# zhouyou-gu/sig-sdp-mmw

Hardware: AMD Instinct MI355X
Metric: mmw_iterations_per_sec (higher is better)
Workload: dtype f32

## Files before the change

include/mmw_hip.h:

```cpp
#ifndef MMW_HIP_H
#define MMW_HIP_H

#include <stddef.h>
#include <stdint.h>

#ifdef __cplusplus
extern "C" {
#endif

typedef struct mmw_solver mmw_solver;

#define MMW_OK 0
#define MMW_ERR_ARG (-1)
#define MMW_ERR_HIP (-2)
#define MMW_ERR_STATE (-3)

enum mmw_dtype { MMW_F32 = 0, MMW_F64 = 1 };
enum mmw_expm_method {
    MMW_EXPM_LANCZOS = 0,
    MMW_EXPM_TAYLOR = 1
};

enum mmw_field {
    MMW_F_Y = 0,
    MMW_F_E_ACCU = 1,
    MMW_F_E_THIS = 2,
    MMW_F_LVAL = 3,
    MMW_F_XVAL = 4,
    MMW_F_XAVG = 5,
    MMW_F_YAVG = 6,
    MMW_F_XHALF = 7,
    MMW_F_SKETCH = 8,
    MMW_F_S_SUM = 9,
    MMW_F_NORM_H = 10,
    MMW_F_ST_DATA = 11,
    MMW_F_PHASE_US = 12,
    MMW_F_EXPM_INFO = 13,
    MMW_F_FACTOR = 14,
    MMW_F_BLOCKING = 16,
    MMW_F_SPMM_KIND = 17,
    MMW_F_E_MAX = 18,
    MMW_F_DUAL_INFO = 19,
    MMW_F_FACTOR_INFO = 20,
    MMW_F_FACTOR_CALL = 21,
    MMW_F_SPLIT_CALL = 22,
    MMW_F_FACTOR_ROWNORM = 23,
    MMW_F_HEAD_CALL = 24,
    MMW_F_PATTERN = 25,
    MMW_F_BUILD_INFO = 26,
    MMW_F_LAPLACIAN = 27,
    MMW_F_SPECTRAL_INFO = 28,
    MMW_F_SPECTRAL_EIG = 29,
    MMW_F_GAP_INFO = 30,
    MMW_F_KERNEL_US = 15
};
enum mmw_ifield {
    MMW_I_L_INDPTR = 0,
    MMW_I_L_INDICES = 1,
    MMW_I_ST_INDPTR = 2,
    MMW_I_ST_INDICES = 3,
    MMW_I_GAIN_X = 4,
    MMW_I_GAIN_Y = 5,
    MMW_I_ASSO_X = 6,
    MMW_I_ASSO_Y = 7,
    MMW_I_DIAG_POS = 8,
    MMW_I_ASSO_POS = 9,
    MMW_I_PATTERN = 10,
    MMW_I_ROUND_LIST_BUILDS = 11
};

const char* mmw_last_error(void);
int mmw_version(void);
int mmw_device_count(int* n);

int mmw_create(mmw_solver** out, int device, int dtype, int32_t K, int32_t Z, int32_t rank_radio, double eta,
               int32_t nit, const int32_t* S_indptr, const int32_t* S_indices, const double* S_data,
               const int32_t* Q_indptr, const int32_t* Q_indices, const double* Q_data, const double* h_max);
int mmw_destroy(mmw_solver* s);

int mmw_sizes(mmw_solver* s, int64_t out[10]);

int mmw_set_expm(mmw_solver* s, int method, int max_order, double tol);
int mmw_set_timing(mmw_solver* s, int enabled);

int mmw_set_profile(mmw_solver* s, int enabled);

int mmw_bench_spmm(mmw_solver* s, int blocked, int reps, double* avg_us);

int mmw_reset(mmw_solver* s, int32_t nit);

int mmw_set_slots(mmw_solver* s, int32_t Z, int32_t nit);
int mmw_set_slots_warm(mmw_solver* s, int32_t Z, int32_t nit);
int mmw_carry(mmw_solver* dst, mmw_solver* src);
int mmw_carry_map(mmw_solver* dst, mmw_solver* src, int32_t* lmap, int64_t nl, int32_t* cmap, int64_t nc);
int mmw_set_eta(mmw_solver* s, double eta);

int mmw_iterate(mmw_solver* s, int32_t n, const double* randv, uint64_t seed);
int mmw_sync(mmw_solver* s);
int mmw_sketch(mmw_solver* s, uint64_t seed, int32_t iteration, double* out, int64_t n);

int mmw_read_f64(mmw_solver* s, int which, double* out, int64_t n);
int mmw_read_i32(mmw_solver* s, int which, int32_t* out, int64_t n);

int mmw_gap(mmw_solver* s, double out[3]);

int mmw_set_gap(mmw_solver* s, int enabled, int32_t m_cap, int32_t first_steps);
int mmw_read_gap(mmw_solver* s, double* out, int64_t n);
int mmw_gap_checks(int32_t K, int32_t m_cap, int32_t* out, int32_t room, int32_t* n);

int mmw_factor(mmw_solver* s, int32_t rank, double* out, uint64_t seed);

int mmw_factor_spectral(mmw_solver* s, int32_t Z, int32_t index_order, double* out, uint64_t seed);

#define MMW_FACTOR_RANDOM_MAX_COLS 2147483583
int mmw_factor_random(mmw_solver* s, int32_t cols, int32_t index_order, double* out, uint64_t seed);

int mmw_expm_apply(int device, int dtype, int method, int max_order, double tol, int32_t K, int32_t D,
                   const int32_t* indptr, const int32_t* indices, const double* data, const double* B,
                   double* out, double info[4], int32_t reps, double* kernel_us);

int mmw_sym_eig(int device, int32_t b, const double* G, double rel_tol, int32_t max_sweeps, double* theta, double* Q, int32_t* sweeps);

int mmw_round(mmw_solver* s, int32_t Zr, int32_t Dp, const double* gX, int32_t nbatch, const double* randv,
              int32_t* z_out, int32_t* rem_out);

typedef struct mmw_env mmw_env;
int mmw_env_create(mmw_env** out, int device, int32_t K, int32_t A, const double* sta_xy, const double* ap_xy, double fre_Hz,
                   double txp_offset, double min_s_n_ratio, double min_sinr, double noise_floor_dbm);
int mmw_env_destroy(mmw_env* e);
int mmw_env_sizes(mmw_env* e, int64_t out[4]);
int mmw_env_state(mmw_env* e, int32_t* S_indptr, int32_t* S_indices, double* S_data, int32_t* Q_indptr, int32_t* Q_indices,
                  double* Q_data, double* h_max);
int mmw_env_evaluate(mmw_env* e, const double* z_vec, int32_t Z, double packet_bit, double bandwidth, double slot_time,
                     double* sinr_out, double* bler_out);
int mmw_create_from_env(mmw_solver** out, mmw_env* env, int dtype, int32_t Z, int32_t rank_radio, double eta, int32_t nit);
int mmw_env_bounds(mmw_env* e, int32_t out[2]);
int mmw_env_move(mmw_env* e, const double* sta_xy);
int mmw_round_env(mmw_solver* s, mmw_env* e, int32_t Zr, int32_t Dp, const double* gX, int32_t nbatch, const double* randv,
                  int32_t* z_out, int32_t* rem_out);
int mmw_round_attempts(mmw_solver* s, int32_t Zr, int32_t Dp, const double* gX, int32_t nattempt, uint64_t seed, int pick_rule,
                       int32_t* z_out, int32_t* rem_out, int32_t* pick_out, int32_t* z_all);
int mmw_round_env_attempts(mmw_solver* s, mmw_env* e, int32_t Zr, int32_t Dp, const double* gX, int32_t nattempt, uint64_t seed, int pick_rule,
                           int32_t* z_out, int32_t* rem_out, int32_t* pick_out, int32_t* z_all);
int mmw_round_randv(mmw_solver* s, int32_t Zr, int32_t Dp, uint64_t seed, int32_t attempt, double* out, int64_t n);

typedef struct mmw_csr mmw_csr;
int mmw_csr_upload(mmw_csr** out, int device, int32_t K, int64_t nnzS, int64_t nnzQ, const int32_t* S_indptr,
                   const int32_t* S_indices, const double* S_data, const int32_t* Q_indptr, const int32_t* Q_indices,
                   const double* Q_data, const double* h_max);
int mmw_csr_wrap(mmw_csr** out, int device, int32_t K, int64_t nnzS, int64_t nnzQ, const int32_t* S_indptr,
                 const int32_t* S_indices, const double* S_data, const int32_t* Q_indptr, const int32_t* Q_indices,
                 const double* Q_data, const double* h_max);
int mmw_csr_destroy(mmw_csr* c);
int mmw_csr_sizes(mmw_csr* c, int64_t out[4]);
int mmw_csr_pointers(mmw_csr* c, void* out[7]);
int mmw_csr_state(mmw_csr* c, int32_t* S_indptr, int32_t* S_indices, double* S_data, int32_t* Q_indptr, int32_t* Q_indices,
                  double* Q_data, double* h_max);
int mmw_csr_bounds(mmw_csr* c, int32_t out[2]);
int mmw_create_from_csr(mmw_solver** out, mmw_csr* csr, int dtype, int32_t Z, int32_t rank_radio, double eta, int32_t nit);

typedef struct mmw_gm mmw_gm;
int mmw_gm_create(mmw_gm** out, int device, int32_t K, const int32_t* S_indptr, const int32_t* S_indices, const double* S_data,
                  const int32_t* Q_indptr, const int32_t* Q_indices, const double* Q_data, const double* h_max);
int mmw_gm_create_from_env(mmw_gm** out, mmw_env* e);
int mmw_gm_key(mmw_gm* g, int kind, double* key_out);
int mmw_gm_destroy(mmw_gm* g);
int mmw_gm_sizes(mmw_gm* g, int64_t out[4]);
int mmw_gm_pass(mmw_gm* g, const int32_t* order, int32_t n, int32_t nattempt, int32_t* list_out, int32_t* nlist);
int mmw_gm_run(mmw_gm* g, const double* key, int32_t Z, int32_t nattempt, int32_t* z_out, int32_t* zz_out, int32_t* rem_out);
int mmw_gm_assign(mmw_gm* g, int32_t Z, const int32_t* order, const int32_t* pref, int32_t* z_out, int32_t* rem_out);

typedef struct mmw_batch mmw_batch;
int mmw_batch_create(mmw_batch** out, int device, int32_t B, const int32_t* K, const int32_t* Z, int32_t rank_radio, double eta,
                     const int32_t* nit, const int32_t* const* S_indptr, const int32_t* const* S_indices, const double* const* S_data,
                     const int32_t* const* Q_indptr, const int32_t* const* Q_indices, const double* const* Q_data, const double* const* h_max);
int mmw_batch_destroy(mmw_batch* b);
int mmw_batch_sizes(mmw_batch* b, int32_t inst, int64_t out[10]);
int mmw_batch_set_slots(mmw_batch* b, const int32_t* Z, int32_t nit);
int mmw_batch_set_slots_warm(mmw_batch* b, const int32_t* Z, int32_t nit);
int mmw_batch_carry(mmw_batch* dst, mmw_batch* src, const int32_t* take);
int mmw_batch_carry_map(mmw_batch* dst, mmw_batch* src, int32_t inst, int32_t* lmap, int64_t nl, int32_t* cmap, int64_t nc);
int mmw_batch_reset(mmw_batch* b, int32_t nit);
int mmw_batch_set_eta(mmw_batch* b, const double* eta);
int mmw_batch_set_expm(mmw_batch* b, int max_order, double tol);
int mmw_batch_iterate(mmw_batch* b, int32_t n, const double* randv, const uint64_t* seeds);
int mmw_batch_set_gap(mmw_batch* b, int enabled, int32_t m_cap);
int mmw_batch_read_gap(mmw_batch* b, int32_t inst, double* out, int64_t n);
#define MMW_BATCH_MAX_PARTS 32
int mmw_batch_set_split(mmw_batch* b, const int32_t* parts);
#define MMW_BATCH_MAX_ROW_PARTS 64
int mmw_batch_set_row_split(mmw_batch* b, const int32_t* rows);
int mmw_batch_row_ranges(mmw_batch* b, int32_t inst, int32_t rows, int32_t* out);
#define MMW_BATCH_MAX_HEAD_PARTS 64
int mmw_batch_set_head_split(mmw_batch* b, const int32_t* parts);
int mmw_batch_head_ranges(mmw_batch* b, int32_t inst, int32_t parts, int32_t* out);
int mmw_batch_read_f64(mmw_batch* b, int32_t inst, int which, double* out, int64_t n);
int mmw_batch_read_i32(mmw_batch* b, int32_t inst, int which, int32_t* out, int64_t n);
int mmw_batch_sketch(mmw_batch* b, int32_t inst, uint64_t seed, int32_t iteration, double* out, int64_t n);
int mmw_batch_export(mmw_batch* b, int32_t inst, mmw_solver* h);
#define MMW_BATCH_EPILOGUE_MAX_K 1024
int mmw_batch_set_factor_split(mmw_batch* b, const int32_t* parts);
int mmw_batch_factor(mmw_batch* b, const int32_t* take, const int32_t* rank, const double* const* xavg);
int mmw_batch_round(mmw_batch* b, const int32_t* take, int32_t nattempt, int stop_at_first, const uint64_t* seeds, int32_t* z_out,
                    int32_t* rem_out, int32_t* used_out);
int mmw_batch_round_randv(mmw_batch* b, int32_t inst, uint64_t seed, int32_t attempt, double* out, int64_t n);
int mmw_batch_gm(mmw_batch* b, int kind, const int32_t* take, const int32_t* Z, int32_t nattempt, int32_t* z_out, int32_t* zz_out,
                 int32_t* rem_out, double* key_out);
int mmw_batch_factor_random(mmw_batch* b, const int32_t* take, const uint64_t* seeds);
int mmw_batch_factor_spectral(mmw_batch* b, const int32_t* take, const int32_t* Z);

typedef struct mmw_batch_env mmw_batch_env;
int mmw_batch_env_create(mmw_batch_env** out, int device, int32_t B, const int32_t* K, const int32_t* A, const double* const* ap_xy,
                         double fre_Hz, double txp_offset, double min_s_n_ratio, double min_sinr, double noise_floor_dbm);
int mmw_batch_env_destroy(mmw_batch_env* e);
int mmw_batch_env_move(mmw_batch_env* e, const double* const* sta_xy);
int mmw_batch_env_sizes(mmw_batch_env* e, int32_t inst, int64_t out[4]);
int mmw_batch_env_state(mmw_batch_env* e, int32_t inst, int32_t* S_indptr, int32_t* S_indices, double* S_data, int32_t* Q_indptr,
                        int32_t* Q_indices, double* Q_data, double* h_max);
int mmw_batch_env_evaluate(mmw_batch_env* e, const double* const* z_vec, const int32_t* Z, double packet_bit, double bandwidth,
                           double slot_time, double* const* sinr_out, double* const* bler_out);
int mmw_batch_round_env(mmw_batch* b, mmw_batch_env* e, const int32_t* take, int32_t nattempt, int stop_at_first,
                        const uint64_t* seeds, int32_t* z_out, int32_t* rem_out, int32_t* used_out);
int mmw_batch_create_from_env(mmw_batch** out, mmw_batch_env* env, const int32_t* Z, int32_t rank_radio, double eta, const int32_t* nit);
int mmw_batch_create_from_csr(mmw_batch** out, int32_t B, mmw_csr* const* csr, const int32_t* Z, int32_t rank_radio, double eta,
                              const int32_t* nit);
int mmw_batch_env_gm(mmw_batch_env* e, int kind, const int32_t* take, const int32_t* Z, int32_t nattempt, int32_t* z_out,
                     int32_t* zz_out, int32_t* rem_out, double* key_out);

#ifdef __cplusplus
}
#endif
#endif
```

sig_sdp_mmw_amd/_lib.py:

```python
import ctypes as C
import os
import weakref

import numpy as np

_HERE = os.path.dirname(os.path.abspath(__file__))
LIB_PATH = os.path.join(_HERE, "libmmw_hip.so")

F32, F64 = 0, 1
EXPM_LANCZOS, EXPM_TAYLOR = 0, 1

F_Y, F_E_ACCU, F_E_THIS, F_LVAL, F_XVAL, F_XAVG, F_YAVG, F_XHALF, F_SKETCH = range(9)
F_S_SUM, F_NORM_H, F_ST_DATA, F_PHASE_US, F_EXPM_INFO, F_FACTOR, F_KERNEL_US, F_BLOCKING, F_SPMM_KIND, F_E_MAX, F_DUAL_INFO = range(9, 20)
F_FACTOR_INFO = 20
F_FACTOR_CALL = 21
F_FACTOR_ROWNORM = 23
F_SPLIT_CALL = 22
F_HEAD_CALL = 24
BATCH_F_PATTERN = 25
BATCH_F_BUILD_INFO = 26
SOLVER_F_LAPLACIAN = 27
SOLVER_F_SPECTRAL_INFO = 28
SOLVER_F_SPECTRAL_EIG = 29
SOLVER_F_GAP_INFO = 30
BATCH_MAX_PARTS = 32
BATCH_MAX_ROW_PARTS = 64
BATCH_MAX_HEAD_PARTS = 64
BATCH_EPILOGUE_MAX_K = 1024
KERNEL_CLASSES = ["spmm", "sddmm", "dual", "loss", "krylov_vec", "sketch", "project", "greedy", "factor"]
I_L_INDPTR, I_L_INDICES, I_ST_INDPTR, I_ST_INDICES, I_GAIN_X, I_GAIN_Y, I_ASSO_X, I_ASSO_Y, I_DIAG_POS, I_ASSO_POS = range(10)
I_ROUND_LIST_BUILDS = 11
I_PATTERN = 10

EXPORTS = ["mmw_last_error", "mmw_version", "mmw_device_count", "mmw_create", "mmw_destroy", "mmw_sizes", "mmw_set_expm",
           "mmw_set_timing", "mmw_set_profile", "mmw_bench_spmm", "mmw_reset", "mmw_set_slots", "mmw_set_slots_warm", "mmw_set_eta", "mmw_iterate", "mmw_sync", "mmw_sketch", "mmw_read_f64", "mmw_read_i32", "mmw_gap",
           "mmw_factor", "mmw_expm_apply", "mmw_sym_eig", "mmw_round", "mmw_env_create", "mmw_env_destroy", "mmw_env_sizes", "mmw_env_state",
           "mmw_env_evaluate", "mmw_create_from_env", "mmw_env_bounds", "mmw_gm_create", "mmw_gm_destroy", "mmw_gm_sizes", "mmw_gm_pass",
           "mmw_gm_run", "mmw_gm_assign", "mmw_batch_create", "mmw_batch_destroy", "mmw_batch_sizes", "mmw_batch_set_slots",
           "mmw_batch_set_slots_warm", "mmw_batch_reset", "mmw_batch_set_eta", "mmw_batch_set_expm", "mmw_batch_iterate", "mmw_batch_read_f64", "mmw_batch_read_i32",
           "mmw_batch_sketch", "mmw_batch_export", "mmw_batch_set_gap", "mmw_batch_read_gap", "mmw_batch_factor", "mmw_batch_round",
           "mmw_batch_round_randv", "mmw_batch_env_create", "mmw_batch_env_destroy", "mmw_batch_env_move", "mmw_batch_env_sizes",
           "mmw_batch_env_state", "mmw_batch_env_evaluate", "mmw_batch_round_env", "mmw_batch_gm", "mmw_batch_env_gm",
           "mmw_batch_factor_random", "mmw_batch_factor_spectral", "mmw_batch_set_split", "mmw_batch_set_factor_split", "mmw_batch_set_row_split",
           "mmw_batch_row_ranges", "mmw_batch_carry", "mmw_batch_carry_map", "mmw_batch_set_head_split", "mmw_batch_head_ranges",
           "mmw_batch_create_from_env", "mmw_batch_create_from_csr", "mmw_csr_upload", "mmw_csr_wrap", "mmw_csr_destroy", "mmw_csr_sizes", "mmw_csr_pointers", "mmw_csr_state",
           "mmw_csr_bounds", "mmw_create_from_csr", "mmw_factor_spectral", "mmw_env_move", "mmw_round_env", "mmw_gm_create_from_env", "mmw_gm_key", "mmw_carry", "mmw_carry_map",
           "mmw_round_attempts", "mmw_round_env_attempts", "mmw_round_randv", "mmw_factor_random",
           "mmw_set_gap", "mmw_read_gap", "mmw_gap_checks"]


class MMWError(RuntimeError):
    pass


_lib = None


def lib():
    global _lib
    if _lib is not None:
        return _lib
    if not os.path.exists(LIB_PATH):
        raise MMWError("HIP library %s not found: build it first (python -c 'import __graft_entry__ as g; g.build()'). "
                       "There is no CPU fallback." % LIB_PATH)
    L = C.CDLL(LIB_PATH)
    p_i32 = C.POINTER(C.c_int32)
    p_f64 = C.POINTER(C.c_double)
    L.mmw_last_error.restype = C.c_char_p
    L.mmw_last_error.argtypes = []
    L.mmw_version.restype = C.c_int
    L.mmw_device_count.argtypes = [C.POINTER(C.c_int)]
    L.mmw_create.argtypes = [C.POINTER(C.c_void_p), C.c_int, C.c_int, C.c_int32, C.c_int32, C.c_int32, C.c_double, C.c_int32,
                             p_i32, p_i32, p_f64, p_i32, p_i32, p_f64, p_f64]
    L.mmw_destroy.argtypes = [C.c_void_p]
    L.mmw_sizes.argtypes = [C.c_void_p, C.POINTER(C.c_int64)]
    L.mmw_set_expm.argtypes = [C.c_void_p, C.c_int, C.c_int, C.c_double]
    L.mmw_set_timing.argtypes = [C.c_void_p, C.c_int]
    L.mmw_set_profile.argtypes = [C.c_void_p, C.c_int]
    L.mmw_bench_spmm.argtypes = [C.c_void_p, C.c_int, C.c_int, p_f64]
    L.mmw_reset.argtypes = [C.c_void_p, C.c_int32]
    L.mmw_set_slots.argtypes = [C.c_void_p, C.c_int32, C.c_int32]
    L.mmw_set_slots_warm.argtypes = [C.c_void_p, C.c_int32, C.c_int32]
    L.mmw_set_eta.argtypes = [C.c_void_p, C.c_double]
    L.mmw_carry.argtypes = [C.c_void_p, C.c_void_p]
    L.mmw_carry_map.argtypes = [C.c_void_p, C.c_void_p, p_i32, C.c_int64, p_i32, C.c_int64]
    L.mmw_iterate.argtypes = [C.c_void_p, C.c_int32, p_f64, C.c_uint64]
    L.mmw_sync.argtypes = [C.c_void_p]
    L.mmw_sketch.argtypes = [C.c_void_p, C.c_uint64, C.c_int32, p_f64, C.c_int64]
    L.mmw_read_f64.argtypes = [C.c_void_p, C.c_int, p_f64, C.c_int64]
    L.mmw_read_i32.argtypes = [C.c_void_p, C.c_int, p_i32, C.c_int64]
    L.mmw_gap.argtypes = [C.c_void_p, p_f64]
    L.mmw_set_gap.argtypes = [C.c_void_p, C.c_int, C.c_int32, C.c_int32]
    L.mmw_read_gap.argtypes = [C.c_void_p, p_f64, C.c_int64]
    L.mmw_gap_checks.argtypes = [C.c_int32, C.c_int32, p_i32, C.c_int32, p_i32]
    L.mmw_factor.argtypes = [C.c_void_p, C.c_int32, p_f64, C.c_uint64]
    L.mmw_factor_spectral.argtypes = [C.c_void_p, C.c_int32, C.c_int32, p_f64, C.c_uint64]
    L.mmw_factor_random.argtypes = [C.c_void_p, C.c_int32, C.c_int32, p_f64, C.c_uint64]
    L.mmw_sym_eig.argtypes = [C.c_int, C.c_int32, p_f64, C.c_double, C.c_int32, p_f64, p_f64, C.POINTER(C.c_int32)]
    L.mmw_expm_apply.argtypes = [C.c_int, C.c_int, C.c_int, C.c_int, C.c_double, C.c_int32, C.c_int32, p_i32, p_i32, p_f64,
                                 p_f64, p_f64, p_f64, C.c_int32, p_f64]
    L.mmw_round.argtypes = [C.c_void_p, C.c_int32, C.c_int32, p_f64, C.c_int32, p_f64, p_i32, p_i32]
    L.mmw_env_create.argtypes = [C.POINTER(C.c_void_p), C.c_int, C.c_int32, C.c_int32, p_f64, p_f64, C.c_double, C.c_double, C.c_double, C.c_double,
                                 C.c_double]
    L.mmw_env_destroy.argtypes = [C.c_void_p]
    L.mmw_env_sizes.argtypes = [C.c_void_p, C.POINTER(C.c_int64)]
    L.mmw_env_state.argtypes = [C.c_void_p, p_i32, p_i32, p_f64, p_i32, p_i32, p_f64, p_f64]
    L.mmw_env_evaluate.argtypes = [C.c_void_p, p_f64, C.c_int32, C.c_double, C.c_double, C.c_double, p_f64, p_f64]
    L.mmw_create_from_env.argtypes = [C.POINTER(C.c_void_p), C.c_void_p, C.c_int, C.c_int32, C.c_int32, C.c_double, C.c_int32]
    L.mmw_env_bounds.argtypes = [C.c_void_p, p_i32]
    L.mmw_env_move.argtypes = [C.c_void_p, p_f64]
    L.mmw_round_env.argtypes = [C.c_void_p, C.c_void_p, C.c_int32, C.c_int32, p_f64, C.c_int32, p_f64, p_i32, p_i32]
    L.mmw_round_attempts.argtypes = [C.c_void_p, C.c_int32, C.c_int32, p_f64, C.c_int32, C.c_uint64, C.c_int, p_i32, p_i32, p_i32, p_i32]
    L.mmw_round_env_attempts.argtypes = [C.c_void_p, C.c_void_p, C.c_int32, C.c_int32, p_f64, C.c_int32, C.c_uint64, C.c_int, p_i32, p_i32, p_i32, p_i32]
    L.mmw_round_randv.argtypes = [C.c_void_p, C.c_int32, C.c_int32, C.c_uint64, C.c_int32, p_f64, C.c_int64]
    L.mmw_gm_create_from_env.argtypes = [C.POINTER(C.c_void_p), C.c_void_p]
    L.mmw_gm_key.argtypes = [C.c_void_p, C.c_int, p_f64]
    for fn in (L.mmw_csr_upload, L.mmw_csr_wrap):
        fn.argtypes = [C.POINTER(C.c_void_p), C.c_int, C.c_int32, C.c_int64, C.c_int64] + [C.c_void_p] * 7
    L.mmw_csr_destroy.argtypes = [C.c_void_p]
    L.mmw_csr_sizes.argtypes = [C.c_void_p, C.POINTER(C.c_int64)]
    L.mmw_csr_pointers.argtypes = [C.c_void_p, C.POINTER(C.c_void_p)]
    L.mmw_csr_state.argtypes = [C.c_void_p, p_i32, p_i32, p_f64, p_i32, p_i32, p_f64, p_f64]
    L.mmw_csr_bounds.argtypes = [C.c_void_p, p_i32]
    L.mmw_create_from_csr.argtypes = [C.POINTER(C.c_void_p), C.c_void_p, C.c_int, C.c_int32, C.c_int32, C.c_double, C.c_int32]
    L.mmw_gm_create.argtypes = [C.POINTER(C.c_void_p), C.c_int, C.c_int32, p_i32, p_i32, p_f64, p_i32, p_i32, p_f64, p_f64]
    L.mmw_gm_destroy.argtypes = [C.c_void_p]
    L.mmw_gm_sizes.argtypes = [C.c_void_p, C.POINTER(C.c_int64)]
    L.mmw_gm_pass.argtypes = [C.c_void_p, p_i32, C.c_int32, C.c_int32, p_i32, p_i32]
    L.mmw_gm_run.argtypes = [C.c_void_p, p_f64, C.c_int32, C.c_int32, p_i32, p_i32, p_i32]
    L.mmw_gm_assign.argtypes = [C.c_void_p, C.c_int32, p_i32, p_i32, p_i32, p_i32]
    pp_i32 = C.POINTER(p_i32)
    pp_f64 = C.POINTER(p_f64)
    L.mmw_batch_create.argtypes = [C.POINTER(C.c_void_p), C.c_int, C.c_int32, p_i32, p_i32, C.c_int32, C.c_double, p_i32,
                                   pp_i32, pp_i32, pp_f64, pp_i32, pp_i32, pp_f64, pp_f64]
    L.mmw_batch_destroy.argtypes = [C.c_void_p]
    L.mmw_batch_sizes.argtypes = [C.c_void_p, C.c_int32, C.POINTER(C.c_int64)]
    L.mmw_batch_set_slots.argtypes = [C.c_void_p, p_i32, C.c_int32]
    L.mmw_batch_set_slots_warm.argtypes = [C.c_void_p, p_i32, C.c_int32]
    L.mmw_batch_carry.argtypes = [C.c_void_p, C.c_void_p, p_i32]
    L.mmw_batch_carry_map.argtypes = [C.c_void_p, C.c_void_p, C.c_int32, p_i32, C.c_int64, p_i32, C.c_int64]
    L.mmw_batch_reset.argtypes = [C.c_void_p, C.c_int32]
    L.mmw_batch_set_eta.argtypes = [C.c_void_p, p_f64]
    L.mmw_batch_set_expm.argtypes = [C.c_void_p, C.c_int, C.c_double]
    L.mmw_batch_iterate.argtypes = [C.c_void_p, C.c_int32, p_f64, C.POINTER(C.c_uint64)]
    L.mmw_batch_read_f64.argtypes = [C.c_void_p, C.c_int32, C.c_int, p_f64, C.c_int64]
    L.mmw_batch_read_i32.argtypes = [C.c_void_p, C.c_int32, C.c_int, p_i32, C.c_int64]
    L.mmw_batch_sketch.argtypes = [C.c_void_p, C.c_int32, C.c_uint64, C.c_int32, p_f64, C.c_int64]
    L.mmw_batch_export.argtypes = [C.c_void_p, C.c_int32, C.c_void_p]
    L.mmw_batch_set_gap.argtypes = [C.c_void_p, C.c_int, C.c_int32]
    L.mmw_batch_read_gap.argtypes = [C.c_void_p, C.c_int32, p_f64, C.c_int64]
    L.mmw_batch_set_split.argtypes = [C.c_void_p, p_i32]
    L.mmw_batch_set_factor_split.argtypes = [C.c_void_p, p_i32]
    L.mmw_batch_set_row_split.argtypes = [C.c_void_p, p_i32]
    L.mmw_batch_row_ranges.argtypes = [C.c_void_p, C.c_int32, C.c_int32, p_i32]
    L.mmw_batch_set_head_split.argtypes = [C.c_void_p, p_i32]
    L.mmw_batch_head_ranges.argtypes = [C.c_void_p, C.c_int32, C.c_int32, p_i32]
    L.mmw_batch_factor.argtypes = [C.c_void_p, p_i32, p_i32, pp_f64]
    L.mmw_batch_round.argtypes = [C.c_void_p, p_i32, C.c_int32, C.c_int, C.POINTER(C.c_uint64), p_i32, p_i32, p_i32]
    L.mmw_batch_round_randv.argtypes = [C.c_void_p, C.c_int32, C.c_uint64, C.c_int32, p_f64, C.c_int64]
    L.mmw_batch_env_create.argtypes = [C.POINTER(C.c_void_p), C.c_int, C.c_int32, p_i32, p_i32, pp_f64, C.c_double, C.c_double, C.c_double,
                                       C.c_double, C.c_double]
    L.mmw_batch_env_destroy.argtypes = [C.c_void_p]
    L.mmw_batch_env_move.argtypes = [C.c_void_p, pp_f64]
    L.mmw_batch_env_sizes.argtypes = [C.c_void_p, C.c_int32, C.POINTER(C.c_int64)]
    L.mmw_batch_env_state.argtypes = [C.c_void_p, C.c_int32, p_i32, p_i32, p_f64, p_i32, p_i32, p_f64, p_f64]
    L.mmw_batch_env_evaluate.argtypes = [C.c_void_p, pp_f64, p_i32, C.c_double, C.c_double, C.c_double, pp_f64, pp_f64]
    L.mmw_batch_round_env.argtypes = [C.c_void_p, C.c_void_p, p_i32, C.c_int32, C.c_int, C.POINTER(C.c_uint64), p_i32, p_i32, p_i32]
    L.mmw_batch_gm.argtypes = [C.c_void_p, C.c_int, p_i32, p_i32, C.c_int32, p_i32, p_i32, p_i32, p_f64]
    L.mmw_batch_env_gm.argtypes = [C.c_void_p, C.c_int, p_i32, p_i32, C.c_int32, p_i32, p_i32, p_i32, p_f64]
    L.mmw_batch_factor_random.argtypes = [C.c_void_p, p_i32, C.POINTER(C.c_uint64)]
    L.mmw_batch_factor_spectral.argtypes = [C.c_void_p, p_i32, p_i32]
    L.mmw_batch_create_from_env.argtypes = [C.POINTER(C.c_void_p), C.c_void_p, p_i32, C.c_int32, C.c_double, p_i32]
    L.mmw_batch_create_from_csr.argtypes = [C.POINTER(C.c_void_p), C.c_int32, C.POINTER(C.c_void_p), p_i32, C.c_int32, C.c_double, p_i32]
    for name in EXPORTS:
        if name not in ("mmw_last_error",):
            getattr(L, name).restype = C.c_int
    _lib = L
    return L


def check(rc):
    if rc != 0:
        raise MMWError("mmw_hip status %d: %s" % (rc, lib().mmw_last_error().decode("utf-8", "replace")))


def _pi(a):
    return a.ctypes.data_as(C.POINTER(C.c_int32))


def _pd(a):
    return a.ctypes.data_as(C.POINTER(C.c_double))


def _i32(a):
    return np.ascontiguousarray(a, dtype=np.int32)


def _f64(a):
    return np.ascontiguousarray(a, dtype=np.float64)


def _u64(seeds, B):
    return np.ascontiguousarray(np.broadcast_to(np.asarray(seeds, dtype=np.uint64), (B,)))


def _pu(a):
    return a.ctypes.data_as(C.POINTER(C.c_uint64))


def _opt_pi(t):
    return None if t is None else _pi(t)


def _gm_call(fn, handle, B, Ks, who, kind, Zs, nattempt, t, keys):
    Z = _i32(np.broadcast_to(np.asarray(Zs, dtype=np.int32), (B,)))
    n = max(1, sum(Ks[i] for i in who))
    zflat = np.empty(n, dtype=np.int32)
    kflat = np.empty(n, dtype=np.float64) if keys else None
    zz = np.empty(B, dtype=np.int32)
    rem = np.empty(B, dtype=np.int32)
    check(fn(handle, int(kind), _opt_pi(t), _pi(Z), int(nattempt), _pi(zflat), _pi(zz), _pi(rem), _pd(kflat) if keys else None))
    z, ks, o = [None] * B, [None] * B, 0
    for i in who:
        z[i] = zflat[o:o + Ks[i]]
        if keys:
            ks[i] = kflat[o:o + Ks[i]]
        o += Ks[i]
    return (z, zz, rem, ks) if keys else (z, zz, rem)


def device_count():
    n = C.c_int(0)
    check(lib().mmw_device_count(C.byref(n)))
    return n.value


def canonical_csr(m):
    import scipy.sparse
    m = scipy.sparse.csr_matrix(m)
    if not m.has_canonical_format:
        m = m.copy()
        m.sum_duplicates()
    return _i32(m.indptr), _i32(m.indices), _f64(m.data)


def _state_arrays(state):
    S, Q, h = state
    K = int(S.shape[0])
    if S.shape != (K, K) or Q.shape != (K, K) or len(h) != K:
        raise MMWError("state must be (S_gain KxK, Q_asso KxK, h_max[K])")
    return K, canonical_csr(S) + canonical_csr(Q) + (_f64(h),)


def _state_out(K, nnzS, nnzQ, fill):
    import scipy.sparse
    sp = np.empty(K + 1, dtype=np.int32); si = np.empty(nnzS, dtype=np.int32); sx = np.empty(nnzS, dtype=np.float64)
    qp = np.empty(K + 1, dtype=np.int32); qi = np.empty(nnzQ, dtype=np.int32); qx = np.empty(nnzQ, dtype=np.float64)
    h = np.empty(K, dtype=np.float64)
    fill(_pi(sp), _pi(si), _pd(sx), _pi(qp), _pi(qi), _pd(qx), _pd(h))
    return scipy.sparse.csr_matrix((sx, si, sp), shape=(K, K)), scipy.sparse.csr_matrix((qx, qi, qp), shape=(K, K)), h


_SIZE_NAMES = ("K", "Z", "D", "Dpad", "nnzL", "nnzST", "E_gain", "E_asso", "C", "iter")
_LEN = {F_Y: "C", F_E_ACCU: "C", F_E_THIS: "C", F_LVAL: "nnzL", F_XVAL: "nnzL", F_XAVG: "nnzL", F_YAVG: "C",
        F_S_SUM: "K", F_NORM_H: "K", F_ST_DATA: "nnzST", SOLVER_F_LAPLACIAN: "nnzL", F_FACTOR_ROWNORM: "K"}
_ILEN = {I_L_INDPTR: ("K", 1), I_L_INDICES: ("nnzL", 0), I_ST_INDPTR: ("K", 1), I_ST_INDICES: ("nnzST", 0), I_GAIN_X: ("E_gain", 0),
         I_GAIN_Y: ("E_gain", 0), I_ASSO_X: ("E_asso", 0), I_ASSO_Y: ("E_asso", 0), I_DIAG_POS: ("K", 0), I_ASSO_POS: ("E_asso", 0)}


def gap_checks(K, m_cap=0):
    n = C.c_int32(0)
    check(lib().mmw_gap_checks(int(K), int(m_cap), None, 0, C.byref(n)))
    out = np.empty(n.value, dtype=np.int32)
    check(lib().mmw_gap_checks(int(K), int(m_cap), _pi(out), int(out.size), C.byref(n)))
    return [int(x) for x in out]


class _Handle:
    _destroy = None

    def _closing(self):
        """Called by `close` while the handle is still valid."""

    def close(self):
        if getattr(self, "_h", None) is not None and self._h.value:
            try:
                self._closing()
            finally:
                getattr(lib(), self._destroy)(self._h)
                self._h = C.c_void_p()

    def __del__(self):
        try:
            self.close()
        except Exception:
            pass


class Solver(_Handle):
    _destroy = "mmw_destroy"

    def __init__(self, Z, state, nit, eta, rank_radio=2, dtype=F64, device=0):
        self.K, (sp, si, sx, qp, qi, qx, hm) = _state_arrays(state)
        self._h = C.c_void_p()
        check(lib().mmw_create(C.byref(self._h), int(device), int(dtype), self.K, int(Z), int(rank_radio), float(eta), int(nit),
                               _pi(sp), _pi(si), _pd(sx), _pi(qp), _pi(qi), _pd(qx), _pd(hm)))
        self._load_sizes()
        self.dtype = dtype
        self._timing = False
        self._timed = 0

    @classmethod
    def from_env(cls, env, Z, nit, eta, rank_radio=2, dtype=F64):
        self = cls.__new__(cls)
        self._h = C.c_void_p()
        check(lib().mmw_create_from_env(C.byref(self._h), env._h, int(dtype), int(Z), int(rank_radio), float(eta), int(nit)))
        self._load_sizes()
        self.dtype = dtype
        self._timing = False
        self._timed = 0
        return self

    @classmethod
    def from_csr(cls, csr, Z, nit, eta, rank_radio=2, dtype=F64):
        self = cls.__new__(cls)
        self._h = C.c_void_p()
        check(lib().mmw_create_from_csr(C.byref(self._h), csr._h, int(dtype), int(Z), int(rank_radio), float(eta), int(nit)))
# ... 1060 lines not shown
```

sig_sdp_mmw_amd/csrc/chunk_policy.h:

```cpp
#pragma once
#include <algorithm>
#include <cmath>

#include "kernels_expm.h"
#include "kernels_mfma.h"
#include "switches.h"

namespace mmw {

struct ChunkPolicy {
    int age0 = 0;
    int age(int iter) const { return age0 + iter; }
    double rho_prev = 0.0, rho_last = 0.0;
    int age_prev = -1, age_last = -1;
    bool warm_fresh = false;
    bool lagged_missed = false;
    bool plan_seen = false;
    bool chain_ok = false;
    int replays = 0;
    int m_guess = 3;
    bool first_guess = false;
    bool first_a16_guess = false;
    bool exact_plans_only = false;
    void on_reset() {
        age0 = 0; warm_fresh = false; age_prev = age_last = -1;
        chain_ok = false; plan_seen = false; lagged_missed = false; m_guess = 3;
    }
    void on_warm_restart(int iter) {
        age0 += iter; warm_fresh = true; age_prev = age_last = -1;
        chain_ok = false; lagged_missed = false;
    }
    void on_discard() { chain_ok = false; }
    void note_plan(const ExpmPlan& p, int iter) {
        if (age_last >= 0 && age(iter) > age_last) { rho_prev = rho_last; age_prev = age_last; }
        rho_last = p.rho; age_last = age(iter);
    }
    double growth_ratio(int iter, int ahead) const {
        double r = (double)(age(iter) + ahead + 1) / (double)std::max(age(iter), 1);
        if (age_prev >= 0 && age_last > age_prev && rho_last > 0.0 && rho_last > rho_prev) {
            const double slope = (rho_last - rho_prev) / (double)(age_last - age_prev);
            r = std::max(r, (rho_last + 1.5 * slope * (double)(ahead + 1)) / rho_last);
        }
        return r;
    }
    bool first_order_ok(const ExpmPlan& p, const Switches& sw, int iter, int ahead, bool fp32, double plane_rounding, bool a16 = false) const {
        if (sw.no_first_order || !fp32 || !p.apost || p.m_eff != 1 || p.first_est == 0u) return false;
        const double est = plan_estimate(p.first_est);
        const double g1 = growth_ratio(iter, ahead), absn_g = p.absn * g1;
        if (!(absn_g < 0.03)) return false;
        if (a16 ? !((F16_PLANE_EXPECT + F16_UNIT) * absn_g <= p.tol) : !(F16_PLANE_EXPECT * absn_g <= p.tol)) return false;
        const double rounding = std::exp(p.rho * g1) * (absn_g * (plane_rounding + (a16 ? F16_UNIT : F16_CA_TWO)) + F16_SUBNORMAL_ROW);
        return est <= p.tol / 4.0 && est * g1 * g1 + rounding <= 0.9 * p.tol;
    }
    int next_launch_order(const ExpmPlan& p, int max_order, int iter, int ahead = 0) const {
        if (p.m_eff <= 0) return std::min(max_order, p.m + 1);
        int spare = 1;
        if (p.apost && p.m_eff >= 1 && p.m_eff <= MAX_ORDER) {
            const double est = plan_estimate(p.conv[p.m_eff]);
            const double grow = std::pow(growth_ratio(iter, ahead), 2.0 * p.m_eff);
            if (est <= p.tol / 8.0 && est * grow <= p.tol / 2.0) spare = 0;
        }
        if (p.m_eff >= p.m_apriori) spare = 0;
        return std::min(max_order, p.m_eff + spare);
    }
    int room_iterations(const ExpmPlan& p, int iter) const {
        if (!p.apost || p.m_eff != 1) return 0;
        const double est = plan_estimate(p.conv[1]);
        if (!(est > 0.0)) return 32;
        double c = 0.5 * (double)age(iter) * (std::sqrt(p.tol / est) - 1.0);
        if (age_prev >= 0 && age_last > age_prev && rho_last > rho_prev && rho_last > 0.0)
            c = std::min(c, 0.5 * (std::sqrt(p.tol / est) - 1.0) * rho_last * (double)(age_last - age_prev) / (1.5 * (rho_last - rho_prev)));
        return c > 32.0 ? 32 : (c < 0.0 ? 0 : (int)c);
    }
    bool plan_has_room(const ExpmPlan& p) const { return p.apost && p.m_eff == 1 && plan_estimate(p.conv[1]) <= p.tol / 8.0; }
    bool lagged_ok(const ExpmPlan& p, const Switches& sw) const {
        if (sw.no_lagged_plan || lagged_missed || !p.apost || p.m_eff != 1) return false;
        return plan_estimate(p.conv[1]) <= p.tol / 2.0;
    }
    int chunk_length(const ExpmPlan& p, const Switches& sw, int iter, int left) const {
        int cap = lagged_ok(p, sw) ? std::max(8, std::min(32, age(iter))) : std::max(4, std::min(32, age(iter) / 2));
        if (chain_ok && age(iter) >= 4) cap = std::max(cap, std::min(32, room_iterations(p, iter)));
        if (warm_fresh) cap = 8;
        int chunk = std::min(left, cap);
        if (left - chunk == 1) ++chunk;
        return chunk;
    }
    void plan_chunk(const ExpmPlan& p, const Switches& sw, int max_order, int iter, int chunk, bool fp32, bool have_a16, double plane_rounding) {
        if (plan_seen) m_guess = next_launch_order(p, max_order, iter, chunk);
        first_guess = plan_seen && first_order_ok(p, sw, iter, chunk, fp32, plane_rounding);
        if (first_guess) m_guess = 1;
        first_a16_guess = first_guess && !sw.no_first_a16 && have_a16 && first_order_ok(p, sw, iter, chunk, fp32, plane_rounding, true);
        if (warm_fresh) {
            m_guess = std::min(max_order, std::max(2, p.m_eff + 1));
            first_guess = false;
        }
    }
    void plan_cautious(const ExpmPlan& p, int max_order) {
        first_guess = false;
        first_a16_guess = false;
        m_guess = std::min(max_order, std::max(std::max(p.m_apriori, p.m_eff), m_guess) + 1);
    }
};
}
```

sig_sdp_mmw_amd/csrc/expm_engine.h:

```cpp
#pragma once
#include <cmath>

#include <functional>
#include <type_traits>

#include "kernels_expm.h"
#include "kernels_mfma.h"
#include "runtime.h"

namespace mmw {

inline int make_layout(int D, int vec, BlockLayout& lay, std::string& err) {
    int lpr = (D + vec - 1) / vec;
    if (lpr <= 32) {
        int p = 1;
        while (p < lpr) p <<= 1;
        lpr = p;
        lay.G = WAVE / lpr;
        lay.NCH = 1;
    } else {
        lpr = (lpr + 7) / 8 * 8;
        if ((lpr + WAVE - 1) / WAVE > 4) {
            err = "sketch width D too large for this build (max 1024 f32 / 512 f64 columns)";
            return MMW_ERR_ARG;
        }
        lay.G = 1;
        lay.NCH = (lpr + WAVE - 1) / WAVE;
    }
    lay.D = D;
    lay.LPR = lpr;
    lay.Dpad = lpr * vec;
    return MMW_OK;
}

template <typename T> inline int slice_bytes(const Switches& sw, int K, const BlockLayout& lay) {
    const int row_bytes = lay.Dpad * (int)sizeof(T);
    if (sw.no_slice_spmm || K < 256) return 0;
    if ((size_t)K * 64 <= (size_t)SLICE_LDS_MAX && row_bytes % 64 == 0) return 64;
    if ((size_t)K * 32 <= (size_t)SLICE_LDS_MAX && row_bytes % 32 == 0) return 32;
    return 0;
}
template <typename T> inline int slice_ranges(int K, const BlockLayout& lay, int sb) {
    const int nslices = lay.Dpad * (int)sizeof(T) / sb;
    return std::max(1, std::min((K + 15) / 16, device_cus() / std::max(1, nslices)));
}
template <typename T> inline int generic_slabs(const Switches& sw, int K, const BlockLayout& lay, int nblk) {
    const int sb = slice_bytes<T>(sw, K, lay);
    return sb ? std::min(nblk, slice_ranges<T>(K, lay, sb)) : nblk;
}
template <typename T, int MODE>
inline int spmm_launch(hipStream_t st, const Switches& sw, int K, const BlockLayout& lay, int nblk, const int* indptr, const int* col, const T* val,
                       const T* in, T* out, T* F, const T* X2, double c1, double c2, double c3, double* partial,
                       const ExpmPlan* plan = nullptr, int step = 0, double* partial_o2 = nullptr, int nslabs_fold = -1) {
    if (const int sb = slice_bytes<T>(sw, K, lay)) {
        const int nslices = lay.Dpad * (int)sizeof(T) / sb;
        int nranges = slice_ranges<T>(K, lay, sb);
        if (MODE == SPMM_LANCZOS) nranges = std::min(nranges, nblk);
        const int fold = nslabs_fold > 0 ? nslabs_fold : nblk;
        const size_t lds = (size_t)K * sb;
        if (sb == 64) {
            MMW_TRY(set_max_lds(reinterpret_cast<const void*>(&k_spmm_slice<T, MODE, 64>), SLICE_LDS_MAX));
            hipLaunchKernelGGL((k_spmm_slice<T, MODE, 64>), dim3(nslices, nranges), dim3(SLICE_THREADS), lds, st, K, lay.Dpad, indptr, col, val, in, out, F, X2, c1, c2, c3,
                               partial, plan, step, partial_o2, fold);
        } else {
            MMW_TRY(set_max_lds(reinterpret_cast<const void*>(&k_spmm_slice<T, MODE, 32>), SLICE_LDS_MAX));
            hipLaunchKernelGGL((k_spmm_slice<T, MODE, 32>), dim3(nslices, nranges), dim3(SLICE_THREADS), lds, st, K, lay.Dpad, indptr, col, val, in, out, F, X2, c1, c2, c3,
                               partial, plan, step, partial_o2, fold);
        }
        MMW_HIP(hipGetLastError());
        return MMW_OK;
    }
    const size_t sh = MODE == SPMM_LANCZOS ? (size_t)WAVES_PER_BLOCK * lay.Dpad * sizeof(double) : 0;
    switch (lay.NCH) {
        case 1: hipLaunchKernelGGL((k_spmm<T, 1, MODE>), dim3(nblk), dim3(BLOCK), sh, st, K, lay, indptr, col, val, in, out, F, X2, c1, c2, c3, partial, plan, step, partial_o2); break;
        case 2: hipLaunchKernelGGL((k_spmm<T, 2, MODE>), dim3(nblk), dim3(BLOCK), sh, st, K, lay, indptr, col, val, in, out, F, X2, c1, c2, c3, partial, plan, step, partial_o2); break;
        case 3: hipLaunchKernelGGL((k_spmm<T, 3, MODE>), dim3(nblk), dim3(BLOCK), sh, st, K, lay, indptr, col, val, in, out, F, X2, c1, c2, c3, partial, plan, step, partial_o2); break;
        default: hipLaunchKernelGGL((k_spmm<T, 4, MODE>), dim3(nblk), dim3(BLOCK), sh, st, K, lay, indptr, col, val, in, out, F, X2, c1, c2, c3, partial, plan, step, partial_o2); break;
    }
    MMW_HIP(hipGetLastError());
    return MMW_OK;
}

inline Blk2Sched blk2_schedule(int nb, int ntiles) {
    const int slots = 2 * device_cus();
    Blk2Sched s;
    int tpw = (int)((double)nb * ntiles / (2.5 * slots) + 0.5);
    tpw = tpw < 1 ? 1 : (tpw > ntiles ? ntiles : tpw);
    s.nfull = 0; s.grid1 = 0; s.tpw_tail = tpw; s.groups_tail = (ntiles + tpw - 1) / tpw;
    return s;
}

inline unsigned long long* g_blk_stamps = nullptr;
template <typename T, int MODE>
inline int spmm_blk_launch(hipStream_t st, const BlkDev& B, int Dpad, const T* val_blk, const T* in, T* out, T* F, const T* X2,
                           double c1, double c2, double c3, double* partial, const ExpmPlan* plan = nullptr, int step = 0,
                           double* partial_o2 = nullptr) {
    if (B.half_tile) {
        constexpr int CT2 = B2_ROW_BYTES / (int)sizeof(T);
        const int ntiles = (Dpad + CT2 - 1) / CT2;
        const Blk2Sched sched = blk2_schedule(B.nb, ntiles);
        const int rem = B.nb - sched.nfull;
        const int grid = sched.grid1 + ((rem * sched.groups_tail + 7) / 8) * 8;
        MMW_TRY(set_max_lds(reinterpret_cast<const void*>(&k_spmm_blk2<T, MODE>), B2_LDS_BYTES));
        hipLaunchKernelGGL((k_spmm_blk2<T, MODE>), dim3(grid), dim3(B2_THREADS), B2_LDS_BYTES, st, B, Dpad, ntiles, sched, val_blk, in, out, F, X2, c1, c2, c3, partial, partial_o2, plan, step, g_blk_stamps);
        MMW_HIP(hipGetLastError());
        return MMW_OK;
    }
    constexpr int CT = BLK_TILE_BYTES / (int)sizeof(T);
    const int ntiles = (Dpad + CT - 1) / CT;
    int tpw = (int)((double)B.nb * ntiles / (3.0 * 256.0) + 0.5);
    tpw = tpw < 1 ? 1 : (tpw > ntiles ? ntiles : tpw);
    const int total = B.nb * ((ntiles + tpw - 1) / tpw);
    const int per = (total + 7) / 8;
    const size_t sh = (size_t)BLK_UNION_ROWS * BLK_TILE_BYTES + BLK_META_LDS + BLK_ROWINFO_LDS + BLK_UNOFF_LDS + (size_t)BLK_WAVES * CT * sizeof(double);
    MMW_TRY(set_max_lds(reinterpret_cast<const void*>(&k_spmm_blk<T, MODE>), (int)sh));
    hipLaunchKernelGGL((k_spmm_blk<T, MODE>), dim3(per * 8), dim3(BLK_THREADS), sh, st, B, Dpad, ntiles, tpw, val_blk, in, out, F, X2, c1, c2, c3, partial, plan, step, g_blk_stamps);
    MMW_HIP(hipGetLastError());
    return MMW_OK;
}

inline unsigned long long* g_mf_stamps = nullptr;
template <int MODE>
inline int spmm_mfma_launch(hipStream_t st, const Switches& sw, const MfmaDev& M, int mt, int Dpad, size_t plane_bytes, const char* planes, const float* in,
                            float* out, double ascale, double shift, double* partial, double* partial_o2, const ExpmPlan* plan, int step, int* viol,
                            MfEpi epi = MfEpi{}, int* grid_out = nullptr ,
                            hipEvent_t ev_a = nullptr, hipEvent_t ev_b = nullptr ) {
    const int ntiles = Dpad / 32;
    const int grid_x = (M.nb + 7) / 8 * 8;
    const int cus = device_cus();
#define MMW_MF_LAUNCH(MT, NT, NW, MS, KC, NB)                                                                                          \
    do {                                                                                                                               \
        constexpr int gtw = (NW / MS) * NT;                                                                                            \
        constexpr int lds_bytes = mf_lds_bytes<MT, gtw, KC, NB, mf_planes(MODE), mf_apieces(MODE)>();                                  \
        MMW_TRY(set_max_lds(reinterpret_cast<const void*>(&k_spmm_mfma<MODE, MT, NT, NW, MS, KC, NB>), lds_bytes));                    \
        if (ev_a)                                                                                                                      \
            hipExtLaunchKernelGGL((k_spmm_mfma<MODE, MT, NT, NW, MS, KC, NB>), dim3(grid_x, (ntiles + gtw - 1) / gtw), dim3(NW * 64),  \
                                  lds_bytes, st, ev_a, ev_b, 0, M, Dpad, plane_bytes, planes, in, out, ascale, shift, partial,         \
                                  partial_o2, plan, step, viol, g_mf_stamps, epi);                                                     \
        else                                                                                                                           \
        hipLaunchKernelGGL((k_spmm_mfma<MODE, MT, NT, NW, MS, KC, NB>), dim3(grid_x, (ntiles + gtw - 1) / gtw), dim3(NW * 64),         \
                           lds_bytes, st, M, Dpad, plane_bytes, planes, in, out, ascale, shift, partial, partial_o2,                   \
                           plan, step, viol, g_mf_stamps, epi);                                                                        \
        if (grid_out) *grid_out = grid_x * ((ntiles + gtw - 1) / gtw);                                                                 \
    } while (0)
    int gt = 12;
    if (sw.mf_gt) gt = sw.mf_gt;
    else {
        auto wgs = [&](int g) { return (long)M.nb * ((ntiles + g - 1) / g); };
        if (wgs(12) * 2 < 3L * cus) gt = 8;
        if (gt == 8 && wgs(8) * 2 < 3L * cus) gt = 4;
    }
    if (ntiles <= 4) gt = 4;
    else if (ntiles <= 8 && gt > 8) gt = 8;
    if (mt == 1) {
        if (gt == 4) MMW_MF_LAUNCH(1, 1, 4, 1, 2, 2);
        else if (gt == 8) MMW_MF_LAUNCH(1, 2, 4, 1, 2, 2);
        else MMW_MF_LAUNCH(1, 3, 4, 1, 1, 3);
    } else {
        if (gt == 4) {
            if constexpr (mf_first(MODE)) MMW_MF_LAUNCH(2, 1, 8, 2, 4, 2);
            else MMW_MF_LAUNCH(2, 1, 8, 2, 2, 2);
        }
        else if (gt == 8) MMW_MF_LAUNCH(2, 2, 8, 2, 2, 2);
        else MMW_MF_LAUNCH(2, 3, 4, 1, 1, 3);
    }
#undef MMW_MF_LAUNCH
    MMW_HIP(hipGetLastError());
    return MMW_OK;
}

template <typename T> struct ExpmEngine {
    const Switches& sw;
    explicit ExpmEngine(const Switches& s) : sw(s) {}
    hipStream_t st = nullptr;
    int K = 0;
    BlockLayout lay{};
    int method = MMW_EXPM_LANCZOS, max_order = 8;
    double tol = 1e-9;
    int nblk = 1, nwide = 1;
    const int* indptr = nullptr;
    const int* col = nullptr;
    const T* val = nullptr;
    DevBuf<T> U;
    DevBuf<T> Tm;
    DevBuf<double> partial_du;
    DevBuf<double> partial, partial_sq, partial_o2, colsum, scal, row_part;
    DevBuf<ExpmPlan> plan_d;
    DevBuf<int> viol_d;
    ExpmPlan* plan_h = nullptr;
    ExpmPlan last{};
    size_t bs = 0;
    KernelTimers* kt = nullptr;
    bool use_blk = false;
    BlkDev blk{};
    const T* val_blk = nullptr;
    int npart = 1;
    bool use_mfma = false;
    MfmaDev mf{};
    int mf_mt = 1;
    DevBuf<unsigned short> planes;
    bool mfma_now() const { return use_mfma && use_blk && std::is_same<T, float>::value && (lay.Dpad % 32) == 0 && last_mfma_ok; }
    int spmm_slabs() const { return mfma_now() ? mf.nb : npart; }
    int check_slabs(int slabs) const {
        if ((size_t)slabs * lay.Dpad > partial.cap || (size_t)slabs * lay.Dpad > partial_o2.cap)
            return fail(MMW_ERR_STATE, "internal: the per-block slabs of the SpMM outgrew their buffers");
        return MMW_OK;
    }
    bool last_mfma_ok = true;
    bool* blk_stale = nullptr;
    std::function<int()> blk_refresh;
    T* rownorm_d = nullptr;
    double* rownorm_part = nullptr;
    unsigned short* out_planes = nullptr;
    bool kt_exact = false;
    bool planes_only = false;
    bool start_colsq_ready = false;
    int npart_start = 0;
    bool apost() const { return (!use_blk || blk.half_tile) && method == MMW_EXPM_LANCZOS && !sw.no_apost; }
    int kbegin(int slot) { return kt ? kt->begin(slot) : MMW_OK; }
    int kend() { return kt ? kt->end() : MMW_OK; }

    ~ExpmEngine() {
        if (plan_h) (void)hipHostFree(plan_h);
    }
    int init(hipStream_t s, int K_, int D, const int* ip, const int* ci, const T* v) {
        st = s;
        K = K_;
        indptr = ip;
        col = ci;
        val = v;
        return resize(D);
    }
    int resize(int D) {
        std::string err;
        if (make_layout(D, V16<T>::N, lay, err) != MMW_OK) return fail(MMW_ERR_ARG, err);
        bs = (size_t)K * lay.Dpad;
        nblk = grid_slabs(K);
        nwide = grid_rows(K);
        ublocks = 0;
        for (auto& r : planes_ready) r = false;
        MMW_TRY(ensure_blocks(4));
        MMW_TRY(Tm.alloc(bs));
        const size_t slabs = std::max((size_t)MAX_PART, std::max(use_blk ? (size_t)blk.nb : (size_t)0, use_mfma ? (size_t)mf.nb : (size_t)0));
        MMW_TRY(partial.alloc(slabs * lay.Dpad));
        MMW_TRY(partial_sq.alloc((size_t)MAX_PART * lay.Dpad));
        MMW_TRY(partial_du.alloc((size_t)MAX_PART * lay.Dpad));
        MMW_TRY(partial_o2.alloc(slabs * lay.Dpad));
        npart = generic_slabs<T>(sw, K, lay, nblk);
        MMW_TRY(colsum.alloc(lay.Dpad));
        MMW_TRY(scal.alloc((size_t)4 * (MAX_ORDER + 2) * lay.Dpad));
        MMW_TRY(row_part.alloc((size_t)3 * ROW_GRID_MAX));
        MMW_TRY(plan_d.alloc(1));
        MMW_HIP(hipMemsetAsync(plan_d.p, 0, sizeof(ExpmPlan), st));
        MMW_TRY(reset_plan_history(false));
        MMW_TRY(viol_d.alloc(1));
        MMW_HIP(hipMemsetAsync(viol_d.p, 0, sizeof(int), st));
        if (!plan_h) MMW_HIP(hipHostMalloc((void**)&plan_h, sizeof(ExpmPlan)));
        if (use_blk) MMW_TRY(enable_blocking(blk, val_blk));
        return MMW_OK;
    }
    int ublocks = 0;
    int ensure_blocks(int n) {
        if (n <= ublocks) return MMW_OK;
        if (n > MAX_ORDER + 1) n = MAX_ORDER + 1;
        if (U.p && U.cap >= bs * (size_t)n) {
            if ((size_t)n > (size_t)std::max(ublocks, 1))
                MMW_HIP(hipMemsetAsync(U.p + bs * (size_t)std::max(ublocks, 1), 0, bs * (size_t)(n - std::max(ublocks, 1)) * sizeof(T), st));
            if (ublocks == 0) MMW_HIP(hipMemsetAsync(U.p, 0, bs * sizeof(T), st));
            U.n = bs * (size_t)n;
            ublocks = n;
            return MMW_OK;
        }
        DevBuf<T> bigger;
        MMW_TRY(bigger.alloc(bs * (size_t)n));
        MMW_HIP(hipMemsetAsync(bigger.p, 0, bs * (size_t)n * sizeof(T), st));
        if (U.p && ublocks > 0) MMW_HIP(hipMemcpyAsync(bigger.p, U.p, bs * sizeof(T), hipMemcpyDeviceToDevice, st));
        MMW_HIP(hipStreamSynchronize(st));
        std::swap(U.p, bigger.p);
        std::swap(U.n, bigger.n);
        std::swap(U.cap, bigger.cap);
        ublocks = n;
        return MMW_OK;
    }
    T* start_block() { return U.p; }
    T* block(int j) { return U.p + (size_t)j * bs; }
    LanczosScalars scalars() {
        LanczosScalars S;
        const size_t n = (size_t)(MAX_ORDER + 2) * lay.Dpad;
        S.alpha = scal.p;
        S.beta = scal.p + n;
        S.sinv = scal.p + 2 * n;
        S.coef = scal.p + 3 * n;
        return S;
    }

    unsigned short* planes_of(int idx) { return planes.p + (size_t)idx * 2 * bs; }
    bool planes_ready[MAX_ORDER + 2] = {false};
    bool planes0_f16 = false;
    int reserve_planes() {
        if (planes.n < (size_t)ublocks * 2 * bs) MMW_TRY(planes.alloc((size_t)ublocks * 2 * bs));
        for (auto& r : planes_ready) r = false;
        return MMW_OK;
    }
    int ensure_planes() {
        if (planes.n < (size_t)ublocks * 2 * bs) {
            MMW_HIP(hipStreamSynchronize(st));
            MMW_TRY(planes.alloc((size_t)ublocks * 2 * bs));
            for (auto& r : planes_ready) r = false;
        }
        return MMW_OK;
    }
    unsigned short* start_planes() {
        if (!mfma_now() || ensure_planes() != MMW_OK) return nullptr;
        return planes_of(0);
    }
    int make_planes(int idx) {
        if constexpr (std::is_same<T, float>::value) {
            MMW_TRY(ensure_planes());
            if (idx == 0 && planes0_f16) planes_ready[0] = false;
            if (planes_ready[idx]) return MMW_OK;
            if (idx == 0) planes0_f16 = false;
            MMW_TRY(kbegin(KT_KRYLOV_VEC));
            hipLaunchKernelGGL(k_split_planes, dim3(grid_elems(bs / 4)), dim3(BLOCK), 0, st, bs / 4, reinterpret_cast<const float4*>(block(idx)),
                               reinterpret_cast<uint2*>(planes_of(idx)), reinterpret_cast<uint2*>(planes_of(idx) + bs));
            MMW_HIP(hipGetLastError());
            return kend();
        }
        return MMW_OK;
    }
    template <int MODE> int launch_spmm(const T* in, T* out, T* F, double ascale, double shift, double inv_k,
                                        const ExpmPlan* plan = nullptr, int step = 0, const unsigned short* planes_in = nullptr) {
        if constexpr (std::is_same<T, float>::value && (MODE == SPMM_PLAIN || MODE == SPMM_LANCZOS)) {
            if (planes_in && mfma_now()) {
                MMW_TRY(check_slabs(mf.nb));
                hipEvent_t ea = nullptr, eb = nullptr;
                if (kt) MMW_TRY(kt->begin_attached(KT_SPMM, &ea, &eb));
                MMW_TRY((spmm_mfma_launch<MODE>(st, sw, mf, mf_mt, lay.Dpad, bs * sizeof(unsigned short), reinterpret_cast<const char*>(planes_in), in, out, ascale,
                                                shift, partial.p, apost() ? partial_o2.p : nullptr, plan, step, viol_d.p, MfEpi{}, nullptr, ea, eb)));
                return kend();
            }
        }
        if (use_blk && blk_stale && *blk_stale) {
            MMW_TRY(blk_refresh());
            *blk_stale = false;
        }
        MMW_TRY(kbegin(KT_SPMM));
        if (use_blk)
            MMW_TRY((spmm_blk_launch<T, MODE>(st, blk, lay.Dpad, val_blk, in, out, F, nullptr, ascale, shift, inv_k, partial.p, plan, step,
                                              apost() ? partial_o2.p : nullptr)));
        else
            MMW_TRY((spmm_launch<T, MODE>(st, sw, K, lay, nblk, indptr, col, val, in, out, F, nullptr, ascale, shift, inv_k, partial.p, plan, step,
                                          apost() ? partial_o2.p : nullptr, npart)));
        return kend();
    }
    int enable_blocking(const BlkDev& b, const T* values_blocked) {
        blk = b;
        val_blk = values_blocked;
        use_blk = true;
        npart = b.nb;
        if ((size_t)b.nb > (size_t)MAX_PART) {
            MMW_TRY(partial.alloc((size_t)b.nb * lay.Dpad));
            MMW_TRY(partial_o2.alloc((size_t)b.nb * lay.Dpad));
        }
        return MMW_OK;
    }
    template <int OP> int colreduce(int nb, int j, const ExpmPlan* plan) {
        const double eps = sizeof(T) == 4 ? 1e-6 : 1e-14;
        hipLaunchKernelGGL((k_colreduce<OP>), dim3((lay.Dpad + 15) / 16), dim3(1024), 0, st, nb, lay.Dpad, partial.p, colsum.p, j, eps, scalars(), plan);
        MMW_HIP(hipGetLastError());
        return MMW_OK;
    }

    int plan_iter = 0;
    int reset_plan_history(bool keep_sums) {
        hipLaunchKernelGGL(k_plan_reset, dim3(1), dim3(64), 0, st, plan_d.p, keep_sums ? 1 : 0);
        MMW_HIP(hipGetLastError());
        return MMW_OK;
    }
    int make_plan(double ascale, int m_launch) {
        hipLaunchKernelGGL((k_rowsums<T>), dim3(nwide), dim3(BLOCK), 0, st, K, indptr, col, val, ascale, row_part.p);
        hipLaunchKernelGGL(k_plan, dim3(1), dim3(PLAN_THREADS), 0, st, K, method, max_order, tol, row_part.p, nwide, plan_d.p, m_launch, viol_d.p, apost() ? 1 : 0,
                           plan_iter);
        MMW_HIP(hipGetLastError());
        if (m_launch > 0) return MMW_OK;
        MMW_HIP(hipMemcpyAsync(plan_h, plan_d.p, sizeof(ExpmPlan), hipMemcpyDeviceToHost, st));
        MMW_HIP(hipStreamSynchronize(st));
        last = *plan_h;
        last_mfma_ok = last.mfma_ok != 0;
        if (last.overflow) return fail(MMW_ERR_STATE, "expm: the one-norm of the matrix is too large for max_order (raise max_order)");
        return MMW_OK;
    }
    int fetch_plan(int* violated) {
        int v = 0;
        MMW_HIP(hipMemcpyAsync(plan_h, plan_d.p, sizeof(ExpmPlan), hipMemcpyDeviceToHost, st));
        MMW_HIP(hipMemcpyAsync(&v, viol_d.p, sizeof(int), hipMemcpyDeviceToHost, st));
        MMW_HIP(hipStreamSynchronize(st));
        last = *plan_h;
        last_mfma_ok = last.mfma_ok != 0;
        if (live_switch(LIVE_VERBOSE)) {
            fprintf(stderr, "[plan] rho %.3e absn %.3e mfma_ok %d tol %.1e m %d (a-priori %d) apost %d m_eff %d est[1] %.3e est[2] %.3e viol %d\n", last.rho,
                    last.absn, last.mfma_ok, last.tol, last.m, last.m_apriori, last.apost, last.m_eff, plan_estimate(last.conv[1]), plan_estimate(last.conv[2]), v);
        }
        if (violated) *violated = v;
        return MMW_OK;
    }
    int clear_violation() {
        MMW_HIP(hipMemsetAsync(viol_d.p, 0, sizeof(int), st));
        return MMW_OK;
    }

    int apply_first(T* out, double ascale, int m_launch, bool plan_made, unsigned short* y_planes, long long* dfx, double* tr_part, int* ntr,
                    const unsigned short* afrag16 = nullptr) {
        if constexpr (std::is_same<T, float>::value) {
            if (!plan_made) MMW_TRY(make_plan(ascale, m_launch));
            MMW_TRY(ensure_planes());
            if (!(planes_ready[0] && planes0_f16)) {
                MMW_TRY(kbegin(KT_KRYLOV_VEC));
                hipLaunchKernelGGL(k_plane_f16, dim3(grid_elems(bs / 4)), dim3(BLOCK), 0, st, bs / 4, reinterpret_cast<const float4*>(U.p),
                                   reinterpret_cast<uint2*>(planes_of(0)));
                MMW_HIP(hipGetLastError());
                MMW_TRY(kend());
            }
            MfEpi E;
            E.y_planes = y_planes; E.dfx = dfx; E.tr_part = tr_part;
            MMW_TRY(check_slabs(mf.nb));
            hipEvent_t ea = nullptr, eb = nullptr;
            if (kt) MMW_TRY(kt->begin_attached(KT_SPMM, &ea, &eb));
            if (afrag16) {
                MfmaDev m16 = mf;
                m16.afrag = reinterpret_cast<const unsigned*>(afrag16);
                MMW_TRY((spmm_mfma_launch<SPMM_FIRST16>(st, sw, m16, mf_mt, lay.Dpad, bs * sizeof(unsigned short), reinterpret_cast<const char*>(planes_of(0)), U.p, out,
                                                        ascale / (double)MF_F16_SCALE, 0.0, partial.p, partial_o2.p, plan_d.p, 1, viol_d.p, E, ntr, ea, eb)));
            } else
                MMW_TRY((spmm_mfma_launch<SPMM_FIRST>(st, sw, mf, mf_mt, lay.Dpad, bs * sizeof(unsigned short), reinterpret_cast<const char*>(planes_of(0)), U.p, out,
                                                      ascale / (double)MF_F16_SCALE, 0.0, partial.p, partial_o2.p, plan_d.p, 1, viol_d.p, E, ntr, ea, eb)));
            MMW_TRY(kend());
            planes_ready[0] = false;
            planes0_f16 = false;
            start_colsq_ready = false;
            return MMW_OK;
        }
        return fail(MMW_ERR_STATE, "the first-order product runs on fp32 matrix-core handles only");
    }
    int first_grid_max() const { return (mf.nb + 7) / 8 * 8 * (lay.Dpad / 32); }

    int apply(T* out, double ascale, int m_launch = 0, bool plan_made = false) {
        if (!plan_made) MMW_TRY(make_plan(ascale, m_launch));
        const int m = m_launch > 0 ? m_launch : last.m;
        const int nsub = m_launch > 0 ? 1 : last.nsub;
        MMW_TRY(ensure_blocks(std::max(3, m)));
        ExpmPlan* pd = plan_d.p;
        const int Dpad = lay.Dpad;
        const int gcol = (Dpad + 63) / 64;
        const int gel = grid_elems(bs);
        const size_t shcol = (size_t)BLOCK * sizeof(double);
        for (int sub = 0; sub < nsub; ++sub) {
            if (sub > 0) {
                hipLaunchKernelGGL((k_copy<T>), dim3(gel), dim3(BLOCK), 0, st, bs, out, U.p);
            }
            if (method == MMW_EXPM_LANCZOS) {
                LanczosScalars S = scalars();
                const int gr = grid_slabs(K * 4);
                const double eps = sizeof(T) == 4 ? 1e-6 : 1e-14;
                int nsq = npart_start;
                if (!(sub == 0 && start_colsq_ready)) {
                    MMW_TRY(kbegin(KT_KRYLOV_VEC));
                    hipLaunchKernelGGL((k_colsq<T>), dim3(gr), dim3(BLOCK), shcol, st, K, Dpad, U.p, partial_sq.p);
                    MMW_TRY(kend());
                    nsq = gr;
                }
                start_colsq_ready = false;
                for (int j = 1; j <= m; ++j) {
                    const bool mf_step = mfma_now();
                    if (mf_step) MMW_TRY(make_planes(j - 1));
                    MMW_TRY((launch_spmm<SPMM_LANCZOS>(block(j - 1), Tm.p, nullptr, ascale, 0.0, 1.0, pd, j, mf_step ? planes_of(j - 1) : nullptr)));
                    planes_ready[j - 1] = false;
                    MMW_TRY(kbegin(KT_KRYLOV_VEC));
#define MMW_LZS(NMAX)                                                                                                               \
    hipLaunchKernelGGL((k_lz_scalars<NMAX>), dim3((Dpad + LZS_COLS - 1) / LZS_COLS), dim3(1024), 0, st, mf_step ? mf.nb : npart, partial.p, \
                       apost() ? partial_o2.p : (double*)nullptr, nsq, partial_sq.p, Dpad, j, m, 1.0 / nsub, eps, S, pd)
                    if (j + 2 <= 4) MMW_LZS(4);
                    else if (j + 2 <= 8) MMW_LZS(8);
                    else MMW_LZS(MAX_ORDER + 2);
#undef MMW_LZS
                    if (kt && kt->on && kt_exact && apost() && j < m) {
                        MMW_TRY(kend());
                        MMW_HIP(hipMemcpyAsync(plan_h, plan_d.p, sizeof(ExpmPlan), hipMemcpyDeviceToHost, st));
                        MMW_HIP(hipStreamSynchronize(st));
                        union { float f; unsigned u; } tb;
                        tb.f = (float)plan_h->tol;
                        if (plan_h->apost && plan_h->conv[j] <= tb.u) break;
                        MMW_TRY(kbegin(KT_KRYLOV_VEC));
                    }
                    if (j < m) {
                        unsigned short* pl_next = nullptr;
                        if (mf_step && ensure_planes() == MMW_OK && j < ublocks) pl_next = planes_of(j);
                        hipLaunchKernelGGL((k_lz_update<T>), dim3(gr), dim3(BLOCK), shcol, st, K, Dpad, j, Tm.p, block(j - 1),
                                           j > 1 ? block(j - 2) : block(j - 1), block(j), S, partial_sq.p, pd, pl_next);
                        planes_ready[j] = pl_next != nullptr;
                        nsq = gr;
                    }
                    MMW_TRY(kend());
                }
                MMW_TRY(kbegin(KT_KRYLOV_VEC));
                const bool last = sub + 1 == nsub;
                hipLaunchKernelGGL((k_lz_combine<T>), dim3(nwide), dim3(BLOCK), 0, st, K, Dpad, m, U.p, bs, Tm.p, S.coef, out, pd,
                                   last ? rownorm_d : (T*)nullptr, last ? rownorm_part : (double*)nullptr, viol_d.p, last ? out_planes : (unsigned short*)nullptr,
                                   last && out_planes && planes_only ? 1 : 0);
                MMW_TRY(kend());
            } else {
                hipLaunchKernelGGL((k_copy<T>), dim3(gel), dim3(BLOCK), 0, st, bs, U.p, out);
                for (int k = 1; k <= m; ++k) {
                    T* in = k == 1 ? U.p : block((k - 1) % 2 + 1);
                    T* o = block(k % 2 + 1);
                    MMW_TRY((launch_spmm<SPMM_TAYLOR>(in, o, out, ascale / nsub, last.mu / nsub, 1.0 / k, pd, k)));
                }
                hipLaunchKernelGGL((k_scale<T>), dim3(gel), dim3(BLOCK), 0, st, bs, out, 1.0, pd);
            }
            MMW_HIP(hipGetLastError());
        }
        return MMW_OK;
    }
};

}
```

sig_sdp_mmw_amd/csrc/solver.h:

```cpp
#pragma once
#include "solver_bench.h"
#include "solver_carry.h"
#include "solver_create.h"
#include "solver_loop.h"
#include "solver_read.h"
#include "solver_replay.h"

struct mmw_env {
    mmw::EnvDevice e;
};
struct mmw_csr {
    mmw::CsrDevice c;
};
struct mmw_solver {
    virtual ~mmw_solver() {}
    virtual CarryInfo carry_info() = 0;
    virtual int carry_pattern(const mmw::HostPattern** out) = 0;
    virtual int carry(mmw_solver* src) = 0;
    virtual int sizes(int64_t out[10]) = 0;
    virtual int set_expm(int method, int max_order, double tol) = 0;
    virtual int set_timing(int enabled) = 0;
    virtual int set_profile(int enabled) = 0;
    virtual int bench_spmm(int blocked, int reps, double* avg_us) = 0;
    virtual int reset(int32_t nit) = 0;
    virtual int set_slots(int32_t Z, int32_t nit, int warm) = 0;
    virtual int set_eta(double eta) = 0;
    virtual int iterate(int32_t n, const double* randv, uint64_t seed) = 0;
    virtual int sync() = 0;
    virtual int sketch(uint64_t seed, int32_t iteration, double* out, int64_t n) = 0;
    virtual int read_f64(int which, double* out, int64_t n) = 0;
    virtual int read_i32(int which, int32_t* out, int64_t n) = 0;
    virtual int gap(double out[3]) = 0;
    virtual int set_gap(int enabled, int32_t m_cap, int32_t first_steps) = 0;
    virtual int read_gap(double* out, int64_t n) = 0;
    virtual int factor(int32_t rank, double* out, uint64_t seed) = 0;
    virtual int factor_spectral(int32_t Z, int32_t index_order, double* out, uint64_t seed) = 0;
    virtual int factor_random(int32_t cols, int32_t index_order, double* out, uint64_t seed) = 0;
    virtual int round(int32_t Zr, int32_t Dp, const double* gX, int32_t nbatch, const double* randv, int32_t* z_out,
                      int32_t* rem_out) = 0;
    virtual int round_env(mmw_env* env, int32_t Zr, int32_t Dp, const double* gX, int32_t nbatch, const double* randv, int32_t* z_out,
                          int32_t* rem_out) = 0;
    virtual int round_attempts(mmw_env* env, bool with_env, int32_t Zr, int32_t Dp, const double* gX, int32_t nattempt, uint64_t seed, int pick_rule,
                               int32_t* z_out, int32_t* rem_out, int32_t* pick_out, int32_t* z_all) = 0;
    virtual int round_randv(int32_t Zr, int32_t Dp, uint64_t seed, int32_t attempt, double* out, int64_t n) = 0;
};
namespace {
inline int host_only_handle() { return fail(MMW_ERR_STATE, "host-only handle"); }
inline int host_only_pattern() { return fail(MMW_ERR_STATE, "this handle was created with device -1 (host pattern only)"); }
template <typename T> struct Solver final : mmw_solver {
    SolverCore<T> core;
    SolverLoop<T> loop;
    PendingChunk<T> pending;
    EmaxRecord emax;
    SolverReads<T> reads;
    DeviceLists envl;
    Extras<T> extras;
    CarriedPlan carried;
    explicit Solver(const Switches& s) : core(s), loop(core.sw), extras(core.sw) {}
    ~Solver() override {
        core.bt.join();
        if (core.host_only) return;
        (void)hipSetDevice(core.device);
        if (core.st) (void)hipStreamDestroy(core.st);
    }
    using Create = SolverCreate<T>;
    int sizes(int64_t out[10]) override {
        const HostPattern& H = core.H;
        out[0] = core.K; out[1] = core.Z; out[2] = core.D; out[3] = core.eng.lay.Dpad; out[4] = H.nnzL(); out[5] = H.nnzST();
        out[6] = H.E_gain(); out[7] = H.E_asso(); out[8] = H.C(); out[9] = core.iter;
        return MMW_OK;
    }
    int set_expm(int method, int max_order, double tol) override {
        if (method != MMW_EXPM_LANCZOS && method != MMW_EXPM_TAYLOR) return fail(MMW_ERR_ARG, "unknown expm method");
        if (max_order < 1 || max_order > MAX_ORDER) return fail(MMW_ERR_ARG, "max_order must be in [1,16]");
        if (!(tol > 0)) return fail(MMW_ERR_ARG, "tol must be positive");
        core.eng.method = method; core.eng.max_order = max_order; core.eng.tol = tol;
        return MMW_OK;
    }
    int set_timing(int enabled) override {
        core.pt.timing = enabled != 0;
        core.pt.timing_stride = enabled > 1 ? enabled : 1;
        return MMW_OK;
    }
    int bench_spmm(int blocked, int reps, double* avg_us) override {
        if (core.host_only) return host_only_handle();
        MMW_HIP(hipSetDevice(core.device));
        if (blocked && !core.bt.HB.usable) return fail(MMW_ERR_STATE, "no locality blocking for this pattern");
        MMW_TRY(sync());
        return solver_bench_spmm(core, loop, blocked, reps, avg_us);
    }
    int set_profile(int enabled) override {
        if (core.host_only) return host_only_handle();
        MMW_TRY(sync());
        KernelTimers& kt = core.kt;
        kt.on = enabled != 0;
        core.kt_shipped = enabled == 2;
        kt.attach = core.kt_shipped && !core.sw.kt_markers;
        core.eng.kt_exact = kt.on && !core.kt_shipped;
        kt.clear();
        return MMW_OK;
    }
    int set_eta(double eta_) override {
        if (!(eta_ >= 0.0)) return fail(MMW_ERR_ARG, "eta must be non-negative");
        if (!core.host_only) {
            MMW_HIP(hipSetDevice(core.device));
            MMW_TRY(settle());
        }
        core.eta = eta_;
        return MMW_OK;
    }
    int set_slots(int32_t Z_, int32_t nit_, int warm) override {
        if (core.host_only) return host_only_pattern();
        MMW_HIP(hipSetDevice(core.device));
        MMW_TRY(settle());
        MMW_HIP(hipStreamSynchronize(core.st));
        if (warm && core.iter == 0) warm = 0;
        if (Z_ >= 2) {
            BlockLayout probe{};
            std::string lerr;
            if ((int64_t)Z_ * core.rank_radio > INT32_MAX || make_layout(Z_ * core.rank_radio, V16<T>::N, probe, lerr) != MMW_OK)
                return fail(MMW_ERR_ARG, "mmw_set_slots: " + (lerr.empty() ? std::string("sketch width D too large for this build") : lerr));
        }
        std::string err = update_slots(core.H, Z_);
        if (!err.empty()) return fail(MMW_ERR_ARG, "mmw_set_slots: " + err);
        core.Z = Z_;
        core.D = core.Z * core.rank_radio;
        MMW_TRY(core.upload_slot_scalars());
        MMW_TRY(core.eng.resize(core.D));
        MMW_TRY(core.Xh.alloc(core.eng.bs));
        MMW_TRY(reads.resize(core));
        MMW_TRY(loop.resize(core));
        MMW_TRY(on_restart(nit_, warm != 0));
        return warm ? core.sums_from_current() : core.initial_point();
    }
    int on_restart(int32_t nit_, bool warm) {
        if (nit_ < 1) return fail(MMW_ERR_ARG, "nit must be >= 1");
        core.nit = nit_;
        loop.on_restart(warm, core.iter, nit_);
        core.iter = 0;
        emax.drop();
        pending.clear();
        carried.drop();
        if (core.eng.viol_d.p) MMW_TRY(core.eng.clear_violation());
        return core.eng.reset_plan_history(warm);
    }
    int reset(int32_t nit_) override {
        if (core.host_only) return host_only_pattern();
        MMW_HIP(hipSetDevice(core.device));
        MMW_TRY(on_restart(nit_, false));
        return core.initial_point();
    }
    int restore_pending() {
        loop.pol.on_discard();
        emax.drop();
        MMW_TRY(core.eng.clear_violation());
        MMW_TRY(pending.restore(core));
        loop.gap.drop_pending();
        core.iter = pending.iter0;
        return core.pt.drop_since(pending.events0, core.st);
    }
    void say_replay(int viol, const char* how) const {
        if (!live_switch(LIVE_VERBOSE)) return;
        const ExpmPlan& p = core.eng.last;
        const ChunkPolicy& pol = loop.pol;
        fprintf(stderr, "[replay] iterations %d..%d (Z %d) %s: reason bits %d (1 order, 2 lagged plan, 4 plan, 8 softmax, 16 operands, 32 first-order certificate); launched m %d, first-order %d, one-half %d; "
                        "plan m %d m_eff %d apriori %d rho %.3g absn %.3g est %.2e first_est %.2e tol %.1e\n",
                pending.iter0, pending.iter0 + pending.n - 1, (int)core.H.Z, how, viol, pol.m_guess, (int)pol.first_guess, (int)pol.first_a16_guess, p.m, p.m_eff, p.m_apriori, p.rho, p.absn,
                plan_estimate(p.conv[std::max(0, std::min(p.m_eff, MAX_ORDER))]), plan_estimate(p.first_est), p.tol);
    }
    void accept_plan() {
        ChunkPolicy& pol = loop.pol;
        pol.plan_seen = true;
        pol.note_plan(core.eng.last, core.iter);
        pol.m_guess = pol.next_launch_order(core.eng.last, core.eng.max_order, core.iter);
    }
    int settle() {
        MMW_TRY(settle_chunk());
        return loop.gap.collect(core.st, core.d_indptr.p, core.d_col.p);
    }
    int settle_chunk() {
        if (!pending.live) return MMW_OK;
        pending.clear();
        ChunkPolicy& pol = loop.pol;
        ExpmEngine<T>& eng = core.eng;
        int viol = 0;
        MMW_TRY(eng.fetch_plan(&viol));
        if (!viol) {
            accept_plan();
            return MMW_OK;
        }
        ++pol.replays;
        const bool operands_only = (viol & VIOL_OPERANDS) && !pol.first_guess;
        if (viol & VIOL_LAGGED) pol.lagged_missed = true;
        say_replay(viol, "discarded");
        MMW_TRY(restore_pending());
        if (core.sw.cautious_replay && !operands_only && eng.method == MMW_EXPM_LANCZOS && pending.n > 1) {
            pol.plan_cautious(eng.last, eng.max_order);
            pol.exact_plans_only = true;
            const int rc = loop.iterate_impl(core, pending.n, nullptr, pending.seed, true);
            pol.exact_plans_only = false;
            MMW_TRY(rc);
            viol = 0;
            MMW_TRY(eng.fetch_plan(&viol));
            if (!viol) {
                accept_plan();
                say_replay(0, "cautious attempt accepted");
                return MMW_OK;
            }
            ++pol.replays;
            say_replay(viol, "cautious attempt discarded");
            MMW_TRY(restore_pending());
        }
        say_replay(0, "replayed synchronously");
        return loop.iterate_impl(core, pending.n, nullptr, pending.seed, false);
    }
    int iterate(int32_t n, const double* randv, uint64_t seed) override {
        if (core.host_only) return host_only_pattern();
        MMW_HIP(hipSetDevice(core.device));
        if (n < 0) return fail(MMW_ERR_ARG, "n must be >= 0");
        MMW_TRY(settle());
        if (core.iter + n > core.nit) return fail(MMW_ERR_STATE, "mmw_iterate: more iterations than announced to mmw_create/mmw_reset");
        ChunkPolicy& pol = loop.pol;
        const bool optimistic = randv == nullptr && n > 1 && !core.kt_exact() && !core.sw.sync_plan;
        if (!optimistic) {
            pol.chain_ok = false;
            MMW_TRY(loop.iterate_impl(core, n, randv, seed, false));
            carried.drop();
            return emax.enqueue(core);
        }
        int left = n;
        while (left > 0) {
            MMW_TRY(settle());
            const ExpmPlan& hist = carried.or_last(core.eng.last);
            const int chunk = pol.chunk_length(hist, core.sw, core.iter, left);
            pol.plan_chunk(hist, core.sw, core.eng.max_order, core.iter, chunk, sizeof(T) == 4, core.bt.afrag16.p != nullptr, loop.plane_rounding());
            MMW_TRY(pending.save(core));
            const int iter0 = core.iter;
            const size_t events0 = core.pt.mark();
            MMW_TRY(loop.iterate_impl(core, chunk, nullptr, seed, chunk > 1));
            pol.warm_fresh = false;
            carried.drop();
            if (chunk > 1) pending.begin(iter0, chunk, seed, events0);
            left -= chunk;
        }
        return emax.enqueue(core);
    }
    CarryInfo carry_info() override { return CarryInfo{core.host_only, core.device, sizeof(T) == 4 ? MMW_F32 : MMW_F64, core.K, core.iter}; }
    int carry_pattern(const HostPattern** out) override {
        MMW_TRY(envl.ensure_host(core));
        *out = &core.H;
        return MMW_OK;
    }
    int carry(mmw_solver* src_) override {
        if (src_ == this) return fail(MMW_ERR_ARG, "mmw_carry: the handle cannot carry from itself");
        MMW_TRY(carry_refusal("mmw_carry", carry_info(), src_->carry_info(), true));
        Solver<T>* src = static_cast<Solver<T>*>(src_);
        if (src->core.iter == 0) return MMW_OK;
        MMW_HIP(hipSetDevice(core.device));
        MMW_TRY(src->settle());
        MMW_TRY(src->core.x.csr_view(src->core));
        MMW_HIP(hipStreamSynchronize(src->core.st));
        MMW_TRY(SolverCarry<T>::gather(core, src->core));
        MMW_TRY(SolverCarry<T>::derived(core));
        emax.drop();
        pending.clear();
        MMW_TRY(SolverCarry<T>::history(core, loop, carried, src->core, src->loop));
        MMW_HIP(hipStreamSynchronize(core.st));
        return MMW_OK;
    }
    int sync() override {
        if (core.host_only) return host_only_pattern();
        MMW_HIP(hipSetDevice(core.device));
        MMW_TRY(settle());
        MMW_TRY(emax.fetch_at_sync(core));
        MMW_TRY(core.kt.flush());
        return core.pt.flush(core.iter, core.st);
    }
    int sketch(uint64_t seed, int32_t iteration, double* out, int64_t n) override {
        if (core.host_only) return host_only_pattern();
        if (iteration < 0) return fail(MMW_ERR_ARG, "mmw_sketch: iteration must be >= 0");
        MMW_HIP(hipSetDevice(core.device));
        MMW_TRY(sync());
        return reads.sketch(core, seed, iteration, out, n);
    }
    int read_f64(int which, double* out, int64_t n) override {
        const HostPattern& H = core.H;
        const std::vector<double>* hv = which == MMW_F_S_SUM ? &H.S_sum : which == MMW_F_NORM_H ? &H.norm_H : which == MMW_F_ST_DATA ? &H.st_data : nullptr;
        if (core.host_only && which == MMW_F_LAPLACIAN) {
            if (n != H.nnzL()) return fail(MMW_ERR_ARG, "mmw_read_f64(LAPLACIAN): wrong length " + std::to_string(n) + ", expected " + std::to_string(H.nnzL()));
            for (int r = 0; r < core.K; ++r) lap_row(H.l_indptr.data(), H.l_indices.data(), H.so_indptr.data(), H.so_indices.data(), H.so_data.data(), r, out);
            return MMW_OK;
        }
        if (core.host_only) return hv ? export_vec(*hv, out, n, "mmw_read_f64") : host_only_pattern();
        MMW_HIP(hipSetDevice(core.device));
        MMW_TRY(sync());
        if (which == MMW_F_ST_DATA) MMW_TRY(envl.ensure_host(core));
        if (hv) return export_vec(*hv, out, n, "mmw_read_f64");
        if (which == MMW_F_LAPLACIAN) return extras.read_laplacian(core.d_indptr.p, core.d_col.p, core.d_diag.p, (size_t)H.nnzL(), out, n);
        return reads.read_f64(core, loop, emax, extras, which, out, n);
    }
    int read_i32(int which, int32_t* out, int64_t n) override {
        if (which == MMW_I_ROUND_LIST_BUILDS) {
            if (n != 1) return fail(MMW_ERR_ARG, "mmw_read_i32(ROUND_LIST_BUILDS): wrong length");
            out[0] = extras.env_builds;
            return MMW_OK;
        }
        MMW_TRY(envl.ensure_host(core));
        const std::vector<int32_t>* v = host_list_i32(core.H, which);
        return v ? export_vec(*v, out, n, "mmw_read_i32") : fail(MMW_ERR_ARG, "mmw_read_i32: unknown field");
    }
    int gap(double out[3]) override {
        if (core.host_only) return host_only_handle();
        MMW_HIP(hipSetDevice(core.device));
        MMW_TRY(settle());
        if (core.iter >= core.nit) return fail(MMW_ERR_STATE, "mmw_gap: call it before an iteration (the running sums then hold iter+1 terms)");
        MMW_TRY(core.x.csr_view(core));
        PatternDev<T> Pc = core.pat();
        Pc.e2w = nullptr; Pc.xasso = nullptr; Pc.xdiag_base = -1;
        return extras.gap(Pc, core.d_lrow.p, core.xavg.p, core.yavg.p, core.iter + 1, out);
    }
    int set_gap(int enabled, int32_t m_cap, int32_t first_steps) override {
        if (core.host_only) return host_only_handle();
        MMW_HIP(hipSetDevice(core.device));
        MMW_TRY(settle());
        return loop.gap.configure(enabled, m_cap, first_steps, core.K, (size_t)core.H.nnzL(), core.nit);
    }
    int read_gap(double* out, int64_t n) override {
        if (core.host_only) return host_only_handle();
        MMW_HIP(hipSetDevice(core.device));
        MMW_TRY(settle());
        return loop.gap.read(core.iter, out, n);
    }
    int factor(int32_t rank, double* out, uint64_t seed) override {
        if (core.host_only) return host_only_handle();
        MMW_HIP(hipSetDevice(core.device));
        MMW_TRY(settle());
        if (core.iter < core.nit) return fail(MMW_ERR_STATE, "mmw_factor: run all announced iterations first (the average divides by nit)");
        MMW_TRY(core.x.csr_view(core));
        return extras.factor(core.d_indptr.p, core.d_col.p, core.xavg.p, core.nit, rank, out, seed);
    }
    int factor_spectral(int32_t Z, int32_t index_order, double* out, uint64_t seed) override {
        if (Z < 1 || Z > core.K) return fail(MMW_ERR_ARG, "mmw_factor_spectral: Z = " + std::to_string(Z) + " must be in [1, K = " + std::to_string(core.K) + "]");
        if (index_order != 0 && index_order != 1) return fail(MMW_ERR_ARG, "mmw_factor_spectral: index_order must be 0 or 1");
        if (core.host_only) return host_only_handle();
        MMW_HIP(hipSetDevice(core.device));
        MMW_TRY(settle());
        return extras.factor_spectral(core.d_indptr.p, core.d_col.p, core.d_diag.p, (size_t)core.H.nnzL(), Z, index_order, out, seed);
    }
    int factor_random(int32_t cols, int32_t index_order, double* out, uint64_t seed) override {
        if (cols < 1) return fail(MMW_ERR_ARG, "mmw_factor_random: cols = " + std::to_string(cols) + " must be >= 1");
        if (index_order != 0 && index_order != 1) return fail(MMW_ERR_ARG, "mmw_factor_random: index_order = " + std::to_string(index_order) + " must be 0 or 1");
        if (cols > MMW_FACTOR_RANDOM_MAX_COLS)
            return fail(MMW_ERR_ARG, "mmw_factor_random: cols = " + std::to_string(cols) + " exceeds " + std::to_string(MMW_FACTOR_RANDOM_MAX_COLS) +
                                         ", the widest D' the rounding's projection walks in its 64-column slabs");
        if (core.host_only) return host_only_handle();
        MMW_HIP(hipSetDevice(core.device));
        return extras.factor_random(cols, index_order, out, seed);
    }
    int round(int32_t Zr, int32_t Dp, const double* gX, int32_t nbatch, const double* randv, int32_t* z_out, int32_t* rem_out) override {
        if (core.host_only) return host_only_handle();
        MMW_HIP(hipSetDevice(core.device));
        return extras.round(Zr, Dp, gX, nbatch, randv, z_out, rem_out);
    }
    int round_env(mmw_env* env, int32_t Zr, int32_t Dp, const double* gX, int32_t nbatch, const double* randv, int32_t* z_out, int32_t* rem_out) override {
        if (core.host_only) return host_only_handle();
        if (!env) return fail(MMW_ERR_ARG, "mmw_round_env: null environment");
        const EnvDevice& E = env->e;
        if (E.K != core.K)
            return fail(MMW_ERR_ARG, "mmw_round_env: the environment has K = " + std::to_string(E.K) + " stations, the handle K = " + std::to_string(core.K));
        if (E.device != core.device)
            return fail(MMW_ERR_ARG, "mmw_round_env: the environment lies on device " + std::to_string(E.device) + ", the handle on device " + std::to_string(core.device));
        MMW_HIP(hipSetDevice(core.device));
        return extras.round_env(E.list_source(), Zr, Dp, gX, nbatch, randv, z_out, rem_out);
    }
    int round_attempts(mmw_env* env, bool with_env, int32_t Zr, int32_t Dp, const double* gX, int32_t nattempt, uint64_t seed, int pick_rule, int32_t* z_out,
                       int32_t* rem_out, int32_t* pick_out, int32_t* z_all) override {
        const std::string who = with_env ? "mmw_round_env_attempts" : "mmw_round_attempts";
        MMW_TRY(Extras<T>::attempts_check(who, Zr, Dp, nattempt, pick_rule, z_out, rem_out, pick_out));
        if (core.K > ROUND_PICK_MAX_K) return fail(MMW_ERR_ARG, who + ": K = " + std::to_string(core.K) + " exceeds " + std::to_string(ROUND_PICK_MAX_K) + ", the most users the pick's key holds");
        if (core.host_only) return host_only_handle();
        if (!with_env) {
            MMW_HIP(hipSetDevice(core.device));
            return extras.round_attempts(Zr, Dp, gX, nattempt, seed, pick_rule, z_out, rem_out, pick_out, z_all);
        }
        if (!env) return fail(MMW_ERR_ARG, who + ": null environment");
        const EnvDevice& E = env->e;
        if (E.K != core.K)
            return fail(MMW_ERR_ARG, who + ": the environment has K = " + std::to_string(E.K) + " stations, the handle K = " + std::to_string(core.K));
        if (E.device != core.device)
            return fail(MMW_ERR_ARG, who + ": the environment lies on device " + std::to_string(E.device) + ", the handle on device " + std::to_string(core.device));
        MMW_HIP(hipSetDevice(core.device));
        return extras.round_env_attempts(E.list_source(), Zr, Dp, gX, nattempt, seed, pick_rule, z_out, rem_out, pick_out, z_all);
    }
    int round_randv(int32_t Zr, int32_t Dp, uint64_t seed, int32_t attempt, double* out, int64_t n) override {
        if (Zr < 1 || Dp < 1) return fail(MMW_ERR_ARG, "mmw_round_randv: Z and D' must be positive");
        if (attempt < 0) return fail(MMW_ERR_ARG, "mmw_round_randv: attempt must be >= 0");
        if (!out || n != (int64_t)Zr * Dp) return fail(MMW_ERR_ARG, "mmw_round_randv: out must hold Z x D' values");
        if (core.host_only) return host_only_handle();
        MMW_HIP(hipSetDevice(core.device));
        return extras.round_randv(Zr, Dp, seed, attempt, out);
    }
};
template <typename T>
int expm_apply_impl(const Switches& sw, int device, int method, int max_order, double tol, int32_t K, int32_t D, const int32_t* indptr,
                    const int32_t* indices, const double* data, const double* B, double* out, double info[4], int32_t reps,
                    double* kernel_us) {
    MMW_HIP(hipSetDevice(device));
    hipStream_t st;
    MMW_HIP(hipStreamCreateWithFlags(&st, hipStreamNonBlocking));
    ScopedStream guard{st};
    const int64_t nnz = indptr[K];
    std::vector<int32_t> ip(indptr, indptr + K + 1), ci(indices, indices + nnz);
    std::vector<double> vv(data, data + nnz);
    DevBuf<int> d_ip, d_ci;
    DevBuf<T> d_v, d_out;
    DevBuf<double> d_b64, d_o64;
    MMW_TRY(d_ip.upload(ip, st));
    MMW_TRY(d_ci.upload(ci, st));
    MMW_TRY(d_v.upload_cast(vv, st));
    ExpmEngine<T> eng(sw);
    MMW_TRY(eng.init(st, K, D, d_ip.p, d_ci.p, d_v.p));
    eng.method = method; eng.max_order = max_order; eng.tol = tol;
    MMW_TRY(d_out.alloc(eng.bs));
    MMW_TRY(d_b64.alloc((size_t)K * D));
    MMW_TRY(d_o64.alloc((size_t)K * D));
    MMW_TRY(copy_h2d(d_b64.p, B, (size_t)K * D * sizeof(double), st));
    hipEvent_t e0, e1;
    MMW_HIP(hipEventCreate(&e0));
    MMW_HIP(hipEventCreate(&e1));
    double us = 0.0;
    if (reps < 1) reps = 1;
    for (int r = 0; r < reps; ++r) {
        hipLaunchKernelGGL((k_import_block<T>), dim3(grid_elems(eng.bs)), dim3(BLOCK), 0, st, K, D, eng.lay.Dpad, d_b64.p, eng.start_block());
        MMW_HIP(hipEventRecord(e0, st));
        int rc = eng.apply(d_out.p, 1.0);
        if (rc != MMW_OK) return rc;
        MMW_HIP(hipEventRecord(e1, st));
        MMW_HIP(hipStreamSynchronize(st));
        float ms = 0;
        MMW_HIP(hipEventElapsedTime(&ms, e0, e1));
        us += ms * 1e3;
    }
    (void)hipEventDestroy(e0);
    (void)hipEventDestroy(e1);
    hipLaunchKernelGGL((k_export_block<T>), dim3(grid_elems((size_t)K * D)), dim3(BLOCK), 0, st, K, D, eng.lay.Dpad, d_out.p, d_o64.p);
    MMW_HIP(hipGetLastError());
    MMW_TRY(copy_d2h(out, d_o64.p, (size_t)K * D * sizeof(double), st));
    if (info) {
        info[0] = eng.last.rho; info[1] = eng.last.m_eff > 0 ? eng.last.m_eff : eng.last.m; info[2] = eng.last.nsub; info[3] = eng.last.mu;
    }
    if (kernel_us) *kernel_us = us / reps;
    return MMW_OK;
}
template <typename Init> int create_solver(mmw_solver** out, int dtype, bool host_only, Init&& init) {
    auto make = [&](auto s) {
        s->core.host_only = host_only;
        const int rc = init(*s);
        if (rc == MMW_OK) *out = s.release();
        return rc;
    };
    if (dtype == MMW_F32) return make(std::make_unique<Solver<float>>(Switches::from_env()));
    if (dtype == MMW_F64) return make(std::make_unique<Solver<double>>(Switches::from_env()));
    return fail(MMW_ERR_ARG, "dtype must be MMW_F32 or MMW_F64");
}
}
```

sig_sdp_mmw_amd/csrc/solver_create.h:

```cpp
#pragma once
#include "csr_device.h"
#include "solver_loop.h"
#include "solver_read.h"
#include "solver_replay.h"

namespace {
template <typename T> struct Solver;
struct DeviceLists {
    DevBuf<int> st_ptr, st_idx, gain_x, gain_y, asso_x, asso_y, gu_ptr, qu_ptr, so_ptr;
    DevBuf<double> st_val, s_sum, sq_sum;
    bool host_done = true;
    template <typename T> int ensure_host(SolverCore<T>& co) {
        if (host_done) return MMW_OK;
        MMW_HIP(hipSetDevice(co.device));
        const size_t nst = (size_t)co.H.n_st, ng = (size_t)co.H.n_gain, na = (size_t)co.H.n_asso;
        co.H.st_indices.resize(nst); co.H.st_data.resize(nst);
        co.H.gain_x.resize(ng); co.H.gain_y.resize(ng); co.H.asso_x.resize(na); co.H.asso_y.resize(na);
        co.H.diag_pos.resize(co.K); co.H.asso_pos.resize(na);
        MMW_TRY(copy_d2h(co.H.st_indices.data(), st_idx.p, nst * sizeof(int32_t), co.st));
        MMW_TRY(copy_d2h(co.H.st_data.data(), st_val.p, nst * sizeof(double), co.st));
        MMW_TRY(copy_d2h(co.H.gain_x.data(), gain_x.p, ng * sizeof(int32_t), co.st));
        MMW_TRY(copy_d2h(co.H.gain_y.data(), gain_y.p, ng * sizeof(int32_t), co.st));
        MMW_TRY(copy_d2h(co.H.asso_x.data(), asso_x.p, na * sizeof(int32_t), co.st));
        MMW_TRY(copy_d2h(co.H.asso_y.data(), asso_y.p, na * sizeof(int32_t), co.st));
// ... 36 lines not shown
        static std::atomic<bool> module_loading{false};
        std::thread warm_thread;
        if (!co.host_only && !module_loading.exchange(true))
            warm_thread = std::thread([dev]() {
                if (hipSetDevice(dev) != hipSuccess) return;
                float* p = nullptr;
                if (hipMalloc((void**)&p, 256 * sizeof(float)) != hipSuccess) return;
                hipLaunchKernelGGL((k_fill<float>), dim3(1), dim3(BLOCK), 0, (hipStream_t) nullptr, (size_t)256, p, 0.0f);
                (void)hipDeviceSynchronize();
                (void)hipFree(p);
            });
        struct Joiner { std::thread& t; ~Joiner() { if (t.joinable()) t.join(); } } joiner{warm_thread};
        co.bt.want_mfma(K_, Z_ * rr, co.sw);
        const bool start_blk = !co.host_only && !co.sw.no_blocking;
        double t_struct = 0.0;
        std::string err = build_pattern(co.H, K_, Z_, Sp, Si, Sx, Qp, Qi, Qx, h, [&]() {
            t_struct = tnow();
            if (start_blk) co.bt.build_thread = std::thread([pc = &co]() { pc->bt.host_blockings(pc->H, pc->sw); });
        });
        if (!err.empty()) co.bt.join();
        const double t_1 = tnow();
        if (!err.empty()) return fail(MMW_ERR_ARG, "mmw_create: " + err);
        co.K = K_; co.Z = Z_; co.rank_radio = rr; co.eta = eta_; co.nit = nit_;
        co.D = co.Z * co.rank_radio;
        if (co.host_only) {
            std::string lerr;
            if (make_layout(co.D, V16<T>::N, co.eng.lay, lerr) != MMW_OK) return fail(MMW_ERR_ARG, lerr);
            if (live_switch(LIVE_HOST_BLOCKING)) {
                report_host_blocking(co.bt.HB, co.H, co.K, blocking_limits<T>(), co.sw);
            }
            if (co.sw.check_blocking) {
                const BlockingLimits lim = blocking_limits<T>();
                if (co.bt.HB.order.empty()) build_blocking(co.bt.HB, co.K, co.H.l_indptr, co.H.l_indices, lim);
                build_sd_tables(co.bt.HB, co.K, co.H.l_indptr, co.H.l_indices);
                if (!co.bt.HB.order.empty() && !co.bt.HB.blk_rowptr.empty() && co.bt.HB.blk_rowptr.back() == co.K) {
                    const std::string berr = verify_blocking(co.bt.HB, co.K, co.H.l_indptr, co.H.l_indices, lim);
                    if (!berr.empty()) return fail(MMW_ERR_STATE, "blocking invariant violated: " + berr);
                    for (int mrows : {64, 32, 7}) {
                        build_mfma_blocking(co.bt.HB, co.K, co.H.l_indptr, co.H.l_indices, mrows, co.sw.mf_union_cap);
                        const std::string merr = verify_mfma_blocking(co.bt.HB, co.K, co.H.l_indptr, co.H.l_indices);
                        if (!merr.empty()) return fail(MMW_ERR_STATE, "blocking invariant violated: " + merr);
                    }
                }
            }
            return MMW_OK;
        }
        MMW_HIP(hipSetDevice(co.device));
        MMW_HIP(hipStreamCreateWithFlags(&co.st, hipStreamNonBlocking));
        MMW_TRY(co.d_indptr.upload(co.H.l_indptr, co.st));
        MMW_TRY(co.d_col.upload(co.H.l_indices, co.st));
        MMW_TRY(co.d_pid.upload(co.H.pid, co.st));
        MMW_TRY(co.d_mirror.upload(co.H.mirror, co.st));
        MMW_TRY(co.d_diag.upload(co.H.diag_pos, co.st));
        MMW_TRY(co.d_apos.upload(co.H.asso_pos, co.st));
        {
            std::vector<int32_t> lrow((size_t)co.H.nnzL());
            for (int k = 0; k < co.K; ++k)
                for (int e = co.H.l_indptr[k]; e < co.H.l_indptr[k + 1]; ++e) lrow[e] = k;
            MMW_TRY(co.d_lrow.upload(lrow, co.st));
        }
        MMW_TRY(co.d_sab.upload_cast(co.H.sab, co.st));
        MMW_TRY(co.d_sba.upload_cast(co.H.sba, co.st));
        MMW_TRY(co.upload_row_vectors());
        return init_common(s, t_0, t_1, t_struct, nullptr);
    }
    static int init_env(Solver<T>& s, int dev, EnvDevice& E, int32_t Z_, int32_t rr, double eta_, int32_t nit_) {
        SolverCore<T>& co = s.core;
        DeviceLists& envl = s.envl;
        co.device = dev;
        const double t_0 = tnow();
        if (Z_ < 2) return fail(MMW_ERR_ARG, "mmw_create_from_env: Z must be >= 2 (the constraints divide by Z-1)");
        if (E.K < 2) return fail(MMW_ERR_ARG, "mmw_create_from_env: K must be >= 2");
        MMW_HIP(hipSetDevice(co.device));
        MMW_HIP(hipStreamCreateWithFlags(&co.st, hipStreamNonBlocking));
        MMW_TRY(E.pattern_inputs());
        co.K = E.K; co.Z = Z_; co.rank_radio = rr; co.eta = eta_; co.nit = nit_;
        co.D = co.Z * co.rank_radio;
        co.H.K = co.K; co.H.Z = co.Z;
        const int A = E.A;
        const int32_t* c6 = E.h_cnt6.data();
        std::vector<int32_t> st_ptr(co.K + 1, 0), gu_ptr(co.K + 1, 0), qu_ptr(co.K + 1, 0), so_ptr(co.K + 1, 0);
        co.H.l_indptr.assign(co.K + 1, 0);
        for (int k = 0; k < co.K; ++k) {
            co.H.l_indptr[k + 1] = co.H.l_indptr[k] + c6[k];
            st_ptr[k + 1] = st_ptr[k] + c6[(size_t)co.K + k];
            gu_ptr[k + 1] = gu_ptr[k] + c6[(size_t)2 * co.K + k];
            qu_ptr[k + 1] = qu_ptr[k] + c6[(size_t)3 * co.K + k];
            so_ptr[k + 1] = so_ptr[k] + (E.h_sptr[k + 1] - E.h_sptr[k]) - c6[(size_t)4 * co.K + k];
            if ((int64_t)co.H.l_indptr[k] + c6[k] > (int64_t)INT32_MAX) return fail(MMW_ERR_ARG, "mmw_create_from_env: pattern too large for int32 indexing");
        }
        const size_t nnz = (size_t)co.H.l_indptr[co.K], nst = (size_t)st_ptr[co.K], ng = (size_t)gu_ptr[co.K], na = (size_t)qu_ptr[co.K];
        co.H.n_st = (int64_t)nst; co.H.n_gain = (int64_t)ng; co.H.n_asso = (int64_t)na;
        co.H.st_indptr = st_ptr;
        MMW_TRY(co.d_indptr.upload(co.H.l_indptr, co.st));
        MMW_TRY(envl.st_ptr.upload(st_ptr, co.st)); MMW_TRY(envl.gu_ptr.upload(gu_ptr, co.st)); MMW_TRY(envl.qu_ptr.upload(qu_ptr, co.st)); MMW_TRY(envl.so_ptr.upload(so_ptr, co.st));
        MMW_TRY(co.d_col.alloc(nnz)); MMW_TRY(co.d_lrow.alloc(nnz)); MMW_TRY(co.d_sab.alloc(nnz)); MMW_TRY(co.d_sba.alloc(nnz)); MMW_TRY(co.d_pid.alloc(nnz)); MMW_TRY(co.d_mirror.alloc(nnz));
        MMW_TRY(co.d_diag.alloc(co.K)); MMW_TRY(co.d_apos.alloc(na));
        MMW_TRY(envl.st_idx.alloc(nst)); MMW_TRY(envl.st_val.alloc(nst));
        MMW_TRY(envl.gain_x.alloc(ng)); MMW_TRY(envl.gain_y.alloc(ng)); MMW_TRY(envl.asso_x.alloc(na)); MMW_TRY(envl.asso_y.alloc(na));
        MMW_TRY(envl.s_sum.alloc(co.K)); MMW_TRY(envl.sq_sum.alloc(co.K));
        PatOut<T> O;
        O.l_ptr = co.d_indptr.p; O.st_ptr = envl.st_ptr.p; O.gu_ptr = envl.gu_ptr.p; O.qu_ptr = envl.qu_ptr.p; O.appos = E.appos.p;
        O.l_idx = co.d_col.p; O.lrow = co.d_lrow.p; O.sab = co.d_sab.p; O.sba = co.d_sba.p; O.pid = co.d_pid.p; O.diag_pos = co.d_diag.p;
        O.st_idx = envl.st_idx.p; O.st_val = envl.st_val.p;
        O.gain_x = envl.gain_x.p; O.gain_y = envl.gain_y.p; O.asso_x = envl.asso_x.p; O.asso_y = envl.asso_y.p; O.asso_pos = co.d_apos.p;
        hipLaunchKernelGGL((k_pat_fill<T>), dim3(grid_rows(co.K)), dim3(BLOCK), 0, co.st, co.K, A, E.P.thr, E.rx.p, E.rxT.p, E.asso.p, O);
        MMW_HIP(hipGetLastError());
        co.H.l_indices.resize(nnz);
        MMW_TRY(copy_d2h(co.H.l_indices.data(), co.d_col.p, nnz * sizeof(int32_t), co.st));
        const double t_struct = tnow();
        co.bt.want_mfma(co.K, Z_ * rr, co.sw);
        if (!co.sw.no_blocking) {
            if (!co.sw.env_rcm) {
                co.bt.HB.rcm_cache = spatial_order(co.K, E.h_sta, 64);
                co.bt.HB.grow = false;
            }
            co.bt.build_thread = std::thread([pc = &co]() { pc->bt.host_blockings(pc->H, pc->sw); });
        }
        hipLaunchKernelGGL(k_pat_mirror, dim3(grid_elems(nnz)), dim3(BLOCK), 0, co.st, nnz, co.d_indptr.p, co.d_col.p, co.d_lrow.p, co.d_mirror.p);
        hipLaunchKernelGGL(k_pat_rowstats, dim3(grid_elems((size_t)co.K)), dim3(BLOCK), 0, co.st, co.K, envl.st_ptr.p, envl.st_val.p, envl.s_sum.p, envl.sq_sum.p);
        MMW_HIP(hipGetLastError());
        co.H.S_sum.resize(co.K); co.H.sq_sum.resize(co.K); co.H.h_max.resize(co.K);
        MMW_TRY(copy_d2h(co.H.S_sum.data(), envl.s_sum.p, (size_t)co.K * sizeof(double), co.st));
        MMW_TRY(copy_d2h(co.H.sq_sum.data(), envl.sq_sum.p, (size_t)co.K * sizeof(double), co.st));
        MMW_TRY(copy_d2h(co.H.h_max.data(), E.h_max.p, (size_t)co.K * sizeof(double), co.st));
        co.H.norm_H.assign(co.K, 0.0);
        co.H.cH.assign(co.K, 0.0);
        {
            const std::string err = update_slots(co.H, co.Z);
            if (!err.empty()) {
                co.bt.join();
                return fail(MMW_ERR_ARG, "mmw_create_from_env: " + err);
            }
        }
        MMW_TRY(co.upload_row_vectors());
        envl.host_done = false;
        const double t_1 = tnow();
        RoundSource R;
        R.q_ptr = E.q_ptr.p; R.q_idx = E.q_idx.p; R.nnzQ = E.nnzQ; R.h_max = E.h_max.p;
        R.s_ptr = E.s_ptr.p; R.s_idx = E.s_idx.p; R.s_val = E.s_val.p;
        return init_common(s, t_0, t_1, t_struct, &R);
    }
    static int init_csr(Solver<T>& s, CsrDevice& Cs, int32_t Z_, int32_t rr, double eta_, int32_t nit_) {
        const char* who = "mmw_create_from_csr";
        SolverCore<T>& co = s.core;
        DeviceLists& dl = s.envl;
        const CsrView V = Cs.V;
        const int K = V.K;
        if (co.host_only) {
            MMW_TRY(Cs.validate(who));
            return init(s, -1, K, Z_, rr, eta_, nit_, V.Sp, V.Si, V.Sx, V.Qp, V.Qi, V.Qx, V.h);
        }
        co.device = Cs.device;
        const double t_0 = tnow();
        MMW_HIP(hipSetDevice(co.device));
        MMW_HIP(hipStreamCreateWithFlags(&co.st, hipStreamNonBlocking));
        const int gk = grid_rows(K);
        const size_t Ks = (size_t)K;
        if (Cs.checked) MMW_TRY(Cs.verdict(who));
        else MMW_TRY(Cs.enqueue_checks(co.st));
        DevBuf<int> cnt, nfnew;
        MMW_TRY(cnt.alloc(4 * Ks)); MMW_TRY(nfnew.alloc(Ks));
        MMW_HIP(hipMemsetAsync(cnt.p, 0, 4 * Ks * sizeof(int), co.st));
        hipLaunchKernelGGL(k_csrpat_count, dim3(gk), dim3(BLOCK), 0, co.st, V, (const unsigned long long*)Cs.d_err.p, cnt.p, cnt.p + Ks, cnt.p + 2 * Ks, cnt.p + 3 * Ks);
        MMW_HIP(hipGetLastError());
        if (!Cs.checked) {
            MMW_TRY(copy_d2h(Cs.err, Cs.d_err.p, sizeof Cs.err, co.st));
            Cs.checked = true;
            MMW_TRY(Cs.verdict(who));
        }
        if (K < 2) return fail(MMW_ERR_ARG, std::string(who) + ": K must be >= 2");
        if (Z_ < 2) return fail(MMW_ERR_ARG, std::string(who) + ": Z must be >= 2 (the constraints divide by Z-1)");
        std::vector<int32_t> h_cnt(4 * Ks);
        MMW_TRY(copy_d2h(h_cnt.data(), cnt.p, h_cnt.size() * sizeof(int32_t), co.st));
        std::vector<int32_t> so_ptr(Ks + 1, 0), f_ptr(Ks + 1, 0), st_ptr(Ks + 1, 0), qu_ptr(Ks + 1, 0), gu_ptr(Ks + 1, 0);
        for (size_t k = 0; k < Ks; ++k) {
            so_ptr[k + 1] = so_ptr[k] + h_cnt[k];
            f_ptr[k + 1] = f_ptr[k] + h_cnt[Ks + k];
            st_ptr[k + 1] = st_ptr[k] + h_cnt[2 * Ks + k];
            qu_ptr[k + 1] = qu_ptr[k] + h_cnt[3 * Ks + k];
        }
        const size_t nso = (size_t)so_ptr[K], nst = (size_t)st_ptr[K], na = (size_t)qu_ptr[K];
        if ((size_t)f_ptr[K] != nst) return fail(MMW_ERR_STATE, std::string(who) + ": internal: the transpose lost entries");
        DevBuf<int> d_fptr, f_idx, fx, tmp_idx;
        DevBuf<double> f_val, tmp_val;
        Extras<T>& ex = s.extras;
        MMW_TRY(dl.so_ptr.upload(so_ptr, co.st)); MMW_TRY(d_fptr.upload(f_ptr, co.st)); MMW_TRY(dl.st_ptr.upload(st_ptr, co.st)); MMW_TRY(dl.qu_ptr.upload(qu_ptr, co.st));
        MMW_TRY(ex.so_indices.alloc(nso)); MMW_TRY(ex.so_data.alloc(nso)); MMW_TRY(ex.so_hmax.alloc(nso));
        MMW_TRY(f_idx.alloc(nst)); MMW_TRY(f_val.alloc(nst)); MMW_TRY(fx.alloc(nst)); MMW_TRY(tmp_idx.alloc(nst)); MMW_TRY(tmp_val.alloc(nst));
        MMW_TRY(dl.st_idx.alloc(nst)); MMW_TRY(dl.st_val.alloc(nst)); MMW_TRY(dl.s_sum.alloc(Ks)); MMW_TRY(dl.sq_sum.alloc(Ks));
        int* cursor = cnt.p + 2 * Ks;
        MMW_HIP(hipMemsetAsync(cursor, 0, Ks * sizeof(int), co.st));
        hipLaunchKernelGGL(k_csrpat_fill, dim3(gk), dim3(BLOCK), 0, co.st, V, (const int*)dl.so_ptr.p, (const int*)d_fptr.p, (const int*)dl.st_ptr.p, cursor, ex.so_indices.p,
                           ex.so_data.p, ex.so_hmax.p, f_idx.p, f_val.p, tmp_idx.p, tmp_val.p);
        hipLaunchKernelGGL(k_csrpat_sort_rows, dim3(gk), dim3(BLOCK), 0, co.st, K, (const int*)dl.st_ptr.p, (const int*)tmp_idx.p, (const double*)tmp_val.p, dl.st_idx.p, dl.st_val.p);
        hipLaunchKernelGGL(k_pat_rowstats, dim3(grid_elems(Ks)), dim3(BLOCK), 0, co.st, K, dl.st_ptr.p, dl.st_val.p, dl.s_sum.p, dl.sq_sum.p);
        hipLaunchKernelGGL(k_csrpat_count_L, dim3(gk), dim3(BLOCK), 0, co.st, V, (const int*)dl.st_ptr.p, (const int*)dl.st_idx.p, (const int*)d_fptr.p, (const int*)f_idx.p, fx.p,
                           nfnew.p, cnt.p, cnt.p + Ks);
        MMW_HIP(hipGetLastError());
        co.K = K; co.Z = Z_; co.rank_radio = rr; co.eta = eta_; co.nit = nit_;
        co.D = co.Z * co.rank_radio;
        co.H.K = K; co.H.Z = Z_;
        co.H.S_sum.resize(Ks); co.H.sq_sum.resize(Ks); co.H.h_max.resize(Ks);
        MMW_TRY(copy_d2h(co.H.S_sum.data(), dl.s_sum.p, Ks * sizeof(double), co.st));
        MMW_TRY(copy_d2h(co.H.sq_sum.data(), dl.sq_sum.p, Ks * sizeof(double), co.st));
        MMW_TRY(copy_d2h(co.H.h_max.data(), V.h, Ks * sizeof(double), co.st));
        MMW_TRY(copy_d2h(h_cnt.data(), cnt.p, 2 * Ks * sizeof(int32_t), co.st));
        co.H.norm_H.assign(Ks, 0.0);
        co.H.cH.assign(Ks, 0.0);
        co.H.n_st = (int64_t)nst; co.H.n_asso = (int64_t)na;
        co.H.st_indptr = st_ptr;
        {
            const std::string err = update_slots(co.H, co.Z);
            if (!err.empty()) return fail(MMW_ERR_ARG, std::string(who) + ": " + err);
        }
        co.H.l_indptr.assign(Ks + 1, 0);
        for (size_t k = 0; k < Ks; ++k) {
            if ((int64_t)co.H.l_indptr[k] + h_cnt[k] > (int64_t)INT32_MAX) return fail(MMW_ERR_ARG, std::string(who) + ": pattern too large for int32 indexing");
            co.H.l_indptr[k + 1] = co.H.l_indptr[k] + h_cnt[k];
            gu_ptr[k + 1] = gu_ptr[k] + h_cnt[Ks + k];
        }
        const size_t nnz = (size_t)co.H.l_indptr[K], ng = (size_t)gu_ptr[K];
        co.H.n_gain = (int64_t)ng;
        MMW_TRY(co.d_indptr.upload(co.H.l_indptr, co.st)); MMW_TRY(dl.gu_ptr.upload(gu_ptr, co.st));
        MMW_TRY(co.d_col.alloc(nnz)); MMW_TRY(co.d_lrow.alloc(nnz)); MMW_TRY(co.d_sab.alloc(nnz)); MMW_TRY(co.d_sba.alloc(nnz)); MMW_TRY(co.d_pid.alloc(nnz)); MMW_TRY(co.d_mirror.alloc(nnz));
        MMW_TRY(co.d_diag.alloc(Ks)); MMW_TRY(co.d_apos.alloc(na));
        MMW_TRY(dl.gain_x.alloc(ng)); MMW_TRY(dl.gain_y.alloc(ng)); MMW_TRY(dl.asso_x.alloc(na)); MMW_TRY(dl.asso_y.alloc(na));
        DevBuf<int> internal;
        MMW_TRY(internal.alloc(1));
        MMW_HIP(hipMemsetAsync(internal.p, 0, sizeof(int), co.st));
        CsrPatOut<T> O;
        O.l_ptr = co.d_indptr.p; O.st_ptr = dl.st_ptr.p; O.f_ptr = d_fptr.p; O.qu_ptr = dl.qu_ptr.p;
        O.st_idx = dl.st_idx.p; O.st_val = dl.st_val.p; O.f_idx = f_idx.p; O.f_val = f_val.p; O.fx = fx.p; O.n_fnew = nfnew.p;
        O.l_idx = co.d_col.p; O.lrow = co.d_lrow.p; O.sab = co.d_sab.p; O.sba = co.d_sba.p; O.pid = co.d_pid.p; O.diag_pos = co.d_diag.p;
        O.asso_x = dl.asso_x.p; O.asso_y = dl.asso_y.p; O.asso_pos = co.d_apos.p; O.internal = internal.p;
        hipLaunchKernelGGL((k_csrpat_fill_L<T>), dim3(gk), dim3(BLOCK), 0, co.st, V, O);
        MMW_HIP(hipGetLastError());
        co.H.l_indices.resize(nnz);
        MMW_TRY(copy_d2h(co.H.l_indices.data(), co.d_col.p, nnz * sizeof(int32_t), co.st));
        const double t_struct = tnow();
        co.bt.want_mfma(K, Z_ * rr, co.sw);
        if (!co.sw.no_blocking) co.bt.build_thread = std::thread([pc = &co]() { pc->bt.host_blockings(pc->H, pc->sw); });
        hipLaunchKernelGGL(k_csrpat_gain_edges, dim3(gk), dim3(BLOCK), 0, co.st, K, (const int*)co.d_indptr.p, (const int*)co.d_col.p, (const int*)co.d_pid.p, (const int*)dl.gu_ptr.p,
                           dl.gain_x.p, dl.gain_y.p);
        hipLaunchKernelGGL(k_pat_mirror, dim3(grid_elems(nnz)), dim3(BLOCK), 0, co.st, nnz, co.d_indptr.p, co.d_col.p, co.d_lrow.p, co.d_mirror.p);
        MMW_HIP(hipGetLastError());
        int h_internal = 0;
        MMW_TRY(copy_d2h(&h_internal, internal.p, sizeof(int), co.st));
        if (h_internal) {
            co.bt.join();
            return fail(MMW_ERR_ARG, std::string(who) + ": internal: gain edge on an association pair");
        }
        MMW_TRY(co.upload_row_vectors());
        dl.host_done = false;
        const double t_1 = tnow();
        RoundSource R;
        R.q_ptr = V.Qp; R.q_idx = V.Qi; R.nnzQ = V.nnzQ; R.h_max = V.h; R.so_filled = true;
        return init_common(s, t_0, t_1, t_struct, &R);
    }
    static int init_extras_device(SolverCore<T>& co, DeviceLists& envl, Extras<T>& extras, const RoundSource& R) {
        MMW_TRY(extras.init_device(co.st, co.K, &co.kt));
        std::vector<int32_t> so_ptr_h((size_t)co.K + 1);
        MMW_TRY(copy_d2h(so_ptr_h.data(), envl.so_ptr.p, so_ptr_h.size() * sizeof(int32_t), co.st));
        const size_t nso = (size_t)so_ptr_h[co.K];
        MMW_TRY(extras.so_indptr.upload(so_ptr_h, co.st));
        MMW_TRY(extras.q_indptr.alloc((size_t)co.K + 1)); MMW_TRY(extras.q_indices.alloc((size_t)R.nnzQ)); MMW_TRY(extras.h_max.alloc(co.K));
        if (!R.so_filled) {
            MMW_TRY(extras.so_indices.alloc(nso)); MMW_TRY(extras.so_data.alloc(nso)); MMW_TRY(extras.so_hmax.alloc(nso));
            hipLaunchKernelGGL(k_pat_so_fill, dim3(grid_rows(co.K)), dim3(BLOCK), 0, co.st, co.K, R.s_ptr, R.s_idx, R.s_val, (const int*)extras.so_indptr.p, R.h_max,
                               extras.so_indices.p, extras.so_data.p, extras.so_hmax.p);
            MMW_HIP(hipGetLastError());
        }
        MMW_HIP(hipMemcpyAsync(extras.q_indptr.p, R.q_ptr, ((size_t)co.K + 1) * sizeof(int), hipMemcpyDeviceToDevice, co.st));
        if (R.nnzQ) MMW_HIP(hipMemcpyAsync(extras.q_indices.p, R.q_idx, (size_t)R.nnzQ * sizeof(int), hipMemcpyDeviceToDevice, co.st));
        MMW_HIP(hipMemcpyAsync(extras.h_max.p, R.h_max, (size_t)co.K * sizeof(double), hipMemcpyDeviceToDevice, co.st));
        MMW_HIP(hipStreamSynchronize(co.st));
        return MMW_OK;
    }
    static int init_common(Solver<T>& s, double t_0, double t_1, double t_struct, const RoundSource* round_src) {
        SolverCore<T>& co = s.core;
        const bool verbose = live_switch(LIVE_VERBOSE);
        MMW_TRY(co.alloc_iterate());
        MMW_TRY(s.loop.alloc_scratch(co));
        MMW_TRY(co.eng.init(co.st, co.K, co.D, co.d_indptr.p, co.d_col.p, co.lval.p));
        co.kt.st = co.st;
        co.eng.kt = &co.kt;
        co.eng.max_order = 12;
        co.eng.tol = sizeof(T) == 4 ? 1e-6 : 1e-9;
        MMW_TRY(co.Xh.alloc(co.eng.bs));
        MMW_TRY(prealloc(co, s.pending, s.loop, s.extras));
        const double t_2 = tnow();
        MMW_TRY(setup_blocking(co, s.loop, s.extras));
        const double t_3 = tnow();
        if (verbose) fprintf(stderr, "[create] pattern %.1f ms (structure after %.1f), uploads+alloc %.1f ms, blocking %.1f ms\n", (t_1 - t_0) * 1e3, (t_struct - t_0) * 1e3, (t_2 - t_1) * 1e3, (t_3 - t_2) * 1e3);
        MMW_TRY(s.reads.resize(co));
        MMW_TRY(s.loop.resize(co));
        MMW_HIP(hipStreamSynchronize(co.st));
        if (round_src) MMW_TRY(init_extras_device(co, s.envl, s.extras, *round_src));
        else MMW_TRY(s.extras.init(co.st, &co.H, co.K, &co.kt));
        return s.reset(co.nit);
    }
    static int prealloc(SolverCore<T>& co, PendingChunk<T>& pending, SolverLoop<T>& loop, Extras<T>& extras) {
        const size_t nnz = (size_t)co.H.nnzL(), C = (size_t)co.H.C();
        for (DevBuf<T>* b : {&pending.sn_lval, &pending.sn_xval, &pending.sn_xavg}) MMW_TRY(b->alloc(nnz));
        for (DevBuf<T>* b : {&pending.sn_Y, &pending.sn_yavg, &pending.sn_eaccu, &loop.yun}) MMW_TRY(b->alloc(C));
        MMW_TRY(pending.sn_plan.alloc(1));
        if ((double)co.eng.bs * sizeof(T) * 4.0 < 8.0e9) MMW_TRY(co.eng.ensure_blocks(std::min(4, co.eng.max_order + 1)));
        if (co.bt.blk_want_mf && (co.eng.lay.Dpad % 32) == 0) {
            MMW_TRY(loop.xh_planes.alloc(2 * co.eng.bs));
            MMW_TRY(co.eng.reserve_planes());
        }
        const int rank = std::min(co.K - 1, (co.Z - 1) * co.rank_radio);
        if (rank >= 1) {
            MMW_TRY(extras.fac_reserve(co.st, co.K, rank, co.bt.blk_want_mf));
            if ((size_t)10 * co.K * co.Z * sizeof(double) <= ((size_t)2 << 30)) MMW_TRY(extras.round_reserve(co.K, co.Z, rank, 10));
        }
        return MMW_OK;
    }
    static int setup_blocking(SolverCore<T>& co, SolverLoop<T>& loop, Extras<T>& extras) {
        if (co.sw.no_blocking) return MMW_OK;
        if (co.bt.build_thread.joinable()) co.bt.build_thread.join();
        else co.bt.host_blockings(co.H, co.sw);
        if (co.bt.blk_want_mf && live_switch(LIVE_VERBOSE))
            fprintf(stderr, "[mmw] matrix-core blocking: ok %d blocks %d rows/block %.1f reuse %.2f row tiles %d k-steps %d\n", (int)co.bt.HB.fits_mfma, co.bt.HB.nbm(),
                    (double)co.K / std::max(1, co.bt.HB.nbm()), co.bt.HB.m_reuse, co.bt.HB.mfma_mt, co.bt.HB.kbase.empty() ? 0 : co.bt.HB.kbase.back());
        if (live_switch(LIVE_VERBOSE))
            fprintf(stderr, "[mmw] blocking: usable %d half-tile %d blocks %d rows/block %.1f union/block %.1f entries %lld (nnz %lld, +%.1f%% padding) sd_max %d\n",
                    (int)co.bt.HB.usable, (int)co.bt.HB.fits_half_tile, co.bt.HB.nb(), (double)co.K / std::max(1, co.bt.HB.nb()), (double)co.bt.HB.un_cols.size() / std::max(1, co.bt.HB.nb()),
                    (long long)co.bt.HB.nent, (long long)co.H.nnzL(), 100.0 * ((double)co.bt.HB.nent / (double)co.H.nnzL() - 1.0), co.bt.HB.sd_max);
        if (!co.bt.HB.usable) return MMW_OK;
        MMW_TRY(co.bt.upload(co.st, co.H, co.K, co.sw, co.d_apos.p));
        if (sizeof(T) == 4 && co.bt.HB.fits_mfma) {
            co.eng.use_mfma = true;
            co.eng.mf.nb = co.bt.HB.nbm();
            co.eng.mf.desc = co.bt.b_mdesc.p;
            co.eng.mf.un_fixed = co.bt.b_munfixed.p;
            co.eng.mf.order = co.bt.b_morder.p;
            co.eng.mf.kbase = co.bt.b_kbase.p;
            co.eng.mf.afrag = co.bt.afrag.p;
            co.eng.mf_mt = co.bt.HB.mfma_mt;
            if (co.bt.sddmm_mfma) {
                MMW_TRY(co.x.xs_val.alloc(co.bt.n_xs));
                MMW_TRY(co.x.xs_avg.alloc(co.bt.n_xs));
                MMW_TRY(loop.rsfx.alloc((size_t)2 * co.K));
            }
            if ((size_t)co.bt.HB.nbm() > (size_t)MAX_PART && co.bt.HB.nbm() > co.bt.HB.nb()) {
                MMW_TRY(co.eng.partial.alloc((size_t)co.bt.HB.nbm() * co.eng.lay.Dpad));
                MMW_TRY(co.eng.partial_o2.alloc((size_t)co.bt.HB.nbm() * co.eng.lay.Dpad));
            }
        }
        if (!co.bt.sddmm_mfma) MMW_TRY(co.bt.ensure_sd(co.st, co.H, co.K, co.eng.lay.Dpad, co.sw.full_tile));
        MMW_HIP(hipStreamSynchronize(co.st));
        extras.fac.set_blocking(co.blkdev(), co.bt.b_bepos.p, co.bt.HB.nent);
        if (co.eng.use_mfma) extras.fac.set_mfma(co.eng.mf, co.bt.HB.mfma_mt, co.bt.b_fpos.p, co.bt.afrag_n, (int64_t)co.H.nnzL());
        co.eng.blk_stale = &co.lblk_stale;
        co.eng.blk_refresh = [pc = &co]() -> int {
            hipLaunchKernelGGL((k_gather_blocked<T>), dim3(grid_elems((size_t)pc->bt.HB.nent)), dim3(BLOCK), 0, pc->st, (size_t)pc->bt.HB.nent, pc->bt.b_bepos.p, pc->lval.p, pc->bt.lval_blk.p);
            MMW_HIP(hipGetLastError());
            return MMW_OK;
        };
        return co.eng.enable_blocking(co.blkdev(), co.bt.lval_blk.p);
    }
};
}
```

sig_sdp_mmw_amd/csrc/solver_loop.h:

```cpp
#pragma once
#include "solver_core.h"
#include "solver_gap.h"

namespace {
struct SketchCarry {
    int64_t done_for = -1;
    uint64_t done_seed = 0;
    int slabs = 0;
    uint64_t last_seed = 0;
    bool last_was_rng = false;
    template <typename Run> bool drawn(const Run& c, int iter) const { return !c.randv && done_for == (int64_t)iter && done_seed == c.seed; }
    void note(int64_t iter, uint64_t seed, int nslabs) { done_for = iter; done_seed = seed; slabs = nslabs; }
    void forget() { done_for = -1; }
    void used(uint64_t seed) { forget(); last_was_rng = true; last_seed = seed; }
    void uploaded() { last_was_rng = false; }
};
template <typename T> struct SolverLoop {
    using Core = SolverCore<T>;
    explicit SolverLoop(const Switches& sw)
        : dual_gap(std::isnan(sw.dual_gap) ? (sizeof(T) == 4 ? 60.0 : 600.0) : sw.dual_gap), fv_measure(!sw.fv_worstcase), rs_enabled(!sw.no_sddmm_rowsums) {}
    ChunkPolicy pol;
    SketchCarry carry;
    DevBuf<T> rsum, drow;
    DevBuf<double> max_part, sum_part, scal, tr_part, stage64;
    DevBuf<T> wH;
    DevBuf<T> yun;
    const double dual_gap;
    static constexpr int LOSS_GRID_MAX = 4096;
    DevBuf<unsigned short> xh_planes;
    DevBuf<long long> rsfx;
    DevBuf<double> tr1_part;
    const bool fv_measure;
    double plane_rounding() const { return fv_measure ? F16_PLANE_EXPECT : 1.02 * F16_UNIT; }
    bool rs_last = false;
    const bool rs_enabled;
    long long n_rs_iters = 0, n_fused_iters = 0, n_first_iters = 0, n_first16_iters = 0;
    GapPhase<T> gap;
    int alloc_scratch(const Core& co) {
        const int K = co.K;
        MMW_TRY(rsum.alloc(K)); MMW_TRY(drow.alloc(K));
        MMW_TRY(max_part.alloc(ROW_GRID_MAX)); MMW_TRY(sum_part.alloc(4 * (size_t)std::max(2048, ROW_GRID_MAX))); MMW_TRY(scal.alloc(8));
        MMW_TRY(tr_part.alloc(ROW_GRID_MAX)); MMW_TRY(wH.alloc(K));
        return MMW_OK;
    }
    int resize(const Core& co) { return stage64.alloc((size_t)co.K * co.D); }
    void on_restart(bool warm, int iter, int nit) {
        if (warm) pol.on_warm_restart(iter);
        else pol.on_reset();
        if (gap.ever) gap.clear_log(nit);
    }
    int sketch_slabs(const Core& co) const { return std::min(grid_rows(co.K), co.sw.sk_slabs); }
    int launch_sketch(Core& co, hipStream_t s, uint64_t seed, uint32_t it, bool planes_f16 = false) {
        const bool lz = co.eng.method == MMW_EXPM_LANCZOS;
        unsigned short* pl = co.eng.start_planes();
        hipLaunchKernelGGL((k_sketch_rng<T>), dim3(sketch_slabs(co)), dim3(BLOCK), lz ? (size_t)(WAVES_PER_BLOCK + 1) * co.eng.lay.Dpad * sizeof(double) : 0, s, co.K, co.D, co.eng.lay.Dpad,
                           seed, it, co.eng.start_block(), lz ? co.eng.partial_sq.p : (double*)nullptr, pl, planes_f16 ? 1 : 0,
                           planes_f16 && lz && fv_measure ? co.eng.partial_du.p : (double*)nullptr);
        co.eng.planes_ready[0] = pl != nullptr;
        co.eng.planes0_f16 = planes_f16 && pl != nullptr;
        MMW_HIP(hipGetLastError());
        return MMW_OK;
    }
    struct ChunkRun {
        int n; const double* randv; uint64_t seed; bool optimistic;
        bool lanczos;
        bool sd_mf_call;
        PatternDev<T> P;
        const T* xcur;
        int gr, gd, gc, gl, Dpad;
        int m_launch;
        bool lag_chunk, chain, chain_plan, fuse_sketch;
        bool xavg_deferred = false;
        bool rs_ok = false;
        FirstVerify fv_pending;
    };
    struct IterRun {
        int it, acc;
        bool lagged_it = false, fused_dual = false, rs_zeroed = false, first_it = false;
        PlanArgs pa;
        int ntr1 = 0;
    };
    template <int NCH> void launch_sddmm(Core& co, const ChunkRun& c, int acc) {
        hipLaunchKernelGGL((k_sddmm<T, NCH>), dim3(c.gr), dim3(BLOCK), 0, co.st, c.P, c.Dpad, co.eng.lay.LPR, co.eng.lay.G, co.Xh.p, drow.p, tr_part.p, c.gr, co.xval.p, co.xavg.p, acc);
    }
    template <int MT, int NB>
    int launch_sddmm_mfma(Core& co, const ChunkRun& c, dim3 grid, const SdMfmaDev& SM, const double* trp, int ntr, int acc, long long* rs_out, const long long* dfx,
                          unsigned long long* stamps, const FirstVerify& fv) {
        MMW_TRY(set_max_lds(reinterpret_cast<const void*>(&k_sddmm_mfma<MT, NB>), sdm_lds_bytes<MT, NB>()));
        hipLaunchKernelGGL((k_sddmm_mfma<MT, NB>), grid, dim3(256 * MT), (sdm_lds_bytes<MT, NB>()), co.st, co.eng.mf, SM, co.K, c.Dpad,
                           reinterpret_cast<const char*>(xh_planes.p), drow.p, trp, ntr, co.x.xs_val.p, co.x.xs_avg.p, acc, rs_out, dfx, stamps, fv);
        return MMW_OK;
    }
    int iterate_impl(Core& co, int32_t n, const double* randv, uint64_t seed, bool optimistic) {
        ChunkRun c{n, randv, seed, optimistic, co.eng.method == MMW_EXPM_LANCZOS};
        c.sd_mf_call = sizeof(T) == 4 && co.bt.sddmm_mfma && co.eng.use_blk && c.lanczos && (co.eng.lay.Dpad % 32) == 0 && co.bt.b_e2w.p != nullptr;
        if (n > 0) MMW_TRY(c.sd_mf_call ? co.x.to_tiles(co) : co.x.to_csr(co));
        c.P = co.pat();
        c.xcur = co.x.live(co).val->p;
        c.gr = grid_rows(co.K);
        c.gd = std::min(c.gr, 5 * device_cus());
        c.gc = grid_elems((size_t)co.H.C());
        c.gl = (int)std::min<size_t>(((size_t)co.H.nnzL() + BLOCK - 1) / BLOCK, (size_t)LOSS_GRID_MAX);
        c.Dpad = co.eng.lay.Dpad;
        c.m_launch = optimistic ? pol.m_guess : 0;
        c.lag_chunk = optimistic && pol.lagged_ok(co.eng.last, co.sw) && !pol.warm_fresh && !pol.exact_plans_only;
        c.chain = optimistic && pol.chain_ok;
        pol.chain_ok = false;
        c.chain_plan = c.chain && pol.plan_has_room(co.eng.last);
        c.rs_ok = c.chain && rs_last && rs_enabled && rsfx.p != nullptr;
        rs_last = false;
        c.fuse_sketch = !co.kt_exact() && !co.pt.timing && co.sw.fused_sketch;
        carry.forget();
        for (int it = 0; it < n; ++it) {
            IterRun s;
            s.it = it;
            s.acc = (co.iter + 1 < co.nit) ? 1 : 0;
            if (gap.on) MMW_TRY(gap.enqueue_row(co.st, co.H, c.P, co.d_lrow.p, co.x.live(co).avg->p, c.xavg_deferred ? c.xcur : (const T*)nullptr, co.yavg.p, co.iter));
            MMW_TRY(co.pt.record(0, co.iter, co.st));
            MMW_TRY(phase_dual(co, c, s));
            MMW_TRY(phase_loss(co, c, s));
            MMW_TRY(phase_expm(co, c, s));
            MMW_TRY(phase_x(co, c, s));
            ++co.iter;
            if (!optimistic) MMW_TRY(gap.collect(co.st, co.d_indptr.p, co.d_col.p));
        }
        MMW_TRY(chunk_tail(co, c));
        return gap.queue_copy(co.st);
    }
    int phase_dual(Core& co, ChunkRun& c, IterRun& s) {
        MMW_TRY(co.kt.begin(KT_DUAL));
        const long long* rs_it = c.rs_ok ? rsfx.p : nullptr;
        const FirstVerify fv = c.fv_pending;
        c.fv_pending = FirstVerify{};
        if (rs_it) ++n_rs_iters;
        if (!rs_it) hipLaunchKernelGGL((k_dual_rows<T>), dim3(c.gr), dim3(BLOCK), 0, co.st, c.P, c.xcur, rsum.p, co.e_this.p);
        s.lagged_it = c.optimistic && (s.it > 0 || c.chain_plan) && c.lanczos && c.lag_chunk;
        if (s.lagged_it) {
            s.pa.plan = co.eng.plan_d.p; s.pa.part = co.eng.row_part.p; s.pa.viol = co.eng.viol_d.p; s.pa.tol = co.eng.tol; s.pa.K = co.K; s.pa.method = co.eng.method;
            s.pa.max_order = co.eng.max_order; s.pa.np = c.gd; s.pa.m_launch = c.m_launch; s.pa.apost = co.eng.apost() ? 1 : 0; s.pa.iter_seen = pol.age(co.iter) - 1;
        }
        s.fused_dual = c.optimistic && (s.it > 0 || c.chain) && !co.sw.no_fused_dual;
        if (s.fused_dual) {
            ++n_fused_iters;
            if (yun.n < (size_t)co.H.C()) MMW_TRY(yun.alloc((size_t)co.H.C()));
            StampBuf dh_stamps;
            const bool want_dst = s.it + 1 == c.n && live_switch(LIVE_DUAL_STAMPS);
            MMW_TRY(dh_stamps.request(want_dst, (size_t)c.gd * WAVES_PER_BLOCK * 8, co.st));
            hipLaunchKernelGGL((k_dual_h<T>), dim3(c.gd), dim3(BLOCK), 0, co.st, c.P, rsum.p, co.e_this.p, co.e_accu.p, co.eta, max_part.p,
                               (const T*)(s.lagged_it ? co.lval.p : nullptr), 0.5, co.eng.row_part.p, (const double*)(scal.p + 4), yun.p, wH.p, sum_part.p,
                               rs_it, c.xcur, FirstVerify{}, dh_stamps.p());
            if (want_dst) MMW_TRY(dump_dual_stamps(co.st, dh_stamps.p(), c.gd));
            hipLaunchKernelGGL(k_dual_scal, dim3(1 + fv.nwg), dim3(DSCAL_THREADS), 0, co.st, sum_part.p, max_part.p, c.gd, scal.p,
                               dual_gap, co.eng.viol_d.p, fv);
        } else {
            hipLaunchKernelGGL((k_dual_h<T>), dim3(c.gd + fv.nwg), dim3(BLOCK), 0, co.st, c.P, rsum.p, co.e_this.p, co.e_accu.p, co.eta, max_part.p,
                               (const T*)(s.lagged_it ? co.lval.p : nullptr), 0.5, co.eng.row_part.p, (const double*)nullptr, (T*)nullptr, (T*)nullptr,
                               (double*)nullptr, rs_it, c.xcur, fv);
            hipLaunchKernelGGL((k_softmax_a<T>), dim3(c.gc), dim3(BLOCK), 0, co.st, c.P, co.e_accu.p, co.Y.p, max_part.p, c.gd, sum_part.p);
            hipLaunchKernelGGL((k_softmax_b<T>), dim3(c.gc + (s.lagged_it ? 1 : 0)), dim3(BLOCK), 0, co.st, (int)co.H.C(), co.Y.p, co.yavg.p, s.acc, sum_part.p, c.gc, scal.p,
                               co.K + (int)co.H.E_asso(), co.d_invn.p, wH.p, s.pa, max_part.p, c.gd);
        }
        MMW_TRY(co.kt.end());
        MMW_TRY(co.pt.record(1, co.iter, co.st));
        return MMW_OK;
    }
    int phase_loss(Core& co, ChunkRun& c, IterRun& s) {
        MMW_TRY(co.kt.begin(KT_LOSS));
        s.rs_zeroed = rs_enabled && rsfx.p != nullptr && co.bt.sddmm_mfma;
        const bool sketch_have = carry.drawn(c, co.iter);
        s.first_it = c.optimistic && pol.first_guess && c.m_launch == 1 && !c.randv && s.rs_zeroed && sizeof(T) == 4 && co.eng.mfma_now() &&
                              c.lanczos && co.eng.use_blk && (c.Dpad % 32) == 0 && !sketch_have;
        SketchArgs<T> skl{};
        if (!c.randv && !sketch_have && !co.kt_exact() && !co.sw.no_loss_sketch) {
            skl.nblocks = sketch_slabs(co); skl.K = co.K; skl.D = co.D; skl.seed = c.seed; skl.iter = (uint32_t)co.iter;
            skl.R = co.eng.start_block();
            skl.colsq_part = c.lanczos ? co.eng.partial_sq.p : nullptr;
            skl.planes = co.eng.start_planes();
            skl.planes_f16 = s.first_it ? 1 : 0;
            skl.dusq_part = s.first_it && fv_measure ? co.eng.partial_du.p : nullptr;
            co.eng.planes_ready[0] = skl.planes != nullptr;
            co.eng.planes0_f16 = s.first_it && skl.planes != nullptr;
            carry.note((int64_t)co.iter, c.seed, skl.nblocks);
        }
        const bool mf_it = co.eng.mfma_now() && c.lanczos;
        if (mf_it) co.lblk_stale = true;
        const PlanArgs pl_loss = s.fused_dual ? s.pa : PlanArgs{};
        hipLaunchKernelGGL((k_loss<T>), dim3(c.gl + skl.nblocks + (pl_loss.plan ? 1 : 0)), dim3(BLOCK), skl.nblocks && c.lanczos ? (size_t)(WAVES_PER_BLOCK + 1) * c.Dpad * sizeof(double) : 0,
                           co.st, c.P, co.d_lrow.p, s.fused_dual ? yun.p : co.Y.p, wH.p, scal.p, co.lval.p, co.eta,
                           (const int*)(co.eng.use_blk && !mf_it ? co.bt.b_bpos.p : nullptr), co.bt.lval_blk.p,
                           (const T*)(c.xavg_deferred ? co.xval.p : nullptr), c.xavg_deferred ? co.xavg.p : (T*)nullptr, skl, c.Dpad,
                           (const int*)(co.eng.use_mfma ? co.bt.b_fpos.p : nullptr), co.bt.afrag.p, s.fused_dual ? co.Y.p : (T*)nullptr, co.yavg.p, s.acc, pl_loss,
                           s.rs_zeroed ? rsfx.p : (long long*)nullptr, s.rs_zeroed ? (s.first_it ? 2 * co.K : co.K) : 0, s.first_it ? 1 : 0,
                           s.first_it && pol.first_a16_guess ? co.bt.afrag16.p : (unsigned short*)nullptr);
        c.xavg_deferred = false;
        MMW_TRY(co.kt.end());
        MMW_TRY(co.pt.record(2, co.iter, co.st));
        return MMW_OK;
    }
    int phase_expm(Core& co, ChunkRun& c, IterRun& s) {
        const bool sketch_rode = carry.drawn(c, co.iter);
        if (!sketch_rode) MMW_TRY(co.kt.begin(KT_SKETCH));
        if (c.randv) {
            MMW_TRY(copy_h2d(stage64.p, c.randv + (size_t)s.it * co.K * co.D, (size_t)co.K * co.D * sizeof(double), co.st));
            hipLaunchKernelGGL((k_import_block<T>), dim3(grid_elems(co.eng.bs)), dim3(BLOCK), 0, co.st, co.K, co.D, c.Dpad, stage64.p, co.eng.start_block());
            co.eng.planes_ready[0] = false;
            carry.uploaded();
        } else {
            if (!sketch_rode) MMW_TRY(launch_sketch(co, co.st, c.seed, (uint32_t)co.iter, s.first_it));
            co.eng.start_colsq_ready = c.lanczos;
            co.eng.npart_start = sketch_rode ? carry.slabs : sketch_slabs(co);
            carry.used(c.seed);
        }
        if (!sketch_rode) MMW_TRY(co.kt.end());
        MMW_HIP(hipGetLastError());
        co.eng.out_planes = nullptr;
        if constexpr (sizeof(T) == 4) {
            if (c.sd_mf_call) {
                if (xh_planes.n < 2 * co.eng.bs) MMW_TRY(xh_planes.alloc(2 * co.eng.bs));
                co.eng.out_planes = xh_planes.p;
            }
        }
        co.eng.planes_only = co.eng.out_planes != nullptr && c.optimistic && s.it + 1 < c.n && !co.sw.keep_xhalf;
        co.eng.rownorm_d = drow.p;
        co.eng.rownorm_part = tr_part.p;
        co.eng.plan_iter = pol.age(co.iter);
        if (s.first_it) {
            const size_t need = (size_t)co.eng.first_grid_max();
            if (tr1_part.n < need) {
                MMW_TRY(tr1_part.alloc(need));
                MMW_HIP(hipMemsetAsync(tr1_part.p, 0, need * sizeof(double), co.st));
            }
            MMW_TRY(co.eng.apply_first(co.eng.planes_only ? (T*)nullptr : co.Xh.p, 0.5, c.m_launch, s.lagged_it, xh_planes.p, rsfx.p + co.K, tr1_part.p, &s.ntr1,
                                    pol.first_a16_guess ? co.bt.afrag16.p : (const unsigned short*)nullptr));
            ++n_first_iters;
            if (pol.first_a16_guess) ++n_first16_iters;
        } else
            MMW_TRY(co.eng.apply(co.Xh.p, 0.5, c.m_launch, s.lagged_it));
        return MMW_OK;
    }
    int phase_x(Core& co, ChunkRun& c, IterRun& s) {
        MMW_TRY(co.kt.begin(KT_SDDMM));
        if (!c.lanczos)
            hipLaunchKernelGGL((k_rownorm2<T>), dim3(c.gr), dim3(BLOCK), 0, co.st, co.K, c.Dpad, co.Xh.p, drow.p, tr_part.p);
        bool sd_done = false;
        c.rs_ok = false;
        if constexpr (sizeof(T) == 4) {
            if (c.sd_mf_call) {
                const SdMfmaDev SM = co.bt.sd_mfma_dev();
                const long long* dfx = s.first_it ? rsfx.p + co.K : nullptr;
                const double* trp = s.first_it ? tr1_part.p : tr_part.p;
                const int ntr = s.first_it ? s.ntr1 : c.gr;
                FirstVerify fv_now;
                if (s.first_it) {
                    fv_now.plan = co.eng.plan_d.p; fv_now.viol = co.eng.viol_d.p; fv_now.o2 = co.eng.partial_o2.p; fv_now.n_o2 = co.eng.mf.nb;
                    fv_now.u2 = co.eng.partial_sq.p; fv_now.du2 = fv_measure ? co.eng.partial_du.p : nullptr; fv_now.rows = co.K; fv_now.n_u2 = co.eng.npart_start; fv_now.Dpad = c.Dpad;
                    fv_now.nwg = c.Dpad / FV_COLS;
                    fv_now.cA = pol.first_a16_guess ? F16_UNIT : F16_CA_TWO;
                    fv_now.du_scale = co.sw.fv_du_scale;
                }
                const bool fv_rides = s.first_it && co.sw.fv_in_sddmm;
                const dim3 grid((co.bt.HB.nbm() + 7) / 8 * 8 + (fv_rides ? 8 : 0), (co.bt.HB.m_ntile_max + SDM_GT - 1) / SDM_GT);
                long long* rs_out = s.rs_zeroed ? rsfx.p : nullptr;
                StampBuf sdm_stamps;
                const size_t n_st = (size_t)grid.x * grid.y * 16 * 8;
                const bool want_st = s.it + 1 == c.n && live_switch(LIVE_SD_STAMPS);
                MMW_TRY(sdm_stamps.request(want_st, n_st, co.st));
                if (co.bt.HB.mfma_mt == 2) MMW_TRY((launch_sddmm_mfma<2, 2>(co, c, grid, SM, trp, ntr, s.acc, rs_out, dfx, sdm_stamps.p(), fv_rides ? fv_now : FirstVerify{})));
                else MMW_TRY((launch_sddmm_mfma<1, 2>(co, c, grid, SM, trp, ntr, s.acc, rs_out, dfx, sdm_stamps.p(), fv_rides ? fv_now : FirstVerify{})));
                if (want_st) MMW_TRY(dump_sddmm_stamps(co.st, sdm_stamps.p(), n_st, grid, co.bt.HB.mfma_mt));
                sd_done = true;
                if (s.first_it && !fv_rides) c.fv_pending = fv_now;
                c.rs_ok = rs_out != nullptr;
            }
        }
        if (!sd_done && co.eng.use_blk) MMW_TRY(co.bt.ensure_sd(co.st, co.H, co.K, co.eng.lay.Dpad, co.sw.full_tile));
        if (sd_done) {
        } else if (co.bt.sddmm_blk2 && co.eng.use_blk) {
            StampBuf sd_stamps;
            MMW_TRY(sd_stamps.request(s.it + 1 == c.n && live_switch(LIVE_SD_STAMPS), (size_t)16 * 8192, co.st));
            const Sd2Dev S = co.bt.sd2_dev();
            constexpr int CT2 = B2_ROW_BYTES / (int)sizeof(T);
            const int per = (co.bt.sd2_nitems + 7) / 8;
            SketchArgs<T> sk{};
            const size_t sd_lds = std::max((size_t)co.bt.HB.un8_max * B2_ROW_BYTES, std::min((size_t)(SD2_THREADS / WAVE) * c.Dpad * sizeof(double), (size_t)65536));
            if (c.fuse_sketch && !c.randv && s.it + 1 < c.n && (size_t)(SD2_THREADS / WAVE) * c.Dpad * sizeof(double) <= sd_lds) {
                constexpr int VBW = SD2_THREADS / BLOCK;
                sk.nblocks = (sketch_slabs(co) + VBW - 1) / VBW;
                sk.K = co.K; sk.D = co.D; sk.seed = c.seed; sk.iter = (uint32_t)(co.iter + 1);
                sk.R = co.eng.start_block();
                sk.colsq_part = c.lanczos ? co.eng.partial_sq.p : nullptr;
                sk.planes = co.eng.start_planes();
                sk.planes_f16 = 0;
                co.eng.planes_ready[0] = sk.planes != nullptr;
                co.eng.planes0_f16 = false;
                carry.note((int64_t)co.iter + 1, c.seed, sk.nblocks * VBW);
            }
            hipLaunchKernelGGL((k_sddmm_blk2<T>), dim3(per * 8 + sk.nblocks), dim3(SD2_THREADS), sd_lds, co.st, co.blkdev(), S, c.P, c.Dpad,
                               (c.Dpad + CT2 - 1) / CT2, co.Xh.p, drow.p, tr_part.p, c.gr, co.xval.p, co.xavg.p, s.acc, sk, sd_stamps.p());
            if (sd_stamps.p()) MMW_TRY(dump_stamps(co.st, sd_stamps.p()));
        } else if (co.bt.sddmm_blk && co.eng.use_blk) {
            const SdDev S = co.bt.sd_dev();
            constexpr int CT = BLK_TILE_BYTES / (int)sizeof(T);
            const int ntiles = (c.Dpad + CT - 1) / CT;
            const int per = (co.bt.HB.nb() + 7) / 8;
            hipLaunchKernelGGL((k_sddmm_blk<T>), dim3(per * 8), dim3(BLK_THREADS), (size_t)BLK_UNION_ROWS * BLK_TILE_BYTES, co.st, co.blkdev(), S, c.P, c.Dpad,
                               ntiles, co.Xh.p, drow.p, tr_part.p, c.gr, co.xval.p, co.xavg.p, s.acc);
        } else
            switch (co.eng.lay.NCH) {
                case 1: launch_sddmm<1>(co, c, s.acc); break;
                case 2: launch_sddmm<2>(co, c, s.acc); break;
                case 3: launch_sddmm<3>(co, c, s.acc); break;
                default: launch_sddmm<4>(co, c, s.acc); break;
            }
        if (sd_done) {
        } else if (s.acc && s.it + 1 < c.n && !co.kt_exact()) c.xavg_deferred = true;
        else if (s.acc) hipLaunchKernelGGL((k_accumulate<T>), dim3((unsigned)std::min<size_t>(((size_t)co.H.nnzL() + BLOCK - 1) / BLOCK, 4096)), dim3(BLOCK), 0, co.st, (size_t)co.H.nnzL(), co.xval.p, co.xavg.p);
        MMW_TRY(co.kt.end());
        MMW_HIP(hipGetLastError());
        MMW_TRY(co.pt.record(3, co.iter, co.st));
        return MMW_OK;
    }
    int chunk_tail(Core& co, ChunkRun& c) {
        if (c.fv_pending.plan) {
            hipLaunchKernelGGL(k_first_verify, dim3(c.fv_pending.nwg), dim3(BLOCK), 0, co.st, c.fv_pending);
            MMW_HIP(hipGetLastError());
        }
        if (c.optimistic && c.n > 1 && c.lag_chunk && c.lanczos) {
            hipLaunchKernelGGL((k_rowsums<T>), dim3(co.eng.nwide), dim3(BLOCK), 0, co.st, co.K, co.d_indptr.p, co.d_col.p, co.lval.p, 0.5, co.eng.row_part.p);
            hipLaunchKernelGGL(k_plan_verify, dim3(1), dim3(PLAN_THREADS), 0, co.st, co.K, co.eng.row_part.p, co.eng.nwide, co.eng.plan_d.p, co.eng.viol_d.p, pol.age(co.iter) - 1);
            MMW_HIP(hipGetLastError());
        }
        pol.chain_ok = c.optimistic && c.n > 1 && pol.replays == 0 && !co.sw.no_chunk_chain;
        rs_last = c.rs_ok;
        return MMW_OK;
    }
};
}
```

sig_sdp_mmw_amd/csrc/solver_replay.h:

```cpp
#pragma once
#include "solver_core.h"

namespace {
template <typename T> struct PendingChunk {
    DevBuf<T> sn_lval, sn_xval, sn_xavg, sn_Y, sn_yavg, sn_eaccu;
    DevBuf<ExpmPlan> sn_plan;
    bool sn_tiles = false;
    bool live = false;
    int iter0 = 0, n = 0;
    size_t events0 = 0;
    uint64_t seed = 0;
    void begin(int iter0_, int n_, uint64_t seed_, size_t events0_) { live = true; iter0 = iter0_; n = n_; seed = seed_; events0 = events0_; }
    void clear() { live = false; }
    int copy_state(SolverCore<T>& co, bool save) {
        const size_t nnz = (size_t)co.H.nnzL(), C = (size_t)co.H.C();
        if (save) sn_tiles = co.x.tiles;
        else co.x.tiles = sn_tiles;
        const typename XLayout<T>::Pair xl = co.x.live(co);
        DevBuf<T>* snap[6] = {&sn_lval, &sn_xval, &sn_xavg, &sn_Y, &sn_yavg, &sn_eaccu};
        DevBuf<T>* cur[6] = {&co.lval, xl.val, xl.avg, &co.Y, &co.yavg, &co.e_accu};
        const size_t len[6] = {nnz, xl.n, xl.n, C, C, C};
        CopySet<T> cs;
        for (int i = 0; i < 6; ++i) {
            if (snap[i]->n < len[i]) MMW_TRY(snap[i]->alloc(len[i]));
            cs.dst[i] = save ? snap[i]->p : cur[i]->p;
            cs.src[i] = save ? cur[i]->p : snap[i]->p;
            cs.n[i] = len[i];
        }
        if (sn_plan.n < 1) MMW_TRY(sn_plan.alloc(1));
        cs.plan_dst = save ? sn_plan.p : co.eng.plan_d.p;
        cs.plan_src = save ? co.eng.plan_d.p : sn_plan.p;
        hipLaunchKernelGGL((k_copy_state<T>), dim3(256, 6), dim3(BLOCK), 0, co.st, cs);
        MMW_HIP(hipGetLastError());
        if (!save && co.bt.lval_blk.p) co.lblk_stale = true;
        if (!save && co.bt.afrag.p) {
            hipLaunchKernelGGL((k_refrag<T>), dim3(grid_elems(nnz)), dim3(BLOCK), 0, co.st, nnz, co.lval.p, co.bt.b_fpos.p, co.bt.afrag.p);
            MMW_HIP(hipGetLastError());
        }
        return MMW_OK;
    }
    int save(SolverCore<T>& co) { return copy_state(co, true); }
    int restore(SolverCore<T>& co) { return copy_state(co, false); }
};
struct EmaxRecord {
    DevBuf<double> d;
    double h = 0.0;
    int enq_iter = -1, got_iter = -1;
    template <typename T> int enqueue(SolverCore<T>& co) {
        if (co.iter <= 0) return MMW_OK;
        if (!d.p) MMW_TRY(d.alloc(1));
        hipLaunchKernelGGL((k_max_of<T>), dim3(1), dim3(1024), 0, co.st, (size_t)co.H.C(), co.e_this.p, d.p);
        MMW_HIP(hipGetLastError());
        enq_iter = co.iter;
        got_iter = -1;
        return MMW_OK;
    }
    template <typename T> int fetch_at_sync(SolverCore<T>& co) {
        const bool want = enq_iter == co.iter && got_iter != co.iter && d.p != nullptr;
        if (want) MMW_HIP(hipMemcpyAsync(&h, d.p, sizeof(double), hipMemcpyDeviceToHost, co.st));
        MMW_HIP(hipStreamSynchronize(co.st));
        if (want) got_iter = co.iter;
        return MMW_OK;
    }
    void drop() { enq_iter = got_iter = -1; }
    bool value_if_current(int iter, double* out) const {
        if (got_iter != iter || got_iter < 0) return false;
        *out = h;
        return true;
    }
};
}
```

sig_sdp_mmw_amd/csrc/switches.h:

```cpp
#pragma once
#include <cmath>
#include <cstdlib>

namespace mmw {

struct Switches {
    bool no_slice_spmm = false;
    int mf_gt = 0;
    bool no_apost = false;
    bool no_blocking = false;
    bool full_tile = false;
    bool no_mfma = false;
    bool no_mfma_sddmm = false;
    int mf_rows = 64;
    int mf_union_cap = 0;
    bool env_rcm = false;
    bool check_blocking = false;
    bool chol_lds = false;
    bool bj_full = false;
    bool factor_no_ns = false;
    bool factor_no_mfma = false;
    bool factor_full_rr = false;
    bool no_fused_dual = false;
    double dual_gap = NAN;
    bool no_lagged_plan = false;
    bool no_first_order = false;
    bool no_first_a16 = false;
    double fv_du_scale = 1.0;
    bool fv_worstcase = false;
    bool fv_in_sddmm = true;
    bool no_sddmm_rowsums = false;
    bool cautious_replay = true;
    bool sync_plan = false;
    bool no_chunk_chain = false;
    bool fused_sketch = false;
    bool no_loss_sketch = false;
    bool keep_xhalf = false;
    int sk_slabs = 256;
    bool kt_markers = false;

    static Switches from_env() {
        Switches s;
        auto on = [](const char* name) { return getenv(name) != nullptr; };
        auto is0 = [](const char* name) { const char* e = getenv(name); return e && atoi(e) == 0; };
        auto num = [](const char* name, int dflt) { const char* e = getenv(name); return e ? atoi(e) : dflt; };
        auto real = [](const char* name, double dflt) { const char* e = getenv(name); return e ? atof(e) : dflt; };
        s.no_slice_spmm = on("MMW_NO_SLICE_SPMM");
        s.mf_gt = num("MMW_MF_GT", 0);
        s.no_apost = on("MMW_NO_APOST");
        if (const char* e = getenv("MMW_BLOCKING")) s.no_blocking = e[0] == '0';
        s.full_tile = on("MMW_FULL_TILE");
        s.no_mfma = on("MMW_NO_MFMA");
        s.no_mfma_sddmm = on("MMW_NO_MFMA_SDDMM");
        s.mf_rows = num("MMW_MF_ROWS", 64);
        s.mf_union_cap = num("MMW_MF_UNION_CAP", 0);
        s.env_rcm = on("MMW_ENV_RCM");
        s.check_blocking = on("MMW_CHECK_BLOCKING");
        s.chol_lds = on("MMW_CHOL_LDS");
        s.bj_full = on("MMW_BJ_FULL");
        s.factor_no_ns = on("MMW_FACTOR_NO_NS");
        s.factor_no_mfma = on("MMW_FACTOR_NO_MFMA");
        s.factor_full_rr = on("MMW_FACTOR_FULL_RR");
        s.no_fused_dual = on("MMW_NO_FUSED_DUAL");
        s.dual_gap = real("MMW_DUAL_GAP", NAN);
        s.no_lagged_plan = on("MMW_NO_LAGGED_PLAN");
        s.no_first_order = on("MMW_NO_FIRST_ORDER");
        s.no_first_a16 = on("MMW_NO_FIRST_A16");
        s.fv_du_scale = real("MMW_FV_DU_SCALE", 1.0);
        s.fv_worstcase = on("MMW_FV_WORSTCASE");
        s.fv_in_sddmm = !is0("MMW_FV_IN_SDDMM");
        s.no_sddmm_rowsums = on("MMW_NO_SDDMM_ROWSUMS");
        s.cautious_replay = !is0("MMW_CAUTIOUS_REPLAY");
        s.sync_plan = on("MMW_SYNC_PLAN");
        s.no_chunk_chain = on("MMW_NO_CHUNK_CHAIN");
        s.fused_sketch = on("MMW_FUSED_SKETCH");
        s.no_loss_sketch = on("MMW_NO_LOSS_SKETCH");
        s.keep_xhalf = on("MMW_KEEP_XHALF");
        s.sk_slabs = num("MMW_SK_SLABS", 256);
        s.kt_markers = on("MMW_KT_MARKERS");
        return s;
    }
};

enum LiveSwitch {
    LIVE_VERBOSE,
    LIVE_FACTOR_VERBOSE,
    LIVE_STAMPS,
    LIVE_SD_STAMPS,
    LIVE_DUAL_STAMPS,
    LIVE_HOST_BLOCKING,
    LIVE_HOST_BLOCKING_HIST,
    LIVE_BENCH_LANCZOS,
    LIVE_BENCH_FIRST,
    LIVE_DEVBUF_EXACT,
};
inline bool live_switch(LiveSwitch w) {
    static const char* const name[] = {"MMW_VERBOSE",       "MMW_FACTOR_VERBOSE",     "MMW_STAMPS",        "MMW_SD_STAMPS",   "MMW_DUAL_STAMPS",
                                       "MMW_HOST_BLOCKING", "MMW_HOST_BLOCKING_HIST", "MMW_BENCH_LANCZOS", "MMW_BENCH_FIRST", "MMW_DEVBUF_EXACT"};
    return getenv(name[w]) != nullptr;
}

}
```

Before: 6583.

## Queue two optimistic chunks so the host plans ahead of device results

Replaces the single pending optimistic chunk with a two-slot queue. Each slot records its plan and violation flag into pinned memory behind a HIP event, so the host can launch a second chunk before the first one settles when its first-order certificate allows it. Growth estimates now account for staleness by inflating the projected spectral growth over the lagged interval. If the older chunk fails its check, the younger chunk is dropped and its iterations are given back for replay. The emax readback also moves to pinned async copies. This aims to remove host-device sync bubbles between chunks, at the cost of more wasted work when a chunk is discarded and more complex replay logic.

```diff
diff --git a/include/mmw_hip.h b/include/mmw_hip.h
--- a/include/mmw_hip.h
+++ b/include/mmw_hip.h
@@ -52,6 +52,7 @@
     MMW_F_SPECTRAL_INFO = 28,
     MMW_F_SPECTRAL_EIG = 29,
     MMW_F_GAP_INFO = 30,
+    MMW_F_CHUNK_INFO = 31,
     MMW_F_KERNEL_US = 15
 };
 enum mmw_ifield {
diff --git a/sig_sdp_mmw_amd/_lib.py b/sig_sdp_mmw_amd/_lib.py
--- a/sig_sdp_mmw_amd/_lib.py
+++ b/sig_sdp_mmw_amd/_lib.py
@@ -23,6 +23,7 @@
 SOLVER_F_SPECTRAL_INFO = 28
 SOLVER_F_SPECTRAL_EIG = 29
 SOLVER_F_GAP_INFO = 30
+SOLVER_F_CHUNK_INFO = 31
 BATCH_MAX_PARTS = 32
 BATCH_MAX_ROW_PARTS = 64
 BATCH_MAX_HEAD_PARTS = 64
diff --git a/sig_sdp_mmw_amd/csrc/chunk_policy.h b/sig_sdp_mmw_amd/csrc/chunk_policy.h
--- a/sig_sdp_mmw_amd/csrc/chunk_policy.h
+++ b/sig_sdp_mmw_amd/csrc/chunk_policy.h
@@ -35,30 +35,35 @@
         if (age_last >= 0 && age(iter) > age_last) { rho_prev = rho_last; age_prev = age_last; }
         rho_last = p.rho; age_last = age(iter);
     }
-    double growth_ratio(int iter, int ahead) const {
+    double growth_ratio(int iter, int ahead, int stale = 0) const {
         double r = (double)(age(iter) + ahead + 1) / (double)std::max(age(iter), 1);
         if (age_prev >= 0 && age_last > age_prev && rho_last > 0.0 && rho_last > rho_prev) {
             const double slope = (rho_last - rho_prev) / (double)(age_last - age_prev);
-            r = std::max(r, (rho_last + 1.5 * slope * (double)(ahead + 1)) / rho_last);
+            const double over = stale > 0 ? 1.5 * slope * (double)stale + 2.25 * slope * (double)(ahead - stale + 1) : 1.5 * slope * (double)(ahead + 1);
+            r = std::max(r, (rho_last + over) / rho_last);
+        } else if (stale > 0) {
+            r = std::max(r, 1.0 + (1.5 * (double)stale + 2.25 * (double)(ahead - stale + 1)) / (double)std::max(age(iter), 1));
         }
         return r;
     }
-    bool first_order_ok(const ExpmPlan& p, const Switches& sw, int iter, int ahead, bool fp32, double plane_rounding, bool a16 = false) const {
+    double growth_to_now(int iter, int stale) const { return stale > 0 ? growth_ratio(iter, stale - 1) : 1.0; }
+    bool first_order_ok(const ExpmPlan& p, const Switches& sw, int iter, int ahead, bool fp32, double plane_rounding, bool a16 = false, int stale = 0) const {
         if (sw.no_first_order || !fp32 || !p.apost || p.m_eff != 1 || p.first_est == 0u) return false;
-        const double est = plan_estimate(p.first_est);
-        const double g1 = growth_ratio(iter, ahead), absn_g = p.absn * g1;
+        const double gn = growth_to_now(iter, stale);
+        const double est = plan_estimate(p.first_est) * gn * gn;
+        const double g1 = growth_ratio(iter, ahead, stale), absn_g = p.absn * g1;
         if (!(absn_g < 0.03)) return false;
         if (a16 ? !((F16_PLANE_EXPECT + F16_UNIT) * absn_g <= p.tol) : !(F16_PLANE_EXPECT * absn_g <= p.tol)) return false;
         const double rounding = std::exp(p.rho * g1) * (absn_g * (plane_rounding + (a16 ? F16_UNIT : F16_CA_TWO)) + F16_SUBNORMAL_ROW);
-        return est <= p.tol / 4.0 && est * g1 * g1 + rounding <= 0.9 * p.tol;
+        return est <= p.tol / 4.0 && plan_estimate(p.first_est) * g1 * g1 + rounding <= 0.9 * p.tol;
     }
-    int next_launch_order(const ExpmPlan& p, int max_order, int iter, int ahead = 0) const {
+    int next_launch_order(const ExpmPlan& p, int max_order, int iter, int ahead = 0, int stale = 0) const {
         if (p.m_eff <= 0) return std::min(max_order, p.m + 1);
         int spare = 1;
         if (p.apost && p.m_eff >= 1 && p.m_eff <= MAX_ORDER) {
             const double est = plan_estimate(p.conv[p.m_eff]);
-            const double grow = std::pow(growth_ratio(iter, ahead), 2.0 * p.m_eff);
-            if (est <= p.tol / 8.0 && est * grow <= p.tol / 2.0) spare = 0;
+            const double grow = std::pow(growth_ratio(iter, ahead, stale), 2.0 * p.m_eff);
+            if (est * std::pow(growth_to_now(iter, stale), 2.0 * p.m_eff) <= p.tol / 8.0 && est * grow <= p.tol / 2.0) spare = 0;
         }
         if (p.m_eff >= p.m_apriori) spare = 0;
         return std::min(max_order, p.m_eff + spare);
@@ -73,23 +78,31 @@
         return c > 32.0 ? 32 : (c < 0.0 ? 0 : (int)c);
     }
     bool plan_has_room(const ExpmPlan& p) const { return p.apost && p.m_eff == 1 && plan_estimate(p.conv[1]) <= p.tol / 8.0; }
+    bool may_run_ahead(const ExpmPlan& last, const Switches& sw, bool carried, bool instrumented) const {
+        return sw.chunk_depth >= 2 && chain_ok && replays == 0 && plan_seen && !warm_fresh && !exact_plans_only && !carried && !instrumented && room_ahead(last);
+    }
+    bool room_ahead(const ExpmPlan& p) const {
+        if (plan_has_room(p)) return true;
+        return p.apost && p.m_eff == 1 && p.first_est != 0u && plan_estimate(p.first_est) <= p.tol / 8.0 && plan_estimate(p.conv[1]) <= p.tol;
+    }
     bool lagged_ok(const ExpmPlan& p, const Switches& sw) const {
         if (sw.no_lagged_plan || lagged_missed || !p.apost || p.m_eff != 1) return false;
         return plan_estimate(p.conv[1]) <= p.tol / 2.0;
     }
-    int chunk_length(const ExpmPlan& p, const Switches& sw, int iter, int left) const {
+    int chunk_length(const ExpmPlan& p, const Switches& sw, int iter, int left, int stale = 0) const {
         int cap = lagged_ok(p, sw) ? std::max(8, std::min(32, age(iter))) : std::max(4, std::min(32, age(iter) / 2));
-        if (chain_ok && age(iter) >= 4) cap = std::max(cap, std::min(32, room_iterations(p, iter)));
+        if (chain_ok && age(iter) >= 4) cap = std::max(cap, std::min(32, room_iterations(p, iter - stale) - stale));
         if (warm_fresh) cap = 8;
         int chunk = std::min(left, cap);
         if (left - chunk == 1) ++chunk;
         return chunk;
     }
-    void plan_chunk(const ExpmPlan& p, const Switches& sw, int max_order, int iter, int chunk, bool fp32, bool have_a16, double plane_rounding) {
-        if (plan_seen) m_guess = next_launch_order(p, max_order, iter, chunk);
-        first_guess = plan_seen && first_order_ok(p, sw, iter, chunk, fp32, plane_rounding);
+    void plan_chunk(const ExpmPlan& p, const Switches& sw, int max_order, int iter, int chunk, bool fp32, bool have_a16, double plane_rounding, int stale = 0) {
+        const int at = iter - stale, ahead = stale + chunk;
+        if (plan_seen) m_guess = next_launch_order(p, max_order, at, ahead, stale);
+        first_guess = plan_seen && first_order_ok(p, sw, at, ahead, fp32, plane_rounding, false, stale);
         if (first_guess) m_guess = 1;
-        first_a16_guess = first_guess && !sw.no_first_a16 && have_a16 && first_order_ok(p, sw, iter, chunk, fp32, plane_rounding, true);
+        first_a16_guess = first_guess && !sw.no_first_a16 && have_a16 && first_order_ok(p, sw, at, ahead, fp32, plane_rounding, true, stale);
         if (warm_fresh) {
             m_guess = std::min(max_order, std::max(2, p.m_eff + 1));
             first_guess = false;
diff --git a/sig_sdp_mmw_amd/csrc/expm_engine.h b/sig_sdp_mmw_amd/csrc/expm_engine.h
--- a/sig_sdp_mmw_amd/csrc/expm_engine.h
+++ b/sig_sdp_mmw_amd/csrc/expm_engine.h
@@ -255,7 +255,7 @@
         MMW_TRY(reset_plan_history(false));
         MMW_TRY(viol_d.alloc(1));
         MMW_HIP(hipMemsetAsync(viol_d.p, 0, sizeof(int), st));
-        if (!plan_h) MMW_HIP(hipHostMalloc((void**)&plan_h, sizeof(ExpmPlan)));
+        if (!plan_h) MMW_HIP(hipHostMalloc((void**)&plan_h, sizeof(ExpmPlan) + sizeof(int)));
         if (use_blk) MMW_TRY(enable_blocking(blk, val_blk));
         return MMW_OK;
     }
@@ -391,18 +391,22 @@
         return MMW_OK;
     }
     int fetch_plan(int* violated) {
-        int v = 0;
+        int* viol_h = reinterpret_cast<int*>(plan_h + 1);
         MMW_HIP(hipMemcpyAsync(plan_h, plan_d.p, sizeof(ExpmPlan), hipMemcpyDeviceToHost, st));
-        MMW_HIP(hipMemcpyAsync(&v, viol_d.p, sizeof(int), hipMemcpyDeviceToHost, st));
+        MMW_HIP(hipMemcpyAsync(viol_h, viol_d.p, sizeof(int), hipMemcpyDeviceToHost, st));
         MMW_HIP(hipStreamSynchronize(st));
-        last = *plan_h;
+        take_plan(*plan_h, *viol_h);
+        if (violated) *violated = *viol_h;
+        return MMW_OK;
+    }
+    void take_plan(const ExpmPlan& p, int v) {
+        last = p;
         last_mfma_ok = last.mfma_ok != 0;
         if (live_switch(LIVE_VERBOSE)) {
-            fprintf(stderr, "[plan] rho %.3e absn %.3e mfma_ok %d tol %.1e m %d (a-priori %d) apost %d m_eff %d est[1] %.3e est[2] %.3e viol %d\n", last.rho,
-                    last.absn, last.mfma_ok, last.tol, last.m, last.m_apriori, last.apost, last.m_eff, plan_estimate(last.conv[1]), plan_estimate(last.conv[2]), v);
-        }
-        if (violated) *violated = v;
-        return MMW_OK;
+            fprintf(stderr, "[plan] rho %.3e absn %.3e mfma_ok %d tol %.1e m %d (a-priori %d) apost %d m_eff %d est[1] %.3e est[2] %.3e first_est %.3e viol %d\n", last.rho,
+                    last.absn, last.mfma_ok, last.tol, last.m, last.m_apriori, last.apost, last.m_eff, plan_estimate(last.conv[1]), plan_estimate(last.conv[2]),
+                    plan_estimate(last.first_est), v);
+        }
     }
     int clear_violation() {
         MMW_HIP(hipMemsetAsync(viol_d.p, 0, sizeof(int), st));
diff --git a/sig_sdp_mmw_amd/csrc/solver.h b/sig_sdp_mmw_amd/csrc/solver.h
--- a/sig_sdp_mmw_amd/csrc/solver.h
+++ b/sig_sdp_mmw_amd/csrc/solver.h
@@ -61,6 +61,7 @@
         core.bt.join();
         if (core.host_only) return;
         (void)hipSetDevice(core.device);
+        if (core.st) (void)hipStreamSynchronize(core.st);
         if (core.st) (void)hipStreamDestroy(core.st);
     }
     using Create = SolverCreate<T>;
@@ -147,102 +148,146 @@
     int reset(int32_t nit_) override {
         if (core.host_only) return host_only_pattern();
         MMW_HIP(hipSetDevice(core.device));
+        MMW_TRY(settle());
         MMW_TRY(on_restart(nit_, false));
         return core.initial_point();
     }
-    int restore_pending() {
+    using Slot = typename PendingChunk<T>::Slot;
+    int restore_pending(Slot& c) {
         loop.pol.on_discard();
         emax.drop();
         MMW_TRY(core.eng.clear_violation());
-        MMW_TRY(pending.restore(core));
+        MMW_TRY(pending.restore(core, c));
         loop.gap.drop_pending();
-        core.iter = pending.iter0;
-        return core.pt.drop_since(pending.events0, core.st);
-    }
-    void say_replay(int viol, const char* how) const {
+        core.iter = c.iter0;
+        return core.pt.drop_since(c.events0, core.st);
+    }
+    void say_replay(const Slot& c, int viol, const char* how) const {
         if (!live_switch(LIVE_VERBOSE)) return;
         const ExpmPlan& p = core.eng.last;
         const ChunkPolicy& pol = loop.pol;
         fprintf(stderr, "[replay] iterations %d..%d (Z %d) %s: reason bits %d (1 order, 2 lagged plan, 4 plan, 8 softmax, 16 operands, 32 first-order certificate); launched m %d, first-order %d, one-half %d; "
                         "plan m %d m_eff %d apriori %d rho %.3g absn %.3g est %.2e first_est %.2e tol %.1e\n",
-                pending.iter0, pending.iter0 + pending.n - 1, (int)core.H.Z, how, viol, pol.m_guess, (int)pol.first_guess, (int)pol.first_a16_guess, p.m, p.m_eff, p.m_apriori, p.rho, p.absn,
+                c.iter0, c.iter0 + c.n - 1, (int)core.H.Z, how, viol, pol.m_guess, (int)pol.first_guess, (int)pol.first_a16_guess, p.m, p.m_eff, p.m_apriori, p.rho, p.absn,
                 plan_estimate(p.conv[std::max(0, std::min(p.m_eff, MAX_ORDER))]), plan_estimate(p.first_est), p.tol);
     }
-    void accept_plan() {
+    void accept_plan(int at) {
         ChunkPolicy& pol = loop.pol;
         pol.plan_seen = true;
-        pol.note_plan(core.eng.last, core.iter);
-        pol.m_guess = pol.next_launch_order(core.eng.last, core.eng.max_order, core.iter);
-    }
+        pol.note_plan(core.eng.last, at);
+        pol.m_guess = pol.next_launch_order(core.eng.last, core.eng.max_order, at);
+    }
+    bool instrumented() const { return loop.gap.on || core.pt.timing || core.kt.on; }
     int settle() {
-        MMW_TRY(settle_chunk());
+        int giveback = 0;
+        MMW_TRY(settle_pending(giveback));
+        if (giveback) {
+            MMW_TRY(run_chunks(giveback, pending.dropped_seed));
+            giveback = 0;
+            MMW_TRY(settle_pending(giveback));
+        }
         return loop.gap.collect(core.st, core.d_indptr.p, core.d_col.p);
     }
-    int settle_chunk() {
-        if (!pending.live) return MMW_OK;
-        pending.clear();
+    int settle_pending(int& giveback) {
+        while (pending.count() > 0) MMW_TRY(settle_chunk(giveback));
+        return MMW_OK;
+    }
+    int settle_chunk(int& giveback) {
+        if (pending.count() == 0) return MMW_OK;
+        Slot& c = pending.pop();
         ChunkPolicy& pol = loop.pol;
         ExpmEngine<T>& eng = core.eng;
-        int viol = 0;
-        MMW_TRY(eng.fetch_plan(&viol));
+        MMW_HIP(hipEventSynchronize(c.ev));
+        int viol = c.record().viol;
+        eng.take_plan(c.record().plan, viol);
         if (!viol) {
-            accept_plan();
+            accept_plan(c.iter0 + c.n);
             return MMW_OK;
         }
         ++pol.replays;
+        if (pending.count() > 0) giveback += pending.drop_youngest();
+        pol.m_guess = c.m_guess; pol.first_guess = c.first_guess; pol.first_a16_guess = c.first_a16_guess;
         const bool operands_only = (viol & VIOL_OPERANDS) && !pol.first_guess;
         if (viol & VIOL_LAGGED) pol.lagged_missed = true;
-        say_replay(viol, "discarded");
-        MMW_TRY(restore_pending());
-        if (core.sw.cautious_replay && !operands_only && eng.method == MMW_EXPM_LANCZOS && pending.n > 1) {
+        say_replay(c, viol, "discarded");
+        MMW_TRY(restore_pending(c));
+        if (core.sw.cautious_replay && !operands_only && eng.method == MMW_EXPM_LANCZOS && c.n > 1) {
             pol.plan_cautious(eng.last, eng.max_order);
             pol.exact_plans_only = true;
-            const int rc = loop.iterate_impl(core, pending.n, nullptr, pending.seed, true);
+            const int rc = loop.iterate_impl(core, c.n, nullptr, c.seed, true);
             pol.exact_plans_only = false;
             MMW_TRY(rc);
             viol = 0;
             MMW_TRY(eng.fetch_plan(&viol));
             if (!viol) {
-                accept_plan();
-                say_replay(0, "cautious attempt accepted");
+                accept_plan(core.iter);
+                say_replay(c, 0, "cautious attempt accepted");
                 return MMW_OK;
             }
             ++pol.replays;
-            say_replay(viol, "cautious attempt discarded");
-            MMW_TRY(restore_pending());
-        }
-        say_replay(0, "replayed synchronously");
-        return loop.iterate_impl(core, pending.n, nullptr, pending.seed, false);
-    }
-    int iterate(int32_t n, const double* randv, uint64_t seed) override {
-        if (core.host_only) return host_only_pattern();
-        MMW_HIP(hipSetDevice(core.device));
-        if (n < 0) return fail(MMW_ERR_ARG, "n must be >= 0");
-        MMW_TRY(settle());
-        if (core.iter + n > core.nit) return fail(MMW_ERR_STATE, "mmw_iterate: more iterations than announced to mmw_create/mmw_reset");
+            say_replay(c, viol, "cautious attempt discarded");
+            MMW_TRY(restore_pending(c));
+        }
+        say_replay(c, 0, "replayed synchronously");
+        return loop.iterate_impl(core, c.n, nullptr, c.seed, false);
+    }
+    int run_chunks(int left, uint64_t seed) {
         ChunkPolicy& pol = loop.pol;
-        const bool optimistic = randv == nullptr && n > 1 && !core.kt_exact() && !core.sw.sync_plan;
-        if (!optimistic) {
-            pol.chain_ok = false;
-            MMW_TRY(loop.iterate_impl(core, n, randv, seed, false));
-            carried.drop();
-            return emax.enqueue(core);
-        }
-        int left = n;
         while (left > 0) {
-            MMW_TRY(settle());
-            const ExpmPlan& hist = carried.or_last(core.eng.last);
-            const int chunk = pol.chunk_length(hist, core.sw, core.iter, left);
-            pol.plan_chunk(hist, core.sw, core.eng.max_order, core.iter, chunk, sizeof(T) == 4, core.bt.afrag16.p != nullptr, loop.plane_rounding());
-            MMW_TRY(pending.save(core));
+            int giveback = 0;
+            if (pending.count() == 2) MMW_TRY(settle_chunk(giveback));
+            left += giveback;
+            giveback = 0;
+            auto plan_next = [&](int stale) {
+                const ExpmPlan& hist = carried.or_last(core.eng.last);
+                const int len = pol.chunk_length(hist, core.sw, core.iter, left, stale);
+                pol.plan_chunk(hist, core.sw, core.eng.max_order, core.iter, len, sizeof(T) == 4, core.bt.afrag16.p != nullptr, loop.plane_rounding(), stale);
+                return len;
+            };
+            bool ahead = pending.count() == 1 && left > 1 && pol.may_run_ahead(core.eng.last, core.sw, carried.live, instrumented());
+            int chunk = 0;
+            if (ahead) {
+                chunk = plan_next(pending.oldest().n);
+                ahead = loop.first_order_throughout(core);
+            }
+            if (!ahead) {
+                MMW_TRY(settle_pending(giveback));
+                MMW_TRY(loop.gap.collect(core.st, core.d_indptr.p, core.d_col.p));
+                left += giveback;
+                chunk = plan_next(0);
+            }
+            if (live_switch(LIVE_VERBOSE))
+                fprintf(stderr, "[chunk] iterations %d..%d%s: m %d, first-order %d, one-half %d\n", core.iter, core.iter + chunk - 1,
+                        ahead ? " (enqueued ahead)" : "", pol.m_guess, (int)pol.first_guess, (int)pol.first_a16_guess);
+            Slot& sl = pending.free_slot();
+            MMW_TRY(pending.save(core, sl));
             const int iter0 = core.iter;
             const size_t events0 = core.pt.mark();
             MMW_TRY(loop.iterate_impl(core, chunk, nullptr, seed, chunk > 1));
             pol.warm_fresh = false;
             carried.drop();
-            if (chunk > 1) pending.begin(iter0, chunk, seed, events0);
+            if (chunk > 1) {
+                pending.begin(sl, iter0, chunk, seed, events0, ahead, pol);
+                MMW_TRY(pending.queue_record(core, sl));
+            }
             left -= chunk;
         }
+        return MMW_OK;
+    }
+    int iterate(int32_t n, const double* randv, uint64_t seed) override {
+        if (core.host_only) return host_only_pattern();
+        MMW_HIP(hipSetDevice(core.device));
+        if (n < 0) return fail(MMW_ERR_ARG, "n must be >= 0");
+        MMW_TRY(settle());
+        if (core.iter + n > core.nit) return fail(MMW_ERR_STATE, "mmw_iterate: more iterations than announced to mmw_create/mmw_reset");
+        const bool optimistic = randv == nullptr && n > 1 && !core.kt_exact() && !core.sw.sync_plan;
+        if (!optimistic) {
+            loop.pol.chain_ok = false;
+            MMW_TRY(loop.iterate_impl(core, n, randv, seed, false));
+            carried.drop();
+            return emax.enqueue(core);
+        }
+        MMW_TRY(run_chunks(n, seed));
         return emax.enqueue(core);
     }
     CarryInfo carry_info() override { return CarryInfo{core.host_only, core.device, sizeof(T) == 4 ? MMW_F32 : MMW_F64, core.K, core.iter}; }
@@ -271,8 +316,12 @@
     int sync() override {
         if (core.host_only) return host_only_pattern();
         MMW_HIP(hipSetDevice(core.device));
-        MMW_TRY(settle());
-        MMW_TRY(emax.fetch_at_sync(core));
+        MMW_TRY(emax.queue_copy(core));
+        MMW_HIP(hipStreamSynchronize(core.st));
+        const int replays0 = loop.pol.replays;
+        MMW_TRY(settle());
+        emax.landed(core.iter);
+        if (loop.pol.replays != replays0) MMW_HIP(hipStreamSynchronize(core.st));
         MMW_TRY(core.kt.flush());
         return core.pt.flush(core.iter, core.st);
     }
@@ -296,6 +345,8 @@
         MMW_TRY(sync());
         if (which == MMW_F_ST_DATA) MMW_TRY(envl.ensure_host(core));
         if (hv) return export_vec(*hv, out, n, "mmw_read_f64");
+        if (which == MMW_F_CHUNK_INFO)
+            return SolverReads<T>::export_vals({(double)pending.n_enqueued, (double)pending.n_ahead, (double)pending.n_dropped, (double)pending.n_rider}, out, n, "chunk info has 4 entries");
         if (which == MMW_F_LAPLACIAN) return extras.read_laplacian(core.d_indptr.p, core.d_col.p, core.d_diag.p, (size_t)H.nnzL(), out, n);
         return reads.read_f64(core, loop, emax, extras, which, out, n);
     }
diff --git a/sig_sdp_mmw_amd/csrc/solver_create.h b/sig_sdp_mmw_amd/csrc/solver_create.h
--- a/sig_sdp_mmw_amd/csrc/solver_create.h
+++ b/sig_sdp_mmw_amd/csrc/solver_create.h
@@ -362,9 +362,14 @@
     }
     static int prealloc(SolverCore<T>& co, PendingChunk<T>& pending, SolverLoop<T>& loop, Extras<T>& extras) {
         const size_t nnz = (size_t)co.H.nnzL(), C = (size_t)co.H.C();
-        for (DevBuf<T>* b : {&pending.sn_lval, &pending.sn_xval, &pending.sn_xavg}) MMW_TRY(b->alloc(nnz));
-        for (DevBuf<T>* b : {&pending.sn_Y, &pending.sn_yavg, &pending.sn_eaccu, &loop.yun}) MMW_TRY(b->alloc(C));
-        MMW_TRY(pending.sn_plan.alloc(1));
+        for (int i = 0; i < (co.sw.chunk_depth >= 2 ? 2 : 1); ++i) {
+            typename PendingChunk<T>::Slot& sl = pending.slot[i];
+            for (DevBuf<T>* b : {&sl.sn_lval, &sl.sn_xval, &sl.sn_xavg}) MMW_TRY(b->alloc(nnz));
+            for (DevBuf<T>* b : {&sl.sn_Y, &sl.sn_yavg, &sl.sn_eaccu}) MMW_TRY(b->alloc(C));
+            MMW_TRY(sl.sn_plan.alloc(1));
+            MMW_TRY(sl.rec.ensure(sizeof(typename PendingChunk<T>::Record)));
+        }
+        MMW_TRY(loop.yun.alloc(C));
         if ((double)co.eng.bs * sizeof(T) * 4.0 < 8.0e9) MMW_TRY(co.eng.ensure_blocks(std::min(4, co.eng.max_order + 1)));
         if (co.bt.blk_want_mf && (co.eng.lay.Dpad % 32) == 0) {
             MMW_TRY(loop.xh_planes.alloc(2 * co.eng.bs));
diff --git a/sig_sdp_mmw_amd/csrc/solver_loop.h b/sig_sdp_mmw_amd/csrc/solver_loop.h
--- a/sig_sdp_mmw_amd/csrc/solver_loop.h
+++ b/sig_sdp_mmw_amd/csrc/solver_loop.h
@@ -49,6 +49,11 @@
         else pol.on_reset();
         if (gap.ever) gap.clear_log(nit);
     }
+    bool rs_zeroes(const Core& co) const { return rs_enabled && rsfx.p != nullptr && co.bt.sddmm_mfma; }
+    bool first_order_chunk(const Core& co) const {
+        return pol.first_guess && rs_zeroes(co) && sizeof(T) == 4 && co.eng.mfma_now() && co.eng.method == MMW_EXPM_LANCZOS && co.eng.use_blk && (co.eng.lay.Dpad % 32) == 0;
+    }
+    bool first_order_throughout(const Core& co) const { return pol.m_guess == 1 && first_order_chunk(co) && !co.sw.fused_sketch; }
     int sketch_slabs(const Core& co) const { return std::min(grid_rows(co.K), co.sw.sk_slabs); }
     int launch_sketch(Core& co, hipStream_t s, uint64_t seed, uint32_t it, bool planes_f16 = false) {
         const bool lz = co.eng.method == MMW_EXPM_LANCZOS;
@@ -166,10 +171,9 @@
     }
     int phase_loss(Core& co, ChunkRun& c, IterRun& s) {
         MMW_TRY(co.kt.begin(KT_LOSS));
-        s.rs_zeroed = rs_enabled && rsfx.p != nullptr && co.bt.sddmm_mfma;
+        s.rs_zeroed = rs_zeroes(co);
         const bool sketch_have = carry.drawn(c, co.iter);
-        s.first_it = c.optimistic && pol.first_guess && c.m_launch == 1 && !c.randv && s.rs_zeroed && sizeof(T) == 4 && co.eng.mfma_now() &&
-                              c.lanczos && co.eng.use_blk && (c.Dpad % 32) == 0 && !sketch_have;
+        s.first_it = c.optimistic && c.m_launch == 1 && !c.randv && first_order_chunk(co) && !sketch_have;
         SketchArgs<T> skl{};
         if (!c.randv && !sketch_have && !co.kt_exact() && !co.sw.no_loss_sketch) {
             skl.nblocks = sketch_slabs(co); skl.K = co.K; skl.D = co.D; skl.seed = c.seed; skl.iter = (uint32_t)co.iter;
diff --git a/sig_sdp_mmw_amd/csrc/solver_replay.h b/sig_sdp_mmw_amd/csrc/solver_replay.h
--- a/sig_sdp_mmw_amd/csrc/solver_replay.h
+++ b/sig_sdp_mmw_amd/csrc/solver_replay.h
@@ -3,21 +3,68 @@
 
 namespace {
 template <typename T> struct PendingChunk {
-    DevBuf<T> sn_lval, sn_xval, sn_xavg, sn_Y, sn_yavg, sn_eaccu;
-    DevBuf<ExpmPlan> sn_plan;
-    bool sn_tiles = false;
-    bool live = false;
-    int iter0 = 0, n = 0;
-    size_t events0 = 0;
-    uint64_t seed = 0;
-    void begin(int iter0_, int n_, uint64_t seed_, size_t events0_) { live = true; iter0 = iter0_; n = n_; seed = seed_; events0 = events0_; }
-    void clear() { live = false; }
-    int copy_state(SolverCore<T>& co, bool save) {
+    struct Record { ExpmPlan plan; int viol; };
+    struct Slot {
+        DevBuf<T> sn_lval, sn_xval, sn_xavg, sn_Y, sn_yavg, sn_eaccu;
+        DevBuf<ExpmPlan> sn_plan;
+        bool sn_tiles = false;
+        PinnedBuf rec;
+        hipEvent_t ev = nullptr;
+        bool live = false;
+        bool ahead = false;
+        int iter0 = 0, n = 0;
+        size_t events0 = 0;
+        uint64_t seed = 0;
+        int m_guess = 0;
+        bool first_guess = false, first_a16_guess = false;
+        Slot() = default;
+        Slot(const Slot&) = delete;
+        Slot& operator=(const Slot&) = delete;
+        ~Slot() { if (ev) (void)hipEventDestroy(ev); }
+        const Record& record() const { return *static_cast<const Record*>(rec.p); }
+    };
+    Slot slot[2];
+    int head = 0, nlive = 0;
+    long long n_enqueued = 0, n_ahead = 0, n_dropped = 0, n_rider = 0;
+    uint64_t dropped_seed = 0;
+    int count() const { return nlive; }
+    Slot& oldest() { return slot[head]; }
+    Slot& free_slot() { return slot[(head + nlive) % 2]; }
+    void begin(Slot& s, int iter0_, int n_, uint64_t seed_, size_t events0_, bool ahead_, const ChunkPolicy& pol) {
+        s.live = true; s.ahead = ahead_; s.iter0 = iter0_; s.n = n_; s.seed = seed_; s.events0 = events0_;
+        s.m_guess = pol.m_guess; s.first_guess = pol.first_guess; s.first_a16_guess = pol.first_a16_guess;
+        ++nlive;
+        ++n_enqueued;
+        if (ahead_) ++n_ahead;
+    }
+    Slot& pop() {
+        Slot& s = slot[head];
+        s.live = false;
+        head = --nlive > 0 ? 1 - head : 0;
+        return s;
+    }
+    int drop_youngest() {
+        Slot& s = pop();
+        ++n_dropped;
+        dropped_seed = s.seed;
+        return s.n;
+    }
+    void clear() { slot[0].live = slot[1].live = false; head = 0; nlive = 0; }
+    int queue_record(SolverCore<T>& co, Slot& s) {
+        MMW_TRY(s.rec.ensure(sizeof(Record)));
+        if (!s.ev) MMW_HIP(hipEventCreateWithFlags(&s.ev, hipEventDisableTiming));
+        Record* r = static_cast<Record*>(s.rec.p);
+        MMW_HIP(hipMemcpyAsync(&r->plan, co.eng.plan_d.p, sizeof(ExpmPlan), hipMemcpyDeviceToHost, co.st));
+        MMW_HIP(hipMemcpyAsync(&r->viol, co.eng.viol_d.p, sizeof(int), hipMemcpyDeviceToHost, co.st));
+        MMW_HIP(hipEventRecord(s.ev, co.st));
+        return MMW_OK;
+    }
+    int copy_state(SolverCore<T>& co, Slot& s, bool save) {
         const size_t nnz = (size_t)co.H.nnzL(), C = (size_t)co.H.C();
-        if (save) sn_tiles = co.x.tiles;
-        else co.x.tiles = sn_tiles;
+        if (save) s.sn_tiles = co.x.tiles;
+        else co.x.tiles = s.sn_tiles;
         const typename XLayout<T>::Pair xl = co.x.live(co);
-        DevBuf<T>* snap[6] = {&sn_lval, &sn_xval, &sn_xavg, &sn_Y, &sn_yavg, &sn_eaccu};
+        DevBuf<T>* snap[6] = {&s.sn_lval, &s.sn_xval, &s.sn_xavg, &s.sn_Y, &s.sn_yavg, &s.sn_eaccu};
         DevBuf<T>* cur[6] = {&co.lval, xl.val, xl.avg, &co.Y, &co.yavg, &co.e_accu};
         const size_t len[6] = {nnz, xl.n, xl.n, C, C, C};
         CopySet<T> cs;
@@ -27,9 +74,9 @@
             cs.src[i] = save ? cur[i]->p : snap[i]->p;
             cs.n[i] = len[i];
         }
-        if (sn_plan.n < 1) MMW_TRY(sn_plan.alloc(1));
-        cs.plan_dst = save ? sn_plan.p : co.eng.plan_d.p;
-        cs.plan_src = save ? co.eng.plan_d.p : sn_plan.p;
+        if (s.sn_plan.n < 1) MMW_TRY(s.sn_plan.alloc(1));
+        cs.plan_dst = save ? s.sn_plan.p : co.eng.plan_d.p;
+        cs.plan_src = save ? co.eng.plan_d.p : s.sn_plan.p;
         hipLaunchKernelGGL((k_copy_state<T>), dim3(256, 6), dim3(BLOCK), 0, co.st, cs);
         MMW_HIP(hipGetLastError());
         if (!save && co.bt.lval_blk.p) co.lblk_stale = true;
@@ -39,13 +86,14 @@
         }
         return MMW_OK;
     }
-    int save(SolverCore<T>& co) { return copy_state(co, true); }
-    int restore(SolverCore<T>& co) { return copy_state(co, false); }
+    int save(SolverCore<T>& co, Slot& s) { return copy_state(co, s, true); }
+    int restore(SolverCore<T>& co, Slot& s) { return copy_state(co, s, false); }
 };
 struct EmaxRecord {
     DevBuf<double> d;
-    double h = 0.0;
+    PinnedBuf h;
     int enq_iter = -1, got_iter = -1;
+    int copy_iter = -1;
     template <typename T> int enqueue(SolverCore<T>& co) {
         if (co.iter <= 0) return MMW_OK;
         if (!d.p) MMW_TRY(d.alloc(1));
@@ -55,17 +103,22 @@
         got_iter = -1;
         return MMW_OK;
     }
-    template <typename T> int fetch_at_sync(SolverCore<T>& co) {
-        const bool want = enq_iter == co.iter && got_iter != co.iter && d.p != nullptr;
-        if (want) MMW_HIP(hipMemcpyAsync(&h, d.p, sizeof(double), hipMemcpyDeviceToHost, co.st));
-        MMW_HIP(hipStreamSynchronize(co.st));
-        if (want) got_iter = co.iter;
+    template <typename T> int queue_copy(SolverCore<T>& co) {
+        copy_iter = -1;
+        if (enq_iter != co.iter || got_iter == co.iter || !d.p) return MMW_OK;
+        MMW_TRY(h.ensure(sizeof(double)));
+        MMW_HIP(hipMemcpyAsync(h.p, d.p, sizeof(double), hipMemcpyDeviceToHost, co.st));
+        copy_iter = co.iter;
         return MMW_OK;
     }
-    void drop() { enq_iter = got_iter = -1; }
+    void landed(int iter) {
+        if (copy_iter >= 0 && copy_iter == iter && enq_iter == iter) got_iter = iter;
+        copy_iter = -1;
+    }
+    void drop() { enq_iter = got_iter = copy_iter = -1; }
     bool value_if_current(int iter, double* out) const {
         if (got_iter != iter || got_iter < 0) return false;
-        *out = h;
+        *out = *static_cast<const double*>(h.p);
         return true;
     }
 };
diff --git a/sig_sdp_mmw_amd/csrc/switches.h b/sig_sdp_mmw_amd/csrc/switches.h
--- a/sig_sdp_mmw_amd/csrc/switches.h
+++ b/sig_sdp_mmw_amd/csrc/switches.h
@@ -33,6 +33,7 @@
     bool cautious_replay = true;
     bool sync_plan = false;
     bool no_chunk_chain = false;
+    int chunk_depth = 2;
     bool fused_sketch = false;
     bool no_loss_sketch = false;
     bool keep_xhalf = false;
@@ -73,6 +74,7 @@
         s.cautious_replay = !is0("MMW_CAUTIOUS_REPLAY");
         s.sync_plan = on("MMW_SYNC_PLAN");
         s.no_chunk_chain = on("MMW_NO_CHUNK_CHAIN");
+        s.chunk_depth = num("MMW_CHUNK_DEPTH", 2) >= 2 ? 2 : 1;
         s.fused_sketch = on("MMW_FUSED_SKETCH");
         s.no_loss_sketch = on("MMW_NO_LOSS_SKETCH");
         s.keep_xhalf = on("MMW_KEEP_XHALF");
```

Result: no change. 6610, median of 6 (+0.4%).
